# icrdr/3D-UNet-Renal-Anatomy-Extraction

Measured on AMD Instinct MI355X. Metric: train voxels/sec (128^3 patch, bs=2 per GPU), whole job, higher is better.
Workload: dtype bf16; 1 GPU; ResUnet3D(num_pool=4, num_features=32, in=1, out=3) train step (fwd+HybirdLoss+bwd+Adam), 2x1x128^3 per GPU, dropout on; global_batch=2, parallelism=dp1, optimizer=optim.Adam (fused multi-tensor)

## Files before the change

3d-unet-renal-anatomy-extraction_amd/_native.py:

```python
import ctypes
import os
import threading

import torch

_HERE = os.path.dirname(os.path.abspath(__file__))
LIB_PATH = os.environ.get("RU3D_LIB", os.path.join(_HERE, "libru3d.so"))

F32, BF16, F16 = 0, 1, 2
PREDICT_MAX_BATCH = 16
LABEL_I64, LABEL_U8 = 0, 1
ROLE_CONV_FWD, ROLE_CONV_DGRAD, ROLE_CONVT_FWD, ROLE_CONVT_DGRAD, ROLE_BIAS = 0, 1, 2, 3, 4
LOSS_HYBIRD, LOSS_DICELOSS, LOSS_FOCAL, LOSS_DICE = 0, 1, 2, 3
MAX_CLASSES = 8


class Tensor(ctypes.Structure):
    _fields_ = [("ptr", ctypes.c_void_p), ("n", ctypes.c_int32), ("d", ctypes.c_int32), ("h", ctypes.c_int32),
                ("w", ctypes.c_int32), ("c", ctypes.c_int32), ("ld", ctypes.c_int32), ("cseg", ctypes.c_int32),
                ("seg_stride", ctypes.c_int64)]


class PackItem(ctypes.Structure):
    _fields_ = [("src", ctypes.c_void_p), ("dst", ctypes.c_void_p), ("cout", ctypes.c_int32), ("cin", ctypes.c_int32),
                ("k", ctypes.c_int32), ("stride", ctypes.c_int32), ("role", ctypes.c_int32),
                ("cout_seg", ctypes.c_int32), ("cin_seg", ctypes.c_int32)]


class PatchParams(ctypes.Structure):
    _fields_ = [("lo", ctypes.c_int32 * 3), ("before", ctypes.c_int32 * 3), ("patch", ctypes.c_int32 * 3),
                ("flip", ctypes.c_int32 * 3), ("image_cval", ctypes.c_float), ("label_cval", ctypes.c_int32),
                ("do_contrast", ctypes.c_int32), ("do_brightness", ctypes.c_int32), ("do_gamma", ctypes.c_int32),
                ("contrast", ctypes.c_float), ("brightness", ctypes.c_float), ("gamma", ctypes.c_float),
                ("gamma_eps", ctypes.c_float)]


class SpatialParams(ctypes.Structure):
    _fields_ = [("centre", ctypes.c_double * 3), ("matrix", ctypes.c_double * 9), ("lattice", ctypes.c_int32 * 3),
                ("spacing", ctypes.c_int32 * 3)]


class DegradeParams(ctypes.Structure):
    _fields_ = [("do_noise", ctypes.c_int32), ("do_blur", ctypes.c_int32), ("do_low_res", ctypes.c_int32),
                ("noise_key", ctypes.c_uint32 * 2), ("reserved", ctypes.c_int32), ("noise_variance", ctypes.c_double),
                ("blur_sigma", ctypes.c_double), ("low_res_zoom", ctypes.c_double)]


class MorphRow(ctypes.Structure):
    _fields_ = [("dx", ctypes.c_int8), ("dy", ctypes.c_int8), ("zmask", ctypes.c_uint16)]


class RenderTile(ctypes.Structure):
    _fields_ = [("volume", ctypes.c_void_p), ("table", ctypes.c_void_p), ("overlay", ctypes.c_void_p * 2),
                ("overlay_table", ctypes.c_void_p * 2), ("vmin", ctypes.c_double), ("vmax", ctypes.c_double),
                ("origin", ctypes.c_double * 2), ("step", ctypes.c_double * 2), ("x0", ctypes.c_int32),
                ("y0", ctypes.c_int32), ("w", ctypes.c_int32), ("h", ctypes.c_int32), ("X", ctypes.c_int32),
                ("Y", ctypes.c_int32), ("Z", ctypes.c_int32), ("C", ctypes.c_int32), ("channel", ctypes.c_int32),
                ("kind", ctypes.c_int32), ("axis", ctypes.c_int32), ("index", ctypes.c_int32),
                ("overlay_mode", ctypes.c_int32 * 2)]


class RenderView(ctypes.Structure):
    _fields_ = [("o", ctypes.c_double * 3), ("du", ctypes.c_double * 3), ("dv", ctypes.c_double * 3),
                ("dw", ctypes.c_double * 3), ("spacing", ctypes.c_double * 3), ("light", ctypes.c_double * 3),
                ("ambient", ctypes.c_double), ("diffuse", ctypes.c_double), ("background", ctypes.c_double * 3),
                ("num_steps", ctypes.c_int32), ("reserved", ctypes.c_int32)]


class DsLevel(ctypes.Structure):
    _fields_ = [("logits", ctypes.c_void_p), ("stride_n", ctypes.c_int64), ("stride_c", ctypes.c_int64),
                ("stride_v", ctypes.c_int64), ("d", ctypes.c_int32), ("h", ctypes.c_int32), ("w", ctypes.c_int32),
                ("shift", ctypes.c_int32)]


DS_MAX_LEVELS = 8
MASK_NE, MASK_EQ, MASK_GT, MASK_GE = 0, 1, 2, 3
TILE_F32, TILE_U8 = 0, 1
OVERLAY_FILL, OVERLAY_OUTLINE = 0, 1
RENDER_MAX_TILES = 256
MORPH_ERODE, MORPH_DILATE = 0, 1
MORPH_MAX_EXTENT, MORPH_MAX_ROWS = 15, 225
CONFUSION_MAX_CLASSES = 32
ORDER_STATS_MAX_RANKS = 8
EDT_MAX_AXIS = 4096
SPATIAL_MAX_YZ = 2560
BOUNDARY_MAX_AXIS = 2048
DEGRADE_MAX_RADIUS = 16
PACK_MAX = 40
_P = ctypes.POINTER(Tensor)
_vp, _i, _i64, _f, _sz, _u64 = (ctypes.c_void_p, ctypes.c_int, ctypes.c_int64, ctypes.c_float, ctypes.c_size_t,
                                ctypes.c_uint64)
_dbl = ctypes.c_double

_LOSS_VIEW = [_vp, _i64, _i64, _i64, _vp, _i, _i]

SIGNATURES = {
    "ru3d_version": (_i, []),
    "ru3d_last_error": (ctypes.c_char_p, []),
    "ru3d_launch_log_begin": (None, []),
    "ru3d_launch_log_end": (ctypes.c_char_p, []),
    "ru3d_packed_weight_bytes": (_sz, [_i, _i, _i, _i, _i, _i]),
    "ru3d_pack_weight": (_i, [_vp, _vp, _i, _i, _i, _i, _i, _i, _vp]),
    "ru3d_pack_weights": (_i, [ctypes.POINTER(PackItem), _i, _i, _vp]),
    "ru3d_unpad_weight_grad": (_i, [_vp, _vp, _i, _i, _i, _i, _i, _vp]),
    "ru3d_conv3d_workspace_bytes": (_sz, [_P, _P, _i, _i, _i]),
    "ru3d_conv3d_fwd": (_i, [_P, _vp, _vp, _P, _P, _i, _i, _i, _i, _vp, _sz, _vp]),
    "ru3d_conv3d_fwd_in_workspace_bytes": (_sz, [_P, _P, _i, _i, _i]),
    "ru3d_conv3d_fwd_in": (_i, [_P, _vp, _vp, _P, _i, _i, _i, _vp, _vp, _vp, _vp, _sz, _f, _vp]),
    "ru3d_conv3d_fwd_in_lrelu_workspace_bytes": (_sz, [_P, _P, _i, _i, _i]),
    "ru3d_conv3d_fwd_in_lrelu": (_i, [_P, _vp, _vp, _P, _i, _i, _i, _vp, _vp, _vp, _P, _P, _f, _vp, _sz, _f, _vp]),
    "ru3d_planar_concat_supported": (_i, [_i, _i, _i, _i, _i, _i, _i]),
    "ru3d_conv3d_dgrad": (_i, [_P, _vp, _P, _P, _i, _i, _i, _vp, _sz, _vp]),
    "ru3d_conv3d_s2_pair_fwd_in_supported": (_i, [_P, _P, _P, _i]),
    "ru3d_conv3d_s2_pair_fwd_in_workspace_bytes": (_sz, [_P, _P, _i]),
    "ru3d_conv3d_s2_pair_fwd_in": (_i, [_P, _vp, _vp, _P, _vp, _vp, _P, _vp, _vp, _vp, _vp, _sz, _f, _i, _vp]),
    "ru3d_conv3d_s1_dgrad_pair_supported": (_i, [_P, _P, _P, _i]),
    "ru3d_conv3d_s1_dgrad_pair": (_i, [_P, _vp, _P, _vp, _P, _i, _vp]),
    "ru3d_conv3d_s2_dgrad_pair_supported": (_i, [_P, _P, _P, _P, _i]),
    "ru3d_conv3d_s2_dgrad_pair": (_i, [_P, _vp, _P, _vp, _P, _P, _i, _vp]),
    "ru3d_conv3d_wgrad_workspace_bytes": (_sz, [_P, _P, _i, _i, _i]),
    "ru3d_conv3d_wgrad": (_i, [_P, _P, _vp, _vp, _sz, _i, _i, _i, _vp]),
    "ru3d_conv3d_wgrad_bias_workspace_bytes": (_sz, [_P, _P, _i, _i, _i]),
    "ru3d_conv3d_wgrad_bias": (_i, [_P, _P, _vp, _vp, _vp, _sz, _i, _i, _i, _vp]),
    "ru3d_conv3d_wgrad_pair_supported": (_i, [_P, _P, _P, _i, _i]),
    "ru3d_conv3d_wgrad_pair_workspace_bytes": (_sz, [_P, _P, _P, _i, _i]),
    "ru3d_conv3d_wgrad_pair": (_i, [_P, _P, _P, _vp, _vp, _vp, _sz, _i, _i, _vp]),
    "ru3d_head_bwd_supported": (_i, [_P, _P, _P, _i]),
    "ru3d_head_bwd_workspace_bytes": (_sz, [_P, _i]),
    "ru3d_head_bwd": (_i, [_P, _P, _vp, _i, _P, _vp, _vp, _vp, _sz, _i, _vp]),
    "ru3d_convtranspose3d_k3s2p1_fwd": (_i, [_P, _vp, _vp, _P, _i, _vp]),
    "ru3d_convtranspose3d_k3s2p1_fwd_in_workspace_bytes": (_sz, [_P, _P, _i]),
    "ru3d_convtranspose3d_k3s2p1_fwd_in": (_i, [_P, _vp, _vp, _P, _vp, _vp, _vp, _sz, _f, _i, _vp]),
    "ru3d_convtranspose3d_k3s2p1_dgrad": (_i, [_P, _vp, _P, _i, _vp]),
    "ru3d_convtranspose3d_k3s2p1_wgrad_workspace_bytes": (_sz, [_P, _P, _i]),
    "ru3d_convtranspose3d_k3s2p1_wgrad": (_i, [_P, _P, _vp, _vp, _sz, _i, _vp]),
    "ru3d_reduce_workspace_bytes": (_sz, [_P]),
    "ru3d_instnorm_stats": (_i, [_P, _vp, _vp, _vp, _vp, _sz, _f, _i, _vp]),
    "ru3d_in_lrelu_fwd": (_i, [_P, _vp, _vp, _P, _P, _f, _i, _vp]),
    "ru3d_skip1x1_in_lrelu_fwd_supported": (_i, [_P, _P, _P, _i]),
    "ru3d_skip1x1_in_lrelu_fwd": (_i, [_P, _vp, _vp, _P, _vp, _vp, _P, _f, _i, _vp]),
    "ru3d_skip1x1_in_lrelu_head_fwd_supported": (_i, [_P, _P, _P, _P, _i]),
    "ru3d_skip1x1_in_lrelu_head_fwd": (_i, [_P, _vp, _vp, _P, _vp, _vp, _P, _vp, _vp, _P, _f, _i, _vp]),
    "ru3d_head_in_bwd_supported": (_i, [_P, _P, _P, _P, _P, _i]),
    "ru3d_head_in_bwd_workspace_bytes": (_sz, [_P, _i]),
    "ru3d_head_in_bwd": (_i, [_P, _P, _vp, _i, _P, _vp, _vp, _P, _P, _vp, _vp, _vp, _vp, _sz, _f, _i, _vp]),
    "ru3d_in_lrelu_bwd": (_i, [_P, _P, _P, _vp, _vp, _P, _P, _vp, _sz, _f, _i, _vp, _vp, _i, _vp]),
    "ru3d_in_lrelu_bwd_apply": (_i, [_P, _P, _vp, _vp, _vp, _P, _f, _i, _i, _vp]),
    "ru3d_conv3d_dgrad_in_bwd_workspace_bytes": (_sz, [_P, _P, _i, _i, _i]),
    "ru3d_conv3d_dgrad_in_bwd": (_i, [_P, _vp, _P, _vp, _vp, _P, _P, _i, _i, _f, _i, _vp, _sz, _vp]),
    "ru3d_channel_sum": (_i, [_P, _vp, _vp, _sz, _i, _vp]),
    "ru3d_batchnorm_stats_pool": (_i, [_P, _vp, _vp, _vp, _sz, _i, _vp]),
    "ru3d_batchnorm_stats_finalize": (_i, [_vp, _i, _i, _i, _dbl, _vp, _vp, _vp, _f, _f, _vp, _vp, _vp, _vp, _vp, _vp, _vp]),
    "ru3d_affine_lrelu_fwd": (_i, [_P, _vp, _vp, _P, _P, _f, _i, _vp]),
    "ru3d_batchnorm_bwd_pool": (_i, [_P, _P, _P, _vp, _vp, _P, _vp, _vp, _sz, _f, _i, _vp]),
    "ru3d_batchnorm_bwd_apply": (_i, [_P, _P, _vp, _vp, _vp, _vp, _dbl, _P, _vp, _sz, _i, _i, _vp]),
    "ru3d_dropout3d_scale": (_i, [_vp, _i, _f, _u64, _u64, _vp]),
    "ru3d_dropout3d_scale_dev": (_i, [_vp, _i, _f, _u64, _u64, _vp, _vp]),
    "ru3d_pointwise": (_i, [_i, _P, _P, _P, _P, _P, _f, _i, _vp]),
    "ru3d_copy_channels": (_i, [_P, _P, _i, _vp]),
    "ru3d_add": (_i, [_P, _P, _P, _i, _vp]),
    "ru3d_cast_f32": (_i, [_P, _P, _i, _vp]),
    "ru3d_ncdhw_to_ndhwc": (_i, [_vp, _P, _i, _vp]),
    "ru3d_ndhwc_to_ncdhw": (_i, [_P, _vp, _i, _vp]),
    "ru3d_loss_state_bytes": (_sz, [_i]),
    "ru3d_loss_state_bad_labels_offset": (_sz, []),
    "ru3d_loss_workspace_bytes": (_sz, [_i, _i64, _i]),
    "ru3d_loss_fwd": (_i, _LOSS_VIEW + [_i64, _i, _i, _f, _vp, _f, _f, _f, _vp, _vp, _vp, _sz, _vp]),
    "ru3d_loss_bwd": (_i, _LOSS_VIEW + [_i64, _i, _f, _vp, _vp, _vp, _i, _vp]),
    "ru3d_tversky": (_i, [_vp, _vp, _i64, _f, _f, _f, _vp, _vp, _sz, _vp]),
    "ru3d_predict_accumulate": (_i, [_P, _i, _i, _vp, _vp, _i, _i, _i, _i, _i, _i, _vp]),
    "ru3d_predict_merge": (_i, [_vp, _vp, _i, _i, _i, _i, _i, _i, _i, _i, _i, _i, _i, _vp, _vp]),
    "ru3d_predict_gather": (_i, [_vp, _i, _i, _i, _i, _vp, _i, _P, _vp]),
    "ru3d_predict_accumulate_weighted": (_i, [_P, _i, _i, _i, _vp, _vp, _vp, _vp, _vp, _i, _i, _i, _i, _i, _i, _vp]),
    "ru3d_group_loss_state_bytes": (_sz, []),
    "ru3d_group_loss_workspace_bytes": (_sz, [_i, _i64, _i]),
    "ru3d_group_loss_fwd": (_i, _LOSS_VIEW + [_i64, _i, _vp, _i, _i, _i, _i, _f, _vp, _f, _f, _f, _vp, _vp, _vp, _sz,
                                              _vp]),
    "ru3d_group_loss_bwd": (_i, _LOSS_VIEW + [_i64, _i, _vp, _i, _i, _i, _f, _vp, _vp, _vp, _i, _vp]),
    "ru3d_topk_select_workspace_bytes": (_sz, [_i64]),
    "ru3d_topk_select_trip_elements": (_i64, []),
    "ru3d_topk_select": (_i, [_vp, _i64, _i64, _vp, _vp, _sz, _vp]),
    "ru3d_topk_loss_state_bytes": (_sz, []),
    "ru3d_topk_loss_workspace_bytes": (_sz, [_i, _i64, _i]),
    "ru3d_topk_loss_fwd": (_i, _LOSS_VIEW + [_i64, _i, _i64, _i, _vp, _f, _f, _f, _f, _vp, _vp, _vp, _vp, _sz, _vp]),
    "ru3d_topk_loss_fwd_launches": (_i, []),
    "ru3d_topk_loss_fwd_timed": (_i, _LOSS_VIEW + [_i64, _i, _i64, _i, _vp, _f, _f, _f, _f, _vp, _vp, _vp, _vp, _sz,
                                                   _vp, _vp]),
    "ru3d_topk_loss_bwd": (_i, _LOSS_VIEW + [_i64, _i, _i, _vp, _vp, _vp, _vp, _i, _vp]),
    "ru3d_predict_accumulate_groups": (_i, [_P, _i, _i, _i, _vp, _vp, _vp, _vp, _vp, _i, _i, _i, _i, _i, _i, _vp]),
    "ru3d_predict_merge_groups": (_i, [_vp, _vp, _i, _i, _i, _i, _vp, _vp, _i, _i, _i, _i, _i, _i, _vp, _vp]),
    "ru3d_components_workspace_bytes": (_sz, [_i, _i, _i]),
    "ru3d_label_components": (_i, [_vp, _i, _i, _i, _vp, _vp, _vp, _sz, _vp]),
    "ru3d_component_stats": (_i, [_vp, _i, _i, _i, _i, _vp, _vp, _vp]),
    "ru3d_filter_components_workspace_bytes": (_sz, [_i]),
    "ru3d_filter_components": (_i, [_vp, _i, _i, _i, _i, _vp, _i, _vp, _vp, _vp, _vp, _sz, _vp]),
    "ru3d_region_accumulate": (_i, [_vp, _i, _i, _i, _i, _i, _i, _i, _vp, _vp, _i, _i, _i, _vp]),
    "ru3d_cascade_merge": (_i, [_vp, _vp, _i, _i, _i, _i, _vp, _vp]),
    "ru3d_mask_bytes": (_sz, [_i, _i, _i]),
    "ru3d_mask_pack": (_i, [_vp, _i, _i, _i, _i, _i, _vp, _vp]),
    "ru3d_mask_unpack": (_i, [_vp, _i, _i, _i, _i, _i, _vp, _vp]),
    "ru3d_binary_morph": (_i, [_vp, _vp, _i, _i, _i, _i, ctypes.POINTER(MorphRow), _i, _i, _vp]),
    "ru3d_confusion_counts": (_i, [_vp, _vp, _i64, _i, _vp, _vp]),
    "ru3d_threshold_bbox": (_i, [_vp, _i, _i, _i, _i, _f, _vp, _vp, _vp]),
    "ru3d_masked_sample_workspace_bytes": (_sz, [_i, _i, _i]),
    "ru3d_masked_sample": (_i, [_vp, _i, _i, _i, _i, _i, _vp, _i, _i, _vp, _i64, _vp, _vp, _sz, _vp]),
    "ru3d_order_stats_workspace_bytes": (_sz, []),
    "ru3d_order_stats": (_i, [_vp, _i64, ctypes.POINTER(ctypes.c_int64), _i, _vp, _vp, _sz, _vp]),
    "ru3d_moments_workspace_bytes": (_sz, []),
    "ru3d_moments": (_i, [_vp, _i64, _vp, _vp, _sz, _vp]),
    "ru3d_edt_workspace_bytes": (_sz, [_i, _i, _i]),
    "ru3d_edt_squared": (_i, [_vp, _i, _i, _i, ctypes.POINTER(_dbl), _vp, _vp, _sz, _vp]),
    "ru3d_mask_surface": (_i, [_vp, _vp, _i, _i, _i, _vp]),
    "ru3d_edt_gather_workspace_bytes": (_sz, [_i, _i, _i]),
    "ru3d_edt_gather": (_i, [_vp, _vp, _i, _i, _i, _vp, _i64, _vp, _vp, _sz, _vp]),
    "ru3d_edt_reduce_workspace_bytes": (_sz, [_i64]),
    "ru3d_edt_reduce": (_i, [_vp, _vp, _i64, _dbl, _vp, _vp, _sz, _vp]),
    "ru3d_skeleton_workspace_bytes": (_sz, [_i, _i, _i]),
    "ru3d_skeleton_thin": (_i, [_vp, _i, _i, _i, _i, _vp, _sz, _vp]),
    "ru3d_skeleton_classify": (_i, [_vp, _i, _i, _i, _vp, _vp, _vp, _vp]),
    "ru3d_skeleton_length": (_i, [_vp, _i, _i, _i, ctypes.POINTER(_dbl), _vp, _vp, _sz, _vp]),
    "ru3d_skeleton_overlap": (_i, [_vp, _vp, _i, _i, _i, _vp, _vp]),
    "ru3d_skeleton_radius_stats": (_i, [_vp, _i64, _vp, _vp]),
    "ru3d_cldice_workspace_bytes": (_sz, [_i, _i, _i, _i, _i]),
    "ru3d_cldice_state_bytes": (_sz, []),
    "ru3d_soft_skeleton_fwd": (_i, [_vp, _i, _i, _i, _i, _i, _vp, _vp, _vp, _vp, _vp, _sz, _vp]),
    "ru3d_soft_skeleton_bwd": (_i, [_vp, _i, _i, _i, _i, _i, _vp, _vp, _vp, _vp, _vp, _vp, _sz, _vp]),
    "ru3d_cldice_fwd": (_i, _LOSS_VIEW + [_i, _i, _i, _i, _vp, _i, _i, _vp, _f, _vp, _vp, _vp, _vp, _vp, _vp, _vp, _vp,
                                          _sz, _vp]),
    "ru3d_cldice_bwd": (_i, _LOSS_VIEW + [_i, _i, _i, _i, _vp, _i, _i, _vp, _vp, _vp, _vp, _vp, _vp, _vp, _f, _i, _vp,
                                          _vp, _sz, _vp]),
    "ru3d_boundary_workspace_bytes": (_sz, [_i, _i, _i, _i]),
    "ru3d_boundary_state_bytes": (_sz, []),
    "ru3d_signed_distance": (_i, [_vp, _i, _i, _i, _i, _i, _i, _vp, _i, _vp, _vp, _vp, _sz, _vp]),
    "ru3d_boundary_fwd": (_i, _LOSS_VIEW + [_i, _i, _i, _i, _vp, _i, _vp, _vp, _vp, _vp, _vp, _sz, _vp]),
    "ru3d_boundary_bwd": (_i, [_vp, _i64, _i64, _i64, _i, _i, _i, _i, _i, _vp, _i, _vp, _vp, _vp, _f, _i, _vp, _vp]),
    "ru3d_ds_state_bytes": (_sz, []),
    "ru3d_ds_state_bad_labels_offset": (_sz, []),
    "ru3d_ds_block_bytes": (_sz, []),
    "ru3d_ds_loss_workspace_bytes": (_sz, [ctypes.POINTER(DsLevel), _i, _i]),
    "ru3d_ds_loss_fwd": (_i, [ctypes.POINTER(DsLevel), _i, _vp, _i, _i, _i, _i, _i, _i, _i, _f, _vp, _f, _f, _f, _vp, _vp,
                              _vp, _vp, _sz, _vp]),
    "ru3d_ds_loss_bwd": (_i, [ctypes.POINTER(DsLevel), ctypes.POINTER(_vp), _i, _vp, _i, _i, _i, _i, _i, _i, _f, _vp, _vp,
                              _vp]),
    "ru3d_mesh_workspace_bytes": (_sz, [_i, _i, _i]),
    "ru3d_mesh_count": (_i, [_vp, _i, _i, _i, _vp, _vp, _sz, _vp]),
    "ru3d_mesh_emit": (_i, [_vp, _i, _i, _i, _vp, _vp, _i64, _vp, _i64, _vp, _vp, _sz, _vp]),
    "ru3d_mesh_smooth": (_i, [_vp, _vp, _vp, _i64, _dbl, _vp]),
    "ru3d_mesh_measure_workspace_bytes": (_sz, [_i64]),
    "ru3d_mesh_measure": (_i, [_vp, _i64, _vp, _i64, _vp, _vp, _sz, _vp]),
    "ru3d_render_tiles": (_i, [_vp, _i, _vp, _i, _i, _vp]),
    "ru3d_render_surface_workspace_bytes": (_sz, [_i, _i, _i]),
    "ru3d_render_surface_prepare": (_i, [_vp, _i, _i, _i, _vp, _vp, _sz, _vp]),
    "ru3d_render_surface": (_i, [_vp, _i, _i, _i, _vp, ctypes.POINTER(RenderView), _vp, _vp, _i, _i, _vp, _sz, _vp]),
    "ru3d_adam_multi": (_i, [_vp, _vp, _i, _i, _f, _f, _f, _f, _f, _f, _f, _vp]),
    "ru3d_adam_multi_dev": (_i, [_vp, _vp, _i, _i, _vp, _vp]),
    "ru3d_adam_multi_amp": (_i, [_vp, _vp, _i, _i, _vp, _vp, _vp]),
    "ru3d_amp_update": (_i, [_vp, _f, _f, _i, _f, _f, _vp]),
    "ru3d_grad_sumsq": (_i, [_vp, _vp, _i, _i, _vp, _vp]),
    "ru3d_grad_norm_finish": (_i, [_vp, _i, _f, _vp, _f, _vp, _vp]),
    "ru3d_grad_norm": (_i, [_vp, _vp, _i, _i, _vp, _f, _f, _vp, _vp]),
    "ru3d_grad_scale_dev": (_i, [_vp, _vp, _i, _i, _vp, _vp]),
    "ru3d_sgd_multi": (_i, [_vp, _vp, _i, _i, _f, _f, _f, _i, _f, _vp, _vp]),
    "ru3d_sgd_multi_dev": (_i, [_vp, _vp, _i, _i, _vp, _vp, _vp]),
    "ru3d_adamw_multi": (_i, [_vp, _vp, _i, _i, _f, _f, _f, _f, _f, _f, _f, _f, _vp, _vp]),
    "ru3d_adamw_multi_dev": (_i, [_vp, _vp, _i, _i, _vp, _vp, _vp]),
    "ru3d_adam_multi_clip": (_i, [_vp, _vp, _i, _i, _f, _f, _f, _f, _f, _f, _f, _vp, _vp]),
    "ru3d_adam_multi_clip_dev": (_i, [_vp, _vp, _i, _i, _vp, _vp, _vp]),
    "ru3d_adam_step": (_i, [_vp, _vp, _vp, _vp, _i64, _f, _f, _f, _f, _f, _f, _f, _vp]),
    "ru3d_augment_workspace_bytes": (_sz, [_i, _i, _i]),
    "ru3d_augment_label_presence": (_i, [_vp, _i, _i, _i, _i, ctypes.POINTER(ctypes.c_int32),
                                        ctypes.POINTER(ctypes.c_int32), _i, _vp, _vp]),
    "ru3d_augment_patch": (_i, [_vp, _vp, _i, _i, _i, _i, _i, ctypes.POINTER(PatchParams), _vp, _vp, _vp, _vp, _sz,
                               _vp]),
    "ru3d_augment_patch_spatial": (_i, [_vp, _vp, _i, _i, _i, _i, _i, ctypes.POINTER(PatchParams),
                                       ctypes.POINTER(SpatialParams), _vp, _vp, _vp, _vp, _vp, _sz, _vp]),
    "ru3d_augment_degrade_workspace_bytes": (_sz, [_i, _i, _i, _i]),
    "ru3d_augment_degrade": (_i, [_vp, _i, _i, _i, _i, ctypes.POINTER(DegradeParams), _vp, _sz, _vp, _vp]),
    "ru3d_augment_intensity": (_i, [_vp, _i64, _vp, _i, ctypes.POINTER(PatchParams), _vp]),
    "ru3d_grad_scale_check": (_i, [_vp, _vp, _i, _i, _f, _vp, _vp]),
    "ru3d_comm_unique_id": (_i, [_vp]),
    "ru3d_comm_init": (_i, [ctypes.POINTER(_vp), _vp, _i, _i, _i]),
    "ru3d_comm_allreduce": (_i, [_vp, _vp, _i64, _i, _i, _vp]),
    "ru3d_comm_reduce_scatter": (_i, [_vp, _vp, _i64, _i, _i, _vp]),
    "ru3d_comm_all_gather": (_i, [_vp, _vp, _i64, _i, _vp]),
    "ru3d_comm_available": (_i, []),
    "ru3d_comm_destroy": (_i, [_vp]),
    "ru3d_probe_begin": (_i, [_i, _i, _i, _i, _i, _i]),
    "ru3d_probe_end": (_i, [ctypes.POINTER(ctypes.c_int), ctypes.POINTER(ctypes.c_double)]),
    "ru3d_set_cu_budget_device": (_i, [_i, _i]),
    "ru3d_set_cu_budget": (_i, [_i]),
    "ru3d_get_cu_budget": (_i, []),
    "ru3d_flat_cast": (_i, [_vp, _i, _vp, _i, _i64, _f, _vp]),
}
COMM_ID_BYTES = 128


def _load():
    if not os.path.exists(LIB_PATH):
        raise ImportError(
            "libru3d.so not found at %s - build it with `python __graft_entry__.py build` "
            "(hipcc --offload-arch=gfx950). There is no non-HIP fallback for the 3D U-Net hot path." % LIB_PATH)
    lib = ctypes.CDLL(LIB_PATH)
    for name, (res, args) in SIGNATURES.items():
        fn = getattr(lib, name)
        fn.restype = res
        fn.argtypes = args
    return lib


lib = _load()


class Ru3dError(RuntimeError):
    pass


def check(rc, what=""):
    if rc != 0:
        msg = lib.ru3d_last_error().decode("utf-8", "replace")
        raise Ru3dError("ru3d %s failed (status %d): %s" % (what, rc, msg))


_tls = threading.local()


def note_device(device):
    _tls.device = device


def stream(device=None):
    if device is not None:
        _tls.device = device
    dev = getattr(_tls, "device", None)
    return ctypes.c_void_p(torch.cuda.current_stream(dev).cuda_stream)


def dtype_code(dt):
    if dt == torch.float32:
        return F32
    if dt == torch.bfloat16:
        return BF16
    if dt == torch.float16:
        return F16
    raise Ru3dError("ru3d: unsupported storage dtype %s (float32, bfloat16 or float16)" % dt)


def require_device(t, what="tensor"):
    if not t.is_cuda:
        raise Ru3dError("ru3d: %s lives on %s; the MI355X-native path has no CPU fallback - move the model "
                        "and its inputs to a HIP device (.cuda())" % (what, t.device))
    _tls.device = t.device


def new_act(n, c, d, h, w, dtype, device, zero=False):
    buf = (torch.zeros if zero else torch.empty)((n, d, h, w, c), dtype=dtype, device=device)
    return buf.permute(0, 4, 1, 2, 3)


def is_ndhwc(t):
    if t.dim() != 5:
        return False
    n, c, d, h, w = t.shape
    sn, sc, sd, sh, sw = t.stride()
    if c > 1 and sc != 1:
        return False
    ld = None
    for size, stride, inner in ((w, sw, 1), (h, sh, w), (d, sd, h * w), (n, sn, d * h * w)):
        if size > 1:
            if stride % inner != 0:
                return False
            cand = stride // inner
            if ld is None:
                ld = cand
            elif cand != ld:
                return False
    return ld is None or ld >= c


def to_ndhwc(t):
    if is_ndhwc(t):
        return t
    return t.contiguous(memory_format=torch.channels_last_3d)


class Split:

    def __init__(self, t):
        n2, c, d, h, w = t.shape
        if n2 % 2 or not is_ndhwc(t) or not t.is_contiguous(memory_format=torch.channels_last_3d):
            raise Ru3dError("ru3d: a split concat must be a dense NDHWC tensor [2N, C/2, D, H, W]")
        self.t = t
        self.shape = torch.Size((n2 // 2, 2 * c, d, h, w))
        self.dtype = t.dtype
        self.device = t.device
        self.is_cuda = t.is_cuda

    def element_size(self):
        return self.t.element_size()

    def desc(self):
        n, c, d, h, w = self.shape
        _tls.device = self.t.device
        return Tensor(self.t.data_ptr(), n, d, h, w, c, c // 2, c // 2, n * d * h * w * (c // 2))


_GEOM = {}


def desc(t):
# ... 51 lines not shown
```

3d-unet-renal-anatomy-extraction_amd/_ops.py:

```python
import ctypes
import os
import threading
import weakref

import torch

import _native as N
from _native import check, desc, ptr, ref, stream

LRELU_SLOPE = 0.01
IN_EPS = 1e-5


def pack_weight(w, role, dtype, stride=1):
    N.require_device(w, "weight")
    w = w.detach()
    if w.dtype != torch.float32 or not w.is_contiguous():
        w = w.float().contiguous()
    k = w.shape[2]
    if role in (N.ROLE_CONVT_FWD, N.ROLE_CONVT_DGRAD):
        cin, cout = w.shape[0], w.shape[1]
    else:
        cout, cin = w.shape[0], w.shape[1]
    code = N.dtype_code(dtype)
    if role in (N.ROLE_CONVT_FWD, N.ROLE_CONVT_DGRAD):
        stride = 2
    nbytes = N.lib.ru3d_packed_weight_bytes(cout, cin, k, stride, role, code)
    if nbytes == 0:
        raise N.Ru3dError("ru3d: cannot pack weight of shape %s" % (tuple(w.shape),))
    out = torch.empty(nbytes, dtype=torch.uint8, device=w.device)
    check(N.lib.ru3d_pack_weight(ptr(w), ptr(out), cout, cin, k, stride, role, code, stream()), "pack_weight")
    return out


_PACK_PLANS = {}
_PACK_CACHE = {}
WEIGHTS_EPOCH = [0]


def cpad(c):
    return (c + 31) // 32 * 32


def padded_dim(real, seg):
    return (real // seg) * cpad(seg) if seg else real


def seg_of(real, have, nseg=1):
    if real % nseg or nseg * cpad(real // nseg) != have:
        raise N.Ru3dError("ru3d: a tensor with %d channels is not the padded form of %d channels in %d segment(s)"
                          % (have, real, nseg))
    return real // nseg


_PREPACK = {}


def _spec_key(sp, code):
    w, role, stride, cs, ci = sp
    return (code, w.data_ptr(), tuple(w.shape), role, stride, cs, ci)


def _prepacked(specs, code):
    if not _PREPACK:
        return None
    st = None
    outs = []
    for sp in specs:
        hit = _PREPACK.get(_spec_key(sp, code))
        if hit is None:
            return None
        pack, wref, ver, epoch, stream_id = hit
        w = sp[0]
        if st is None:
            st = torch.cuda.current_stream(w.device).cuda_stream
        if wref() is not w or ver != w._version or epoch != WEIGHTS_EPOCH[0] or stream_id != st:
            return None
        outs.append(pack)
    return outs


def prepack(specs, dtype):
    _PREPACK.clear()
    code = N.dtype_code(dtype)
    seen, uniq = set(), []
    for sp in specs:
        sp = sp if len(sp) == 5 else (sp[0], sp[1], sp[2], 0, 0)
        k = _spec_key(sp, code)
        if k not in seen:
            seen.add(k)
            uniq.append(sp)
    if not uniq:
        return

    def order(sp):
        w, role = sp[0], sp[1]
        if role == N.ROLE_BIAS:
            return (2, 0)
        return (0 if w.shape[2] == 3 else 1, 0)
    uniq.sort(key=order)
    packs = pack_weights(uniq, dtype)
    st = torch.cuda.current_stream(uniq[0][0].device).cuda_stream
    for sp, pk in zip(uniq, packs):
        _PREPACK[_spec_key(sp, code)] = (pk, weakref.ref(sp[0]), sp[0]._version, WEIGHTS_EPOCH[0], st)


def pack_weights(specs, dtype):
    code = N.dtype_code(dtype)
    specs = [sp if len(sp) == 5 else (sp[0], sp[1], sp[2], 0, 0) for sp in specs]
    pre = _prepacked(specs, code)
    if pre is not None:
        return pre
    key = (code,) + tuple((w.data_ptr(), w.shape, role, stride, cs, ci) for w, role, stride, cs, ci in specs)
    plan = _PACK_PLANS.get(key)
    if plan is None:
        metas, sizes = [], []
        for w, role, stride, cout_seg, cin_seg in specs:
            N.require_device(w, "weight")
            if w.dtype != torch.float32 or not w.is_contiguous():
                raise N.Ru3dError("ru3d: weights must be contiguous float32 parameters")
            if role == N.ROLE_BIAS:
                cout, cin, k, stride = w.shape[0], 1, 1, 1
                nbytes = 4 * padded_dim(cout, cout_seg)
            else:
                k = w.shape[2]
                if role in (N.ROLE_CONVT_FWD, N.ROLE_CONVT_DGRAD):
                    cin, cout, stride = w.shape[0], w.shape[1], 2
                else:
                    cout, cin = w.shape[0], w.shape[1]
                nbytes = N.lib.ru3d_packed_weight_bytes(padded_dim(cout, cout_seg), padded_dim(cin, cin_seg), k, stride,
                                                        role, code)
            if nbytes == 0:
                raise N.Ru3dError("ru3d: cannot pack weight of shape %s" % (tuple(w.shape),))
            metas.append((w.data_ptr(), cout, cin, k, stride, role, cout_seg, cin_seg))
            sizes.append((nbytes + 255) // 256 * 256)
        offs, off = [], 0
        for sz in sizes:
            offs.append(off)
            off += sz
        chunks = []
        for i0 in range(0, len(metas), N.PACK_MAX):
            chunk = metas[i0:i0 + N.PACK_MAX]
            items = (N.PackItem * len(chunk))()
            for j, (src, cout, cin, k, stride, role, cout_seg, cin_seg) in enumerate(chunk):
                items[j] = N.PackItem(src, 0, cout, cin, k, stride, role, cout_seg, cin_seg)
            chunks.append((i0, items))
        plan = (sizes, offs, off, chunks)
        if len(_PACK_PLANS) > 4096:
            _PACK_PLANS.clear()
        _PACK_PLANS[key] = plan
    sizes, offs, total, chunks = plan
    dev0 = specs[0][0].device
    N.note_device(dev0)
    ver = tuple(sp[0]._version for sp in specs) + (WEIGHTS_EPOCH[0], torch.cuda.current_stream(dev0).cuda_stream)
    use_cache = not torch.is_grad_enabled()
    hit = _PACK_CACHE.get(key) if use_cache else None
    if hit is not None and hit[0] == ver and all(r() is sp[0] for r, sp in zip(hit[2], specs)):
        return hit[1]
    buf = torch.empty(total, dtype=torch.uint8, device=dev0)
    base = buf.data_ptr()
    outs = [buf[o:o + sz] for o, sz in zip(offs, sizes)]
    st = stream()
    for i0, items in chunks:
        for j in range(len(items)):
            items[j].dst = base + offs[i0 + j]
        check(N.lib.ru3d_pack_weights(items, len(items), code, st), "pack_weights")
    if use_cache:
        if len(_PACK_CACHE) > 4096:
            _PACK_CACHE.clear()
        _PACK_CACHE[key] = (ver, outs, [weakref.ref(sp[0]) for sp in specs])
    return outs


def unpad_wgrad(dw_p, cout, cin, cout_seg, cin_seg):
    if not cout_seg and not cin_seg:
        return dw_p
    k = dw_p.shape[2]
    out = torch.empty((cout, cin, k, k, k), dtype=torch.float32, device=dw_p.device)
    N.note_device(dw_p.device)
    check(N.lib.ru3d_unpad_weight_grad(ptr(dw_p), ptr(out), cout, cin, k * k * k, cout_seg, cin_seg, stream()),
          "unpad_weight_grad")
    return out


def _bias(b):
    if b is None:
        return None
    b = b.detach()
    return b if (b.dtype == torch.float32 and b.is_contiguous()) else b.float().contiguous()


def _conv_out(size, k, s):
    return (size + 2 * (k // 2) - k) // s + 1


class Probe:

    def __init__(self, n, cin, cout, extent):
        self.key = (int(n),) + tuple(int(e) for e in extent) + (int(cin), int(cout))
        self.count = 0
        self.total_ms = 0.0
        self.active = False

    def start(self):
        check(N.lib.ru3d_probe_begin(*self.key), "probe_begin")
        self.active = True

    def stop(self):
        if not self.active:
            return
        n = ctypes.c_int(0)
        ms = ctypes.c_double(0.0)
        check(N.lib.ru3d_probe_end(ctypes.byref(n), ctypes.byref(ms)), "probe_end")
        self.count += n.value
        self.total_ms += ms.value
        self.active = False

    def result(self):
        self.stop()
        return self.count, (self.total_ms / self.count if self.count else 0.0)


def set_probe(p):
    cur = _PROBE[0]
    if cur is not None and cur is not p:
        cur.stop()
    _PROBE[0] = p
    if p is not None:
        p.start()


_PROBE = [None]


class launch_log:

    def __init__(self):
        self.names = []

    def __enter__(self):
        N.lib.ru3d_launch_log_begin()
        return self

    def __exit__(self, *exc):
        s = N.lib.ru3d_launch_log_end().decode("utf-8", "replace")
        self.names = s.split(";") if s else []
        return False


def _conv_ws(dsrc, ddst, k, stride, dtype, device):
    if k != 3 or stride != 1 or dtype == torch.float32:
        return None, 0
    need = N.lib.ru3d_conv3d_workspace_bytes(ref(dsrc), ref(ddst), k, stride, N.dtype_code(dtype))
    if need == 0:
        return None, 0
    buf = N.workspace(need, device)
    return ptr(buf), buf.numel()


def conv_fwd(x, pw, bias, cout, k, stride, res=None, out_dtype=None):
    n, _, d, h, w = x.shape
    out_dtype = out_dtype or x.dtype
    y = N.new_act(n, cout, _conv_out(d, k, stride), _conv_out(h, k, stride), _conv_out(w, k, stride), out_dtype,
                  x.device)
    b = _bias(bias)
    dx, dyy = desc(x), desc(y)
    dr = desc(res) if res is not None else None
    ws, wsn = _conv_ws(dx, dyy, k, stride, x.dtype, x.device)
    check(N.lib.ru3d_conv3d_fwd(ref(dx), ptr(pw), ptr(b), ref(dr), ref(dyy), k, stride, N.dtype_code(x.dtype),
                                N.dtype_code(out_dtype), ws, wsn, stream()), "conv3d_fwd")
    return y


def conv_fwd_in(x, pw, bias, cout, k, stride, drop_scale=None):
    n, _, d, h, w = x.shape
    y = N.new_act(n, cout, _conv_out(d, k, stride), _conv_out(h, k, stride), _conv_out(w, k, stride), x.dtype, x.device)
    mean = torch.empty(n * cout, dtype=torch.float32, device=x.device)
    scale = torch.empty(n * cout, dtype=torch.float32, device=x.device)
    b = _bias(bias)
    dx, dyy = desc(x), desc(y)
    code = N.dtype_code(x.dtype)
    ws = N.workspace(N.lib.ru3d_conv3d_fwd_in_workspace_bytes(ref(dx), ref(dyy), k, stride, code), x.device)
    check(N.lib.ru3d_conv3d_fwd_in(ref(dx), ptr(pw), ptr(b), ref(dyy), k, stride, code, ptr(drop_scale), ptr(mean),
                                   ptr(scale), ptr(ws), ws.numel(), IN_EPS, stream()), "conv3d_fwd_in")
    return y, mean, scale


# ... 1133 lines not shown
```

3d-unet-renal-anatomy-extraction_amd/csrc/api.hip:

```cpp
#include "common.h"
#include "conv.h"
#include <string>

#ifndef RU3D_STORAGE_F16

static thread_local std::string g_last_error;

int ru3d_fail(int code, const char* fmt, ...) {
    char buf[512];
    va_list ap;
    va_start(ap, fmt);
    vsnprintf(buf, sizeof(buf), fmt, ap);
    va_end(ap);
    g_last_error = buf;
    return code;
}

static thread_local std::string g_launch_log;
static thread_local bool g_launch_log_armed = false;

int ru3d_check_launch(const char* what) {
    if (g_launch_log_armed) {
        if (!g_launch_log.empty()) g_launch_log += ';';
        g_launch_log += what;
    }
    hipError_t e = hipGetLastError();
    if (e != hipSuccess) {
        ru3d_fail((int)e, "%s: %s", what, hipGetErrorString(e));
        return (int)e > 0 ? (int)e : 1;
    }
    return 0;
}

extern "C" int ru3d_version(void) { return RU3D_VERSION; }
extern "C" const char* ru3d_last_error(void) { return g_last_error.c_str(); }
extern "C" void ru3d_launch_log_begin(void) {
    g_launch_log.clear();
    g_launch_log_armed = true;
}
extern "C" const char* ru3d_launch_log_end(void) {
    g_launch_log_armed = false;
    return g_launch_log.c_str();
}
#endif

namespace RU3D_NS {

static bool dtype_ok(int d) { return d == RU3D_F32 || d == RU3D_BF16; }
static int conv_out(int in, int k, int s) { return (in + 2 * (k / 2) - k) / s + 1; }

static void role_channels(int cout, int cin, int role, int* kin, int* kout, int64_t* s_o, int64_t* s_i, int taps) {
    switch (role) {
        case RU3D_ROLE_CONV_FWD:
            *kin = cin; *kout = cout; *s_o = (int64_t)cin * taps; *s_i = taps; break;
        case RU3D_ROLE_CONV_DGRAD:
            *kin = cout; *kout = cin; *s_o = taps; *s_i = (int64_t)cin * taps; break;
        case RU3D_ROLE_CONVT_FWD:
            *kin = cin; *kout = cout; *s_o = taps; *s_i = (int64_t)cout * taps; break;
        default:
            *kin = cout; *kout = cin; *s_o = (int64_t)cout * taps; *s_i = taps; break;
    }
}

static bool role_uses_mfma(int kin, int kout, int k, int stride, int role, int dtype) {
    (void)stride;
    (void)role;
    return mfma_conv_eligible(kin, kout, k, dtype, dtype);
}

extern "C" size_t ru3d_packed_weight_bytes(int cout, int cin, int k, int stride, int role, int dtype) {
    RU3D_FWD_F16(dtype, ru3d_packed_weight_bytes_f16(cout, cin, k, stride, role, dtype));
    if (cout <= 0 || cin <= 0 || (k != 1 && k != 3) || (stride != 1 && stride != 2) || role < 0 || role > 3 ||
        !dtype_ok(dtype))
        return 0;
    const int taps = k * k * k;
    int kin, kout;
    int64_t s_o, s_i;
    role_channels(cout, cin, role, &kin, &kout, &s_o, &s_i, taps);
    if (role_uses_mfma(kin, kout, k, stride, role, dtype)) return mfma_packed_bytes(kin, kout, taps);
    return (size_t)taps * kin * generic_cout_pad(kout) * (dtype == RU3D_F32 ? 4 : 2);
}

extern "C" int ru3d_pack_weight(const float* src, void* dst, int cout, int cin, int k, int stride, int role, int dtype,
                                void* stream) {
    RU3D_FWD_F16(dtype, ru3d_pack_weight_f16(src, dst, cout, cin, k, stride, role, dtype, stream));
    Ru3dDeviceGuard dev_guard(stream);
    RU3D_REQUIRE(src && dst, "pack_weight: null pointer");
    RU3D_REQUIRE(cout > 0 && cin > 0 && (k == 1 || k == 3) && (stride == 1 || stride == 2),
                 "pack_weight: bad shape cout=%d cin=%d k=%d stride=%d", cout, cin, k, stride);
    RU3D_REQUIRE(role >= 0 && role <= 3 && dtype_ok(dtype), "pack_weight: bad role/dtype");
    const int taps = k * k * k;
    int kin, kout;
    int64_t s_o, s_i;
    role_channels(cout, cin, role, &kin, &kout, &s_o, &s_i, taps);
    if (role_uses_mfma(kin, kout, k, stride, role, dtype))
        return pack_mfma_launch(src, dst, kin, kout, taps, s_o, s_i, 0, as_stream(stream));
    return pack_generic_launch(src, dst, kin, kout, taps, s_o, s_i, 0, dtype, as_stream(stream));
}

static int pad32(int c) { return (c + 31) / 32 * 32; }
static int padded_dim(int real, int seg) { return seg > 0 ? (real / seg) * pad32(seg) : real; }

extern "C" int ru3d_pack_weights(const ru3d_pack_item* items, int count, int dtype, void* stream) {
    RU3D_FWD_F16(dtype, ru3d_pack_weights_f16(items, count, dtype, stream));
    Ru3dDeviceGuard dev_guard(stream);
    RU3D_REQUIRE(items && count > 0 && count <= RU3D_PACK_MAX, "pack_weights: count must be 1..%d", RU3D_PACK_MAX);
    RU3D_REQUIRE(dtype_ok(dtype), "pack_weights: bad dtype");
    PackBatch b;
    b.count = count;
    for (int i = 0; i < count; i++) {
        const ru3d_pack_item& it = items[i];
        RU3D_REQUIRE(it.src && it.dst && it.cout > 0 && it.cin > 0 && (it.k == 1 || it.k == 3) &&
                         (it.stride == 1 || it.stride == 2) && it.role >= 0 && it.role <= RU3D_ROLE_BIAS,
                     "pack_weights: bad item %d", i);
        RU3D_REQUIRE(it.cout_seg >= 0 && it.cin_seg >= 0 && (it.cout_seg == 0 || it.cout % it.cout_seg == 0) &&
                         (it.cin_seg == 0 || it.cin % it.cin_seg == 0),
                     "pack_weights: item %d: segments (%d, %d) do not divide (%d, %d)", i, it.cout_seg, it.cin_seg,
                     it.cout, it.cin);
        PackOne& p = b.item[i];
        p.src = it.src;
        p.dst = it.dst;
        if (it.role == RU3D_ROLE_BIAS) {
            p.mfma = 2;
            p.cout = padded_dim(it.cout, it.cout_seg);
            p.cin = 1; p.taps = 1; p.cout_pad = p.cout; p.s_o = 1; p.s_i = 1;
            p.co_real = it.cout_seg; p.co_pad = it.cout_seg ? pad32(it.cout_seg) : 0;
            p.ci_real = 0; p.ci_pad = 0;
            p.total = p.cout;
            continue;
        }
        const int taps = it.k * it.k * it.k;
        int kin, kout;
        int64_t s_o, s_i;
        role_channels(it.cout, it.cin, it.role, &kin, &kout, &s_o, &s_i, taps);
        const bool in_is_cin = (it.role == RU3D_ROLE_CONV_FWD || it.role == RU3D_ROLE_CONVT_FWD);
        const int kin_seg = in_is_cin ? it.cin_seg : it.cout_seg, kout_seg = in_is_cin ? it.cout_seg : it.cin_seg;
        const int kin_p = padded_dim(kin, kin_seg), kout_p = padded_dim(kout, kout_seg);
        p.cin = kin_p; p.cout = kout_p; p.taps = taps; p.s_o = s_o; p.s_i = s_i;
        p.ci_real = kin_seg; p.ci_pad = kin_seg ? pad32(kin_seg) : 0;
        p.co_real = kout_seg; p.co_pad = kout_seg ? pad32(kout_seg) : 0;
        p.mfma = role_uses_mfma(kin_p, kout_p, it.k, it.stride, it.role, dtype) ? 1 : 0;
        p.cout_pad = generic_cout_pad(kout_p);
        p.total = p.mfma ? (int64_t)taps * kin_p * kout_p : (int64_t)taps * kin_p * p.cout_pad;
    }
    PackPairBatch pairs;
    pairs.count = 0;
    if (dtype == RU3D_BF16) {
        for (int i = 0; i < count; i++) {
            PackOne& p = b.item[i];
            const ru3d_pack_item& it = items[i];
            if (p.mfma != 1 || (p.cin % 32) || (p.cout % 32) || (p.taps != 27 && p.taps != 1)) continue;
            const bool is_t = it.role == RU3D_ROLE_CONVT_FWD || it.role == RU3D_ROLE_CONVT_DGRAD;
            const bool a_major = it.role == RU3D_ROLE_CONV_FWD || it.role == RU3D_ROLE_CONVT_DGRAD;
            const int a_seg = is_t ? it.cin_seg : it.cout_seg, b_seg = is_t ? it.cout_seg : it.cin_seg;
            const int a_realdim = is_t ? it.cin : it.cout, b_realdim = is_t ? it.cout : it.cin;
            int slot = -1;
            for (int j = 0; j < pairs.count; j++)
                if (pairs.item[j].src == it.src && pairs.item[j].taps == p.taps &&
                    pairs.item[j].adim == padded_dim(a_realdim, a_seg) && pairs.item[j].bdim == padded_dim(b_realdim, b_seg) &&
                    pairs.item[j].a_real == a_seg && pairs.item[j].b_real == b_seg &&
                    (a_major ? !pairs.item[j].dst_a : !pairs.item[j].dst_b))
                    slot = j;
            if (slot < 0) {
                slot = pairs.count++;
                PackPair& q = pairs.item[slot];
                q.src = it.src; q.dst_a = nullptr; q.dst_b = nullptr;
                q.adim = padded_dim(a_realdim, a_seg); q.bdim = padded_dim(b_realdim, b_seg); q.taps = p.taps;
                q.a_real = a_seg; q.a_pad = a_seg ? pad32(a_seg) : 0;
                q.b_real = b_seg; q.b_pad = b_seg ? pad32(b_seg) : 0;
                q.s_a = (int64_t)b_realdim * p.taps;
            }
            (a_major ? pairs.item[slot].dst_a : pairs.item[slot].dst_b) = p.dst;
            p.mfma = 3;
        }
    }
    bool rest = false;
    for (int i = 0; i < count; i++) rest = rest || b.item[i].mfma != 3;
    if (pairs.count) {
        int rc = pack_pair_launch(pairs, as_stream(stream));
        if (rc || !rest) return rc;
    }
    return pack_batch_launch(b, dtype, as_stream(stream));
}

#ifndef RU3D_STORAGE_F16
extern "C" int ru3d_unpad_weight_grad(const float* src, float* dst, int cout, int cin, int taps, int cout_seg,
                                      int cin_seg, void* stream) {
    Ru3dDeviceGuard dev_guard(stream);
    RU3D_REQUIRE(src && dst && cout > 0 && cin > 0 && taps > 0, "unpad_weight_grad: bad argument");
    RU3D_REQUIRE(cout_seg >= 0 && cin_seg >= 0 && (cout_seg == 0 || cout % cout_seg == 0) &&
                     (cin_seg == 0 || cin % cin_seg == 0), "unpad_weight_grad: bad segments");
    return unpad_weight_launch(src, dst, cout, cin, taps, cout_seg, cout_seg ? pad32(cout_seg) : 0, cin_seg,
                               cin_seg ? pad32(cin_seg) : 0, padded_dim(cin, cin_seg), as_stream(stream));
}
#endif

static ConvGeom conv_geom(const ru3d_tensor* x, const ru3d_tensor* y, const ru3d_tensor* res, int k, int stride,
                          int transposed = 0, int flip = 0, int zero_far = 0) {
    ConvGeom g;
    g.N = x->n;
    g.Di = x->d; g.Hi = x->h; g.Wi = x->w; g.Cin = x->c; g.ldx = x->ld;
    g.Do = y->d; g.Ho = y->h; g.Wo = y->w; g.Cout = y->c; g.ldy = y->ld;
    g.CoutPad = generic_cout_pad(y->c);
    g.ldr = res ? res->ld : 0;
    g.k = k; g.stride = stride; g.pad = k / 2;
    g.transposed = transposed; g.zero_far = zero_far; g.flip = flip;
    g.x_cseg = x->cseg; g.x_segstride = x->seg_stride; g.y_cseg = y->cseg; g.y_segstride = y->seg_stride;
    return g;
}
static ConvGeom fwd_geom(const ru3d_tensor* x, const ru3d_tensor* y, int k, int stride) { return conv_geom(x, y, nullptr, k, stride); }
static ConvGeom dgrad_s1_geom(const ru3d_tensor* dy, const ru3d_tensor* da, int k) { return conv_geom(dy, da, nullptr, k, 1, 0, 1); }

static Conv3S1Plan s1_plan_for(const ConvGeom& g, int dtype) {
    return mfma_conv_eligible(g.Cin, g.Cout, g.k, dtype, dtype) ? conv3_s1_plan(g) : Conv3S1Plan();
}

static int run_conv(const ru3d_tensor* x, const void* w, const float* bias, const ru3d_tensor* res,
                    const ru3d_tensor* y, int k, int stride, int transposed, int flip, int zero_far, int dtype,
                    int y_dtype, hipStream_t st, void* ws = nullptr, size_t ws_bytes = 0) {
    const ConvGeom g = conv_geom(x, y, res, k, stride, transposed, flip, zero_far);
    if (g.x_cseg || g.y_cseg) {
        if (!(mfma_conv_eligible(g.Cin, g.Cout, k, dtype, y_dtype) && mfma_conv_geometry_ok(g)))
            return ru3d_fail(-1, "conv3d: no kernel takes a split tensor for this shape / dtype");
        return conv_mfma_launch(x->ptr, w, bias, res ? res->ptr : nullptr, y->ptr, g, st, nullptr, ws, ws_bytes);
    }
    if (stem_fwd_eligible(g, dtype, y_dtype, res)) return stem_fwd_launch(x->ptr, w, bias, y->ptr, g, dtype, st);
    if (head_fwd_eligible(g, dtype, res)) return head_fwd_launch(x->ptr, w, bias, y->ptr, g, dtype, y_dtype, st);
    if (!bias && head_dgrad_eligible(g, dtype, y_dtype, res)) return head_dgrad_launch(x->ptr, w, y->ptr, g, dtype, st);
    if (mfma_conv_eligible(g.Cin, g.Cout, k, dtype, y_dtype) && mfma_conv_geometry_ok(g))
        return conv_mfma_launch(x->ptr, w, bias, res ? res->ptr : nullptr, y->ptr, g, st, nullptr, ws, ws_bytes);
    if (mfma_conv_eligible(g.Cin, g.Cout, k, dtype, dtype))
        return ru3d_fail(-1, "conv3d: %d -> %d channels k=%d is packed in MFMA fragment order, which has no kernel for "
                             "input dtype %d -> output dtype %d", g.Cin, g.Cout, k, dtype, y_dtype);
    return conv_generic_launch(x->ptr, w, bias, res ? res->ptr : nullptr, y->ptr, g, dtype, y_dtype, st);
}

static bool res_ok(const ru3d_tensor* res, const ru3d_tensor* y) {
    return !res || (tensor_ok(res) && res->n == y->n && res->d == y->d && res->h == y->h && res->w == y->w &&
                    res->c == y->c);
}

extern "C" size_t ru3d_conv3d_workspace_bytes(const ru3d_tensor* x, const ru3d_tensor* y, int k, int stride, int dtype) {
    RU3D_FWD_F16(dtype, ru3d_conv3d_workspace_bytes_f16(x, y, k, stride, dtype));
    if (!tensor_ok_split(x) || !tensor_ok(y) || dtype != RU3D_BF16 || k != 3 || stride != 1) return 0;
    return s1_plan_for(fwd_geom(x, y, k, stride), dtype).ws_bytes;
}

extern "C" int ru3d_conv3d_fwd(const ru3d_tensor* x, const void* w_packed, const float* bias, const ru3d_tensor* res,
                               const ru3d_tensor* y, int k, int stride, int dtype, int y_dtype, void* ws,
                               size_t ws_bytes, void* stream) {
    RU3D_FWD_F16(dtype, ru3d_conv3d_fwd_f16(x, w_packed, bias, res, y, k, stride, dtype, y_dtype, ws, ws_bytes, stream));
    Ru3dDeviceGuard dev_guard(stream);
    RU3D_REQUIRE(tensor_ok_split(x) && tensor_ok(y) && w_packed, "conv3d_fwd: bad tensor/weight");
    RU3D_REQUIRE((k == 1 || k == 3) && (stride == 1 || stride == 2), "conv3d_fwd: k=%d stride=%d unsupported", k, stride);
    RU3D_REQUIRE(dtype_ok(dtype) && dtype_ok(y_dtype) && !(dtype == RU3D_F32 && y_dtype == RU3D_BF16),
                 "conv3d_fwd: bad dtypes %d -> %d", dtype, y_dtype);
    RU3D_REQUIRE(x->n == y->n && y->d == conv_out(x->d, k, stride) && y->h == conv_out(x->h, k, stride) &&
                     y->w == conv_out(x->w, k, stride),
                 "conv3d_fwd: output extents (%d,%d,%d) do not match input (%d,%d,%d) k=%d s=%d", y->d, y->h, y->w,
                 x->d, x->h, x->w, k, stride);
    RU3D_REQUIRE(res_ok(res, y), "conv3d_fwd: residual shape mismatch");
    return run_conv(x, w_packed, bias, res, y, k, stride, 0, 0, 0, dtype, y_dtype, as_stream(stream), ws, ws_bytes);
}

static size_t fwd_in_ws_bytes(const ru3d_tensor* y, const Conv3S1Plan& p) {
    size_t need = ru3d_reduce_workspace_bytes(y);
    if (p.can_stats && p.slab_bytes > need) need = p.slab_bytes;
    return p.ws_bytes > need ? p.ws_bytes : need;
}

extern "C" size_t ru3d_conv3d_fwd_in_workspace_bytes(const ru3d_tensor* x, const ru3d_tensor* y, int k, int stride,
                                                     int dtype) {
    RU3D_FWD_F16(dtype, ru3d_conv3d_fwd_in_workspace_bytes_f16(x, y, k, stride, dtype));
    if (!tensor_ok_split(x) || !tensor_ok(y)) return 0;
    return fwd_in_ws_bytes(y, s1_plan_for(fwd_geom(x, y, k, stride), dtype));
}

static int conv_fwd_in(const ru3d_tensor* x, const void* w_packed, const float* bias, const ru3d_tensor* y, int k, int stride,
                       int dtype, const float* drop_scale, float* mean, float* scale, void* ws, size_t ws_bytes, float eps,
                       void* stream, const ConvGeom& g, const Conv3S1Plan& p) {
    RU3D_REQUIRE(ws_bytes >= fwd_in_ws_bytes(y, p), "conv3d_fwd_in: workspace too small");
    if (p.can_stats) {
        RU3D_REQUIRE(x->n == y->n && y->d == x->d && y->h == x->h && y->w == x->w, "conv3d_fwd_in: extents mismatch");
        int rc = conv_mfma_launch(x->ptr, w_packed, bias, nullptr, y->ptr, g, as_stream(stream), (float*)ws, nullptr, 0, nullptr,
                                  0, 0.f, nullptr, 0, nullptr, nullptr, &p);
        if (rc) return rc;
        return stats_slab_finalize_launch((const float*)ws, p.gx, p.cb, g.N, g.Cout, 1.0 / ((double)g.Do * g.Ho * g.Wo),
                                          drop_scale, eps, mean, scale, as_stream(stream));
    }
    int rc = ru3d_conv3d_fwd(x, w_packed, bias, nullptr, y, k, stride, dtype, dtype, ws, ws_bytes, stream);
    if (rc) return rc;
    return ru3d_instnorm_stats(y, drop_scale, mean, scale, ws, ws_bytes, eps, dtype, stream);
}

extern "C" int ru3d_conv3d_fwd_in(const ru3d_tensor* x, const void* w_packed, const float* bias, const ru3d_tensor* y,
                                  int k, int stride, int dtype, const float* drop_scale, float* mean, float* scale,
                                  void* ws, size_t ws_bytes, float eps, void* stream) {
    RU3D_FWD_F16(dtype, ru3d_conv3d_fwd_in_f16(x, w_packed, bias, y, k, stride, dtype, drop_scale, mean, scale, ws, ws_bytes, eps, stream));
    Ru3dDeviceGuard dev_guard(stream);
    RU3D_REQUIRE(tensor_ok_split(x) && tensor_ok(y) && w_packed && mean && scale && ws, "conv3d_fwd_in: bad argument");
    const ConvGeom g = fwd_geom(x, y, k, stride);
    return conv_fwd_in(x, w_packed, bias, y, k, stride, dtype, drop_scale, mean, scale, ws, ws_bytes, eps, stream, g,
                       s1_plan_for(g, dtype));
}

static bool small_conv_path(const ConvGeom& g, const Conv3S1Plan& p, int dtype) {
    return g.k == 3 && g.stride == 1 && mfma_conv_eligible(g.Cin, g.Cout, g.k, dtype, dtype) && !p.can_stats;
}

#ifndef RU3D_STORAGE_F16
extern "C" size_t ru3d_conv3d_fwd_in_lrelu_workspace_bytes(const ru3d_tensor* x, const ru3d_tensor* y, int k, int stride,
                                                           int dtype) {
    return ru3d_conv3d_fwd_in_workspace_bytes(x, y, k, stride, dtype);
}
#endif

extern "C" int ru3d_conv3d_fwd_in_lrelu(const ru3d_tensor* x, const void* w_packed, const float* bias, const ru3d_tensor* y,
                                        int k, int stride, int dtype, const float* drop_scale, float* mean, float* scale,
                                        const ru3d_tensor* res, const ru3d_tensor* out, float slope, void* ws,
                                        size_t ws_bytes, float eps, void* stream) {
    RU3D_FWD_F16(dtype, ru3d_conv3d_fwd_in_lrelu_f16(x, w_packed, bias, y, k, stride, dtype, drop_scale, mean, scale, res, out, slope, ws, ws_bytes, eps, stream));
    Ru3dDeviceGuard dev_guard(stream);
    RU3D_REQUIRE(tensor_ok_split(x) && tensor_ok(y) && tensor_ok(out) && w_packed && mean && scale && ws,
                 "conv3d_fwd_in_lrelu: bad argument");
    RU3D_REQUIRE(res_ok(res, y) && res_ok(out, y), "conv3d_fwd_in_lrelu: res / out do not have the shape of y");
    const ConvGeom g = fwd_geom(x, y, k, stride);
    const Conv3S1Plan p = s1_plan_for(g, dtype);
    const int small = (small_conv_path(g, p, dtype) && x->n == y->n && y->d == x->d && y->h == x->h &&
                       y->w == x->w) ? in_small_mode(y, false, res, out) : 0;
    if (small) {
        RU3D_REQUIRE(ws_bytes >= fwd_in_ws_bytes(y, p), "conv3d_fwd_in_lrelu: workspace too small");
// ... 477 lines not shown
```

3d-unet-renal-anatomy-extraction_amd/csrc/conv_generic.hip:

```cpp
#include "common.h"
#include "conv.h"

namespace RU3D_NS {

template <typename T, typename TO, int CO_T, int VEC, bool TRANSPOSED>
__global__ __launch_bounds__(256) void conv_generic_kernel(const T* __restrict__ x, const T* __restrict__ w,
                                                           const float* __restrict__ bias,
                                                           const TO* __restrict__ res, TO* __restrict__ y,
                                                           ConvGeom g) {
    const int64_t total = (int64_t)g.N * g.Do * g.Ho * g.Wo;
    const int64_t vo = (int64_t)blockIdx.x * 256 + threadIdx.x;
    if (vo >= total) return;
    const int co0 = blockIdx.y * CO_T;
    int ow = (int)(vo % g.Wo);
    int64_t t = vo / g.Wo;
    int oh = (int)(t % g.Ho);
    t /= g.Ho;
    int od = (int)(t % g.Do);
    int n = (int)(t / g.Do);

    float acc[CO_T];
#pragma unroll
    for (int j = 0; j < CO_T; j++) acc[j] = 0.f;

    const int k = g.k, s = g.stride, p = g.pad;
    for (int kd = 0; kd < k; kd++) {
        int id;
        if (!TRANSPOSED) {
            id = od * s + kd - p;
            if (id < 0 || id >= g.Di) continue;
        } else {
            int q = od + p - kd;
            if (q < 0 || (q % s) != 0) continue;
            id = q / s;
            if (id >= g.Di) continue;
        }
        for (int kh = 0; kh < k; kh++) {
            int ih;
            if (!TRANSPOSED) {
                ih = oh * s + kh - p;
                if (ih < 0 || ih >= g.Hi) continue;
            } else {
                int q = oh + p - kh;
                if (q < 0 || (q % s) != 0) continue;
                ih = q / s;
                if (ih >= g.Hi) continue;
            }
            for (int kw = 0; kw < k; kw++) {
                int iw;
                if (!TRANSPOSED) {
                    iw = ow * s + kw - p;
                    if (iw < 0 || iw >= g.Wi) continue;
                } else {
                    int q = ow + p - kw;
                    if (q < 0 || (q % s) != 0) continue;
                    iw = q / s;
                    if (iw >= g.Wi) continue;
                }
                const int tap = (kd * k + kh) * k + kw;
                const T* xp = x + ((((int64_t)n * g.Di + id) * g.Hi + ih) * g.Wi + iw) * g.ldx;
                const int wtap = g.flip ? (k * k * k - 1 - tap) : tap;
                const T* wp = w + (int64_t)wtap * g.Cin * g.CoutPad + co0;
                for (int ci = 0; ci < g.Cin; ci += VEC) {
                    float xv[VEC];
                    load_vec<T, VEC>(xp + ci, xv);
#pragma unroll
                    for (int u = 0; u < VEC; u++) {
                        const T* wr = wp + (int64_t)(ci + u) * g.CoutPad;
#pragma unroll
                        for (int j = 0; j < CO_T; j++) acc[j] = fmaf(xv[u], to_f32<T>(wr[j]), acc[j]);
                    }
                }
            }
        }
    }
    const bool far = g.zero_far && (od == g.Do - 1 || oh == g.Ho - 1 || ow == g.Wo - 1);
#pragma unroll
    for (int j = 0; j < CO_T; j++) {
        const int co = co0 + j;
        if (co < g.Cout) {
            float v = acc[j];
            if (bias) v += bias[co];
            if (far) v = 0.f;
            if (res) v += to_f32<TO>(res[vo * g.ldr + co]);
            y[vo * g.ldy + co] = from_f32<TO>(v);
        }
    }
}

int generic_cot(int cout) { return cout <= 4 ? 4 : (cout % 16 == 0 ? 16 : 8); }
int generic_cout_pad(int cout) {
    int t = generic_cot(cout);
    return (cout + t - 1) / t * t;
}

template <typename T, typename TO, int CO_T, int VEC>
static int launch_generic2(const void* x, const void* w, const float* bias, const void* res, void* y,
                           const ConvGeom& g, hipStream_t st) {
    const int64_t total = (int64_t)g.N * g.Do * g.Ho * g.Wo;
    dim3 grid((unsigned)((total + 255) / 256), (unsigned)(g.CoutPad / CO_T));
    if (g.transposed)
        hipLaunchKernelGGL((conv_generic_kernel<T, TO, CO_T, VEC, true>), grid, dim3(256), 0, st, (const T*)x,
                           (const T*)w, bias, (const TO*)res, (TO*)y, g);
    else
        hipLaunchKernelGGL((conv_generic_kernel<T, TO, CO_T, VEC, false>), grid, dim3(256), 0, st, (const T*)x,
                           (const T*)w, bias, (const TO*)res, (TO*)y, g);
    return ru3d_check_launch("conv_generic");
}

template <typename T, typename TO>
static int launch_generic1(const void* x, const void* w, const float* bias, const void* res, void* y,
                           const ConvGeom& g, hipStream_t st) {
    const bool v4 = (g.Cin % 4 == 0) && (g.ldx % 4 == 0) && (((uintptr_t)x) % (4 * sizeof(T)) == 0);
    const int cot = generic_cot(g.Cout);
#define GO(CO, V) return launch_generic2<T, TO, CO, V>(x, w, bias, res, y, g, st)
    if (cot == 4) { if (v4) GO(4, 4); else GO(4, 1); }
    if (cot == 8) { if (v4) GO(8, 4); else GO(8, 1); }
    if (v4) GO(16, 4); else GO(16, 1);
#undef GO
}

int conv_generic_launch(const void* x, const void* w, const float* bias, const void* res, void* y,
                        const ConvGeom& g, int dtype, int y_dtype, hipStream_t st) {
    if (dtype == RU3D_F32 && y_dtype == RU3D_F32) return launch_generic1<float, float>(x, w, bias, res, y, g, st);
    if (dtype == RU3D_BF16 && y_dtype == RU3D_BF16) return launch_generic1<bf16, bf16>(x, w, bias, res, y, g, st);
    if (dtype == RU3D_BF16 && y_dtype == RU3D_F32) return launch_generic1<bf16, float>(x, w, bias, res, y, g, st);
    return ru3d_fail(-1, "conv_generic: unsupported dtype pair (%d -> %d)", dtype, y_dtype);
}

template <typename T>
__global__ void pack_generic_kernel(const float* __restrict__ src, T* __restrict__ dst, int cin, int cout,
                                    int cout_pad, int taps, int64_t s_o, int64_t s_i, int flip) {
    const int64_t total = (int64_t)taps * cin * cout_pad;
    for (int64_t i = (int64_t)blockIdx.x * blockDim.x + threadIdx.x; i < total; i += (int64_t)gridDim.x * blockDim.x) {
        int co = (int)(i % cout_pad);
        int64_t t = i / cout_pad;
        int ci = (int)(t % cin);
        int tap = (int)(t / cin);
        float v = 0.f;
        if (co < cout) {
            int st = flip ? (taps - 1 - tap) : tap;
            v = src[co * s_o + ci * s_i + st];
        }
        dst[i] = from_f32<T>(v);
    }
}

int pack_generic_launch(const float* src, void* dst, int cin, int cout, int taps, int64_t s_o, int64_t s_i,
                        int flip, int dtype, hipStream_t st) {
    const int cp = generic_cout_pad(cout);
    const int64_t total = (int64_t)taps * cin * cp;
    int blocks = (int)((total + 255) / 256);
    if (blocks > 4096) blocks = 4096;
    if (dtype == RU3D_F32)
        hipLaunchKernelGGL(pack_generic_kernel<float>, dim3(blocks), dim3(256), 0, st, src, (float*)dst, cin, cout, cp,
                           taps, s_o, s_i, flip);
    else
        hipLaunchKernelGGL(pack_generic_kernel<bf16>, dim3(blocks), dim3(256), 0, st, src, (bf16*)dst, cin, cout, cp,
                           taps, s_o, s_i, flip);
    return ru3d_check_launch("pack_generic");
}

#define PACK_TILE_FLOATS (32 * (16 * 27 + 1))
__device__ __forceinline__ int pack_src_index(int p, int real, int pad) {
    if (pad == 0) return p;
    const int seg = p / pad, off = p - seg * pad;
    return off < real ? seg * real + off : -1;
}

template <typename T>
__global__ __launch_bounds__(256) void pack_batch_kernel(PackBatch b) {
    __shared__ float tile[PACK_TILE_FLOATS];
    const PackOne& p = b.item[blockIdx.y];
    T* dst = (T*)p.dst;
    const int taps = p.taps;
    if (p.mfma == 3) return;
    if (p.mfma == 2) {
        float* out = (float*)p.dst;
        for (int i = blockIdx.x * 256 + threadIdx.x; i < p.cout; i += gridDim.x * 256) {
            const int sc = pack_src_index(i, p.co_real, p.co_pad);
            out[i] = sc >= 0 ? p.src[sc] : 0.f;
        }
        return;
    }
    const bool rows_co = (p.s_i == taps), rows_ci = (p.s_o == taps);
    if (p.mfma && sizeof(T) == 2 && taps <= 27 && (rows_co || rows_ci)) {
        const int KS = p.cin / 16, NTT = p.cout / 32;
        const int nrows = rows_co ? 32 : 16, rowlen = (rows_co ? 16 : 32) * taps, pitch = rowlen + 1;
        for (int unit = blockIdx.x; unit < KS * NTT; unit += gridDim.x) {
            const int ks = unit / NTT, nt = unit % NTT;
            const int co_s = pack_src_index(nt * 32, p.co_real, p.co_pad);
            const int ci_s = pack_src_index(ks * 16, p.ci_real, p.ci_pad);
            int co_n = 32, ci_n = 16;
            if (p.co_pad) co_n = co_s < 0 ? 0 : min(32, p.co_real - (nt * 32) % p.co_pad);
            if (p.ci_pad) ci_n = ci_s < 0 ? 0 : min(16, p.ci_real - (ks * 16) % p.ci_pad);
            const float* base = p.src + (int64_t)(co_s < 0 ? 0 : co_s) * p.s_o + (int64_t)(ci_s < 0 ? 0 : ci_s) * p.s_i;
            const int64_t row_stride = rows_co ? p.s_o : p.s_i;
            const int row_n = rows_co ? co_n : ci_n, col_n = (rows_co ? ci_n : co_n) * taps;
            __syncthreads();
            for (int e = threadIdx.x; e < nrows * rowlen; e += 256) {
                const int r = e / rowlen, j = e - r * rowlen;
                tile[r * pitch + j] = (r < row_n && j < col_n) ? base[(int64_t)r * row_stride + j] : 0.f;
            }
            __syncthreads();
            for (int e = threadIdx.x; e < taps * 64; e += 256) {
                const int tap = e >> 6, lane = e & 63;
                const int co = lane & 31, ci0 = 8 * (lane >> 5);
                bf16x8 v;
#pragma unroll
                for (int j = 0; j < 8; j++) {
                    const int ci = ci0 + j;
                    const float f = rows_co ? tile[co * pitch + ci * taps + tap] : tile[ci * pitch + co * taps + tap];
                    v[j] = (bf16)f;
                }
                *reinterpret_cast<bf16x8*>((bf16*)p.dst + ((((int64_t)tap * KS + ks) * NTT + nt) * 64 + lane) * 8) = v;
            }
        }
        return;
    }
    for (int64_t i = (int64_t)blockIdx.x * 256 + threadIdx.x; i < p.total; i += (int64_t)gridDim.x * 256) {
        float v = 0.f;
        if (p.mfma) {
            const int KS = p.cin / 16, NTT = p.cout / 32;
            const int j = (int)(i & 7);
            const int lane = (int)((i >> 3) & 63);
            int64_t t = i >> 9;
            const int nt = (int)(t % NTT);
            t /= NTT;
            const int ks = (int)(t % KS);
            const int tap = (int)(t / KS);
            const int co = pack_src_index(nt * 32 + (lane & 31), p.co_real, p.co_pad);
            const int ci = pack_src_index(ks * 16 + 8 * (lane >> 5) + j, p.ci_real, p.ci_pad);
            if (co >= 0 && ci >= 0) v = p.src[co * p.s_o + ci * p.s_i + tap];
        } else {
            const int co = (int)(i % p.cout_pad);
            const int64_t t = i / p.cout_pad;
            const int ci = pack_src_index((int)(t % p.cin), p.ci_real, p.ci_pad);
            const int tap = (int)(t / p.cin);
            const int cs = co < p.cout ? pack_src_index(co, p.co_real, p.co_pad) : -1;
            if (cs >= 0 && ci >= 0) v = p.src[cs * p.s_o + ci * p.s_i + tap];
        }
        dst[i] = from_f32<T>(v);
    }
}

#define PP_PITCH 40
#define PP_PLANE (32 * PP_PITCH + 8)
template <int TAPS>
__global__ __launch_bounds__(256) void pack_pair_kernel(PackPairBatch pb) {
    __shared__ __attribute__((aligned(16))) bf16 tile[TAPS * PP_PLANE];
    const PackPair& p = pb.item[blockIdx.y];
    if (p.taps != TAPS) return;
    constexpr int taps = TAPS;
    const int TA = p.adim / 32, TB = p.bdim / 32;
    const int lane = threadIdx.x & 63, wave = threadIdx.x >> 6;
    for (int unit = blockIdx.x; unit < TA * TB; unit += gridDim.x) {
        const int ta = unit / TB, tb = unit % TB;
        const int a_s = pack_src_index(ta * 32, p.a_real, p.a_pad), b_s = pack_src_index(tb * 32, p.b_real, p.b_pad);
        int a_n = 32, b_n = 32;
        if (p.a_pad) a_n = a_s < 0 ? 0 : min(32, p.a_real - (ta * 32) % p.a_pad);
        if (p.b_pad) b_n = b_s < 0 ? 0 : min(32, p.b_real - (tb * 32) % p.b_pad);
        const float* base = p.src + (int64_t)(a_s < 0 ? 0 : a_s) * p.s_a + (int64_t)(b_s < 0 ? 0 : b_s) * taps;
        constexpr int run = 32 * taps;
        const int run_n = b_n * taps;
        __syncthreads();
        const bool vec_ok = ((p.s_a | run_n) & 3) == 0 && ((((uintptr_t)base) & 15) == 0);
        if (vec_ok) {
            constexpr int run4 = run / 4;
            for (int e0 = threadIdx.x; e0 < 32 * run4; e0 += 8 * 256) {
                f32x4 v[8];
#pragma unroll
                for (int u = 0; u < 8; u++) {
                    const int e = e0 + u * 256;
                    const int a = e / run4, j4 = e - a * run4;
                    const f32x4 z4 = {0.f, 0.f, 0.f, 0.f};
                    v[u] = (e < 32 * run4 && a < a_n && 4 * j4 < run_n)
                               ? *reinterpret_cast<const f32x4*>(base + (int64_t)a * p.s_a + 4 * j4) : z4;
                }
#pragma unroll
                for (int u = 0; u < 8; u++) {
                    const int e = e0 + u * 256;
                    if (e < 32 * run4) {
                        const int a = e / run4, j4 = e - a * run4;
#pragma unroll
                        for (int q = 0; q < 4; q++) {
                            const int j = 4 * j4 + q;
                            const int b = j / taps, tap = j - b * taps;
                            tile[tap * PP_PLANE + a * PP_PITCH + b] = (bf16)v[u][q];
                        }
                    }
                }
            }
        } else {
            for (int e0 = threadIdx.x; e0 < 32 * run; e0 += 4 * 256) {
                float v[4];
#pragma unroll
                for (int u = 0; u < 4; u++) {
                    const int e = e0 + u * 256;
                    const int a = e / run, j = e - a * run;
                    v[u] = (e < 32 * run && a < a_n && j < run_n) ? base[(int64_t)a * p.s_a + j] : 0.f;
                }
#pragma unroll
                for (int u = 0; u < 4; u++) {
                    const int e = e0 + u * 256;
                    const int a = e / run, j = e - a * run;
                    const int b = j / taps, tap = j - b * taps;
                    if (e < 32 * run) tile[tap * PP_PLANE + a * PP_PITCH + b] = (bf16)v[u];
                }
            }
        }
        __syncthreads();
        if (p.dst_a) {
            const int KS = p.bdim / 16, NTT = TA;
            for (int f = wave; f < taps * 2; f += 4) {
                const int tap = f >> 1, kc = f & 1;
                const bf16x8 v = *reinterpret_cast<const bf16x8*>(&tile[tap * PP_PLANE + (lane & 31) * PP_PITCH + 16 * kc + 8 * (lane >> 5)]);
                *reinterpret_cast<bf16x8*>((bf16*)p.dst_a + ((((int64_t)tap * KS + 2 * tb + kc) * NTT + ta) * 64 + lane) * 8) = v;
            }
        }
        if (p.dst_b) {
            const int KS = p.adim / 16, NTT = TB;
            for (int f = wave; f < taps * 2; f += 4) {
                const int tap = f >> 1, kc = f & 1;
                const int a0 = 16 * kc + 8 * (lane >> 5);
                bf16x8 v;
#pragma unroll
                for (int j = 0; j < 8; j++) v[j] = tile[tap * PP_PLANE + (a0 + j) * PP_PITCH + (lane & 31)];
                *reinterpret_cast<bf16x8*>((bf16*)p.dst_b + ((((int64_t)tap * KS + 2 * ta + kc) * NTT + tb) * 64 + lane) * 8) = v;
            }
        }
    }
}

int pack_pair_launch(const PackPairBatch& b, hipStream_t st) {
    int64_t mx = 1;
    for (int i = 0; i < b.count; i++) {
        const int64_t units = (int64_t)(b.item[i].adim / 32) * (b.item[i].bdim / 32);
        mx = units > mx ? units : mx;
    }
    if (mx > 1024) mx = 1024;
    bool t27 = false, t1 = false;
    for (int i = 0; i < b.count; i++) {
        t27 = t27 || b.item[i].taps == 27;
        t1 = t1 || b.item[i].taps == 1;
    }
    if (t27) hipLaunchKernelGGL(pack_pair_kernel<27>, dim3((unsigned)mx, b.count), dim3(256), 0, st, b);
    if (t1) hipLaunchKernelGGL(pack_pair_kernel<1>, dim3((unsigned)mx, b.count), dim3(256), 0, st, b);
    return ru3d_check_launch("pack_pair");
}

__global__ __launch_bounds__(256) void unpad_weight_kernel(const float* __restrict__ src, float* __restrict__ dst,
                                                           int cout, int cin, int taps, int co_real, int co_pad,
                                                           int ci_real, int ci_pad, int cin_p) {
    const int64_t total = (int64_t)cout * cin * taps;
    for (int64_t i = (int64_t)blockIdx.x * 256 + threadIdx.x; i < total; i += (int64_t)gridDim.x * 256) {
        const int tap = (int)(i % taps);
        const int64_t t = i / taps;
        const int ci = (int)(t % cin), co = (int)(t / cin);
        const int cop = co_pad ? (co / co_real) * co_pad + co % co_real : co;
        const int cip = ci_pad ? (ci / ci_real) * ci_pad + ci % ci_real : ci;
        dst[i] = src[((int64_t)cop * cin_p + cip) * taps + tap];
    }
}

int unpad_weight_launch(const float* src, float* dst, int cout, int cin, int taps, int co_real, int co_pad, int ci_real,
                        int ci_pad, int cin_p, hipStream_t st) {
    const int64_t total = (int64_t)cout * cin * taps;
    int64_t blocks = (total + 1023) / 1024;
    if (blocks > 2048) blocks = 2048;
    hipLaunchKernelGGL(unpad_weight_kernel, dim3((unsigned)blocks), dim3(256), 0, st, src, dst, cout, cin, taps, co_real,
                       co_pad, ci_real, ci_pad, cin_p);
    return ru3d_check_launch("unpad_weight_grad");
}

int pack_batch_launch(const PackBatch& b, int dtype, hipStream_t st) {
    int64_t mx = 1;
    for (int i = 0; i < b.count; i++) mx = b.item[i].total > mx ? b.item[i].total : mx;
    int64_t blocks = (mx + 1023) / 1024;
    if (blocks > 2048) blocks = 2048;
    dim3 grid((unsigned)blocks, b.count);
    if (dtype == RU3D_F32)
        hipLaunchKernelGGL(pack_batch_kernel<float>, grid, dim3(256), 0, st, b);
    else
        hipLaunchKernelGGL(pack_batch_kernel<bf16>, grid, dim3(256), 0, st, b);
    return ru3d_check_launch("pack_batch");
}

#define WG_PB 16
template <typename T>
__global__ __launch_bounds__(256) void wgrad_generic_kernel(const T* __restrict__ x, const T* __restrict__ dy,
                                                            float* __restrict__ part, WgradGeom g) {
    __shared__ float xs[WG_PB][64 + 4];
    __shared__ float ds[WG_PB][64 + 4];
    const int tid = threadIdx.x;
    const int chunk = blockIdx.x, tap = blockIdx.y;
    const int co_tiles = (g.Cout + 63) / 64;
    const int ci0 = (blockIdx.z / co_tiles) * 64, co0 = (blockIdx.z % co_tiles) * 64;
    const int kw = tap % g.k, kh = (tap / g.k) % g.k, kd = tap / (g.k * g.k);
    const int ty = tid / 16, tx = tid % 16;
    float acc[4][4];
#pragma unroll
    for (int i = 0; i < 4; i++)
#pragma unroll
        for (int j = 0; j < 4; j++) acc[i][j] = 0.f;

    const int64_t P = (int64_t)g.N * g.Do * g.Ho * g.Wo;
    const int64_t p_begin = (int64_t)chunk * g.chunk_len;
    int64_t p_end = p_begin + g.chunk_len;
    if (p_end > P) p_end = P;

    for (int64_t p0 = p_begin; p0 < p_end; p0 += WG_PB) {
#pragma unroll
        for (int r = 0; r < 4; r++) {
            const int e = tid + r * 256;
            const int pl = e / 64, c = e % 64;
            const int64_t pos = p0 + pl;
            float xv = 0.f, dv = 0.f;
            if (pos < p_end) {
                int ow = (int)(pos % g.Wo);
                int64_t t = pos / g.Wo;
                int oh = (int)(t % g.Ho);
                t /= g.Ho;
                int od = (int)(t % g.Do);
                int n = (int)(t / g.Do);
                if (co0 + c < g.Cout) dv = to_f32<T>(dy[pos * g.lddy + co0 + c]);
                const int id = od * g.stride + kd - g.pad, ih = oh * g.stride + kh - g.pad,
                          iw = ow * g.stride + kw - g.pad;
                if (ci0 + c < g.Cin && id >= 0 && id < g.Di && ih >= 0 && ih < g.Hi && iw >= 0 && iw < g.Wi)
                    xv = to_f32<T>(x[((((int64_t)n * g.Di + id) * g.Hi + ih) * g.Wi + iw) * g.ldx + ci0 + c]);
            }
            xs[pl][c] = xv;
            ds[pl][c] = dv;
        }
        __syncthreads();
#pragma unroll
        for (int pl = 0; pl < WG_PB; pl++) {
            float a[4], b[4];
#pragma unroll
            for (int i = 0; i < 4; i++) a[i] = xs[pl][ty * 4 + i];
#pragma unroll
            for (int j = 0; j < 4; j++) b[j] = ds[pl][tx * 4 + j];
#pragma unroll
            for (int i = 0; i < 4; i++)
#pragma unroll
                for (int j = 0; j < 4; j++) acc[i][j] = fmaf(a[i], b[j], acc[i][j]);
        }
        __syncthreads();
    }
    float* pp = part + ((int64_t)chunk * g.taps + tap) * g.Cin * g.Cout;
#pragma unroll
    for (int i = 0; i < 4; i++) {
        const int ci = ci0 + ty * 4 + i;
        if (ci >= g.Cin) continue;
#pragma unroll
        for (int j = 0; j < 4; j++) {
            const int co = co0 + tx * 4 + j;
            if (co < g.Cout) pp[(int64_t)ci * g.Cout + co] = acc[i][j];
        }
    }
}

template <int QX>
__global__ __launch_bounds__(256) void wgrad_reduce_kernel(const float* __restrict__ part, float* __restrict__ dw,
                                                           int chunks, int taps, int cin, int cout, int64_t s_o,
                                                           int64_t s_i) {
    constexpr int KY = 256 / QX;
    __shared__ f32x4 sh[KY][QX];
    const int64_t total = (int64_t)taps * cin * cout;
    const int ox = threadIdx.x % QX, ky = threadIdx.x / QX;
    const int64_t i0 = ((int64_t)blockIdx.x * QX + ox) * 4;
    f32x4 s = {0.f, 0.f, 0.f, 0.f};
    const bool full = (i0 + 3 < total) && ((total & 3) == 0);
    if (full) {
        f32x4 s0 = s, s1 = s, s2 = s, s3 = s;
        int c = ky;
        for (; c + 3 * KY < chunks; c += 4 * KY) {
            s0 += *reinterpret_cast<const f32x4*>(part + (int64_t)c * total + i0);
            s1 += *reinterpret_cast<const f32x4*>(part + (int64_t)(c + KY) * total + i0);
            s2 += *reinterpret_cast<const f32x4*>(part + (int64_t)(c + 2 * KY) * total + i0);
            s3 += *reinterpret_cast<const f32x4*>(part + (int64_t)(c + 3 * KY) * total + i0);
        }
        for (; c < chunks; c += KY) s0 += *reinterpret_cast<const f32x4*>(part + (int64_t)c * total + i0);
        s = (s0 + s1) + (s2 + s3);
// ... 167 lines not shown
```

3d-unet-renal-anatomy-extraction_amd/csrc/optim.hip:

```cpp
#include "common.h"
#include <stddef.h>

template <class Rule>
__device__ __forceinline__ void multi_body(const ru3d_adam_tensor* __restrict__ tensors,
                                           const int32_t* __restrict__ block_map, int chunk_elems, const Rule rule,
                                           const float* __restrict__ coef) {
    const ru3d_adam_tensor t = tensors[block_map[2 * blockIdx.x]];
    if (!t.grad) return;
    const bool first = rule.first();
    if ((first && !t.exp_avg) || (Rule::kSecond && !t.exp_avg_sq)) return;
    const int64_t begin = (int64_t)block_map[2 * blockIdx.x + 1] * chunk_elems;
    int64_t end = begin + chunk_elems;
    if (end > t.count) end = t.count;
    const float c = coef ? *coef : 1.f;
    uintptr_t bits = ((uintptr_t)t.param) | ((uintptr_t)t.grad);
    if (first) bits |= (uintptr_t)t.exp_avg;
    if (Rule::kSecond) bits |= (uintptr_t)t.exp_avg_sq;
    int64_t i = begin + (int64_t)threadIdx.x * 4;
    if ((bits & 15) == 0) {
        for (; i + 3 < end; i += 1024) {
            f32x4 p = *reinterpret_cast<const f32x4*>(t.param + i);
            const f32x4 g = *reinterpret_cast<const f32x4*>(t.grad + i);
            f32x4 m = {0.f, 0.f, 0.f, 0.f}, v = {0.f, 0.f, 0.f, 0.f};
            if (first) m = *reinterpret_cast<const f32x4*>(t.exp_avg + i);
            if (Rule::kSecond) v = *reinterpret_cast<const f32x4*>(t.exp_avg_sq + i);
#pragma unroll
            for (int k = 0; k < 4; k++) {
                float pk = p[k], mk = m[k], vk = v[k];
                rule.elem(pk, g[k], c, mk, vk);
                p[k] = pk; m[k] = mk; v[k] = vk;
            }
            *reinterpret_cast<f32x4*>(t.param + i) = p;
            if (first) *reinterpret_cast<f32x4*>(t.exp_avg + i) = m;
            if (Rule::kSecond) *reinterpret_cast<f32x4*>(t.exp_avg_sq + i) = v;
        }
    }
    for (; i < end; i += 1024)
        for (int k = 0; k < 4 && i + k < end; k++) {
            float pk = t.param[i + k], mk = first ? t.exp_avg[i + k] : 0.f, vk = Rule::kSecond ? t.exp_avg_sq[i + k] : 0.f;
            rule.elem(pk, t.grad[i + k], c, mk, vk);
            t.param[i + k] = pk;
            if (first) t.exp_avg[i + k] = mk;
            if (Rule::kSecond) t.exp_avg_sq[i + k] = vk;
        }
}

struct SgdRule {
    float lr, mu, wd, gscale;
    bool nesterov;
    static constexpr bool kSecond = false;
    __device__ __forceinline__ bool first() const { return mu != 0.f; }
    __device__ __forceinline__ void elem(float& p, float g, float c, float& b, float&) const {
#pragma clang fp contract(off)
        const float gh = g * gscale * c;
        float d = gh;
        if (wd != 0.f) d = gh + wd * p;
        float u = d;
        if (mu != 0.f) {
            b = mu * b + d;
            u = nesterov ? d + mu * b : b;
        }
        p -= lr * u;
    }
};

__device__ __forceinline__ SgdRule sgd_rule(float lr, float mu, float wd, float nesterov, float gscale) {
    SgdRule r;
    r.lr = lr; r.mu = mu; r.wd = wd; r.gscale = gscale; r.nesterov = nesterov != 0.f;
    return r;
}

__global__ __launch_bounds__(256) void sgd_multi_kernel(const ru3d_adam_tensor* __restrict__ tensors,
                                                        const int32_t* __restrict__ block_map, int chunk_elems, float lr,
                                                        float mu, float wd, float nesterov, float gscale,
                                                        const float* __restrict__ coef) {
    multi_body(tensors, block_map, chunk_elems, sgd_rule(lr, mu, wd, nesterov, gscale), coef);
}

__global__ __launch_bounds__(256) void sgd_multi_dev_kernel(const ru3d_adam_tensor* __restrict__ tensors,
                                                            const int32_t* __restrict__ block_map, int chunk_elems,
                                                            const float* __restrict__ hyper,
                                                            const float* __restrict__ coef) {
    multi_body(tensors, block_map, chunk_elems, sgd_rule(hyper[0], hyper[1], hyper[2], hyper[3], hyper[6]), coef);
}

template <bool kDecay>
struct AdamRule {
    float b1, b2, eps, step, bc2_sqrt, gscale, keep;
    static constexpr bool kSecond = true;
    __device__ __forceinline__ bool first() const { return true; }
    __device__ __forceinline__ void elem(float& p, float g, float c, float& m, float& v) const {
#pragma clang fp contract(off)
        const float gi = g * gscale * c;
        if (kDecay) p = p * keep;
        m = b1 * m + (1.f - b1) * gi;
        v = b2 * v + (1.f - b2) * gi * gi;
        p -= step * (m / (sqrtf(v) / bc2_sqrt + eps));
    }
};

template <bool kDecay>
__device__ __forceinline__ AdamRule<kDecay> adam_rule(float lr, float b1, float b2, float eps, float bc1, float bc2_sqrt,
                                                      float gscale, float wd) {
#pragma clang fp contract(off)
    AdamRule<kDecay> r;
    r.b1 = b1; r.b2 = b2; r.eps = eps; r.bc2_sqrt = bc2_sqrt; r.gscale = gscale;
    r.step = lr / bc1;
    r.keep = 1.f - lr * wd;
    return r;
}

__global__ __launch_bounds__(256) void adam_clip_kernel(const ru3d_adam_tensor* __restrict__ tensors,
                                                        const int32_t* __restrict__ block_map, int chunk_elems, float lr,
                                                        float b1, float b2, float eps, float bc1, float bc2_sqrt,
                                                        float gscale, const float* __restrict__ coef) {
    multi_body(tensors, block_map, chunk_elems, adam_rule<false>(lr, b1, b2, eps, bc1, bc2_sqrt, gscale, 0.f), coef);
}

__global__ __launch_bounds__(256) void adam_clip_dev_kernel(const ru3d_adam_tensor* __restrict__ tensors,
                                                            const int32_t* __restrict__ block_map, int chunk_elems,
                                                            const float* __restrict__ hyper,
                                                            const float* __restrict__ coef) {
    multi_body(tensors, block_map, chunk_elems,
               adam_rule<false>(hyper[0], hyper[1], hyper[2], hyper[3], hyper[4], hyper[7], hyper[6], 0.f), coef);
}

__global__ __launch_bounds__(256) void adamw_multi_kernel(const ru3d_adam_tensor* __restrict__ tensors,
                                                          const int32_t* __restrict__ block_map, int chunk_elems, float lr,
                                                          float b1, float b2, float eps, float wd, float bc1, float bc2,
                                                          float gscale, const float* __restrict__ coef) {
    multi_body(tensors, block_map, chunk_elems, adam_rule<true>(lr, b1, b2, eps, bc1, sqrtf(bc2), gscale, wd), coef);
}

__global__ __launch_bounds__(256) void adamw_multi_dev_kernel(const ru3d_adam_tensor* __restrict__ tensors,
                                                              const int32_t* __restrict__ block_map, int chunk_elems,
                                                              const float* __restrict__ hyper,
                                                              const float* __restrict__ coef) {
    multi_body(tensors, block_map, chunk_elems,
               adam_rule<true>(hyper[0], hyper[1], hyper[2], hyper[3], hyper[4], sqrtf(hyper[5]), hyper[6], hyper[7]),
               coef);
}

__global__ __launch_bounds__(256) void adam_kernel(float* __restrict__ p, const float* __restrict__ g,
                                                   float* __restrict__ m, float* __restrict__ v, int64_t count,
                                                   float lr, float b1, float b2, float eps, float bc1, float bc2_sqrt,
                                                   float gscale) {
    for (int64_t i = (int64_t)blockIdx.x * 256 + threadIdx.x; i < count; i += (int64_t)gridDim.x * 256) {
        const float gi = g[i] * gscale;
        const float mi = b1 * m[i] + (1.f - b1) * gi;
        const float vi = b2 * v[i] + (1.f - b2) * gi * gi;
        m[i] = mi;
        v[i] = vi;
        const float denom = sqrtf(vi) / bc2_sqrt + eps;
        p[i] -= (lr / bc1) * (mi / denom);
    }
}

extern "C" int ru3d_adam_step(float* param, const float* grad, float* exp_avg, float* exp_avg_sq, int64_t count,
                              float lr, float beta1, float beta2, float eps, float bias_corr1, float bias_corr2,
                              float grad_scale, void* stream) {
    Ru3dDeviceGuard dev_guard(stream);
    RU3D_REQUIRE(param && grad && exp_avg && exp_avg_sq && count > 0, "adam_step: bad argument");
    int64_t b = (count + 1023) / 1024;
    if (b > 4096) b = 4096;
    hipLaunchKernelGGL(adam_kernel, dim3((unsigned)b), dim3(256), 0, as_stream(stream), param, grad, exp_avg,
                       exp_avg_sq, count, lr, beta1, beta2, eps, bias_corr1, sqrtf(bias_corr2), grad_scale);
    return ru3d_check_launch("adam_step");
}

__device__ __forceinline__ void adam_multi_body(const ru3d_adam_tensor* __restrict__ tensors,
                                                const int32_t* __restrict__ block_map, int chunk_elems, float lr,
                                                float b1, float b2, float eps, float bc1, float bc2_sqrt, float gscale) {
#pragma clang fp contract(off)
    const ru3d_adam_tensor t = tensors[block_map[2 * blockIdx.x]];
    if (!t.grad) return;
    const int64_t begin = (int64_t)block_map[2 * blockIdx.x + 1] * chunk_elems;
    int64_t end = begin + chunk_elems;
    if (end > t.count) end = t.count;
    const float step = lr / bc1;
    const bool vec = ((((uintptr_t)t.param) | ((uintptr_t)t.grad) | ((uintptr_t)t.exp_avg) | ((uintptr_t)t.exp_avg_sq)) & 15) == 0;
    int64_t i = begin + (int64_t)threadIdx.x * 4;
    if (vec) {
        for (; i + 3 < end; i += 1024) {
            f32x4 p = *reinterpret_cast<const f32x4*>(t.param + i);
            const f32x4 g = *reinterpret_cast<const f32x4*>(t.grad + i);
            f32x4 m = *reinterpret_cast<const f32x4*>(t.exp_avg + i);
            f32x4 v = *reinterpret_cast<const f32x4*>(t.exp_avg_sq + i);
#pragma unroll
            for (int k = 0; k < 4; k++) {
                const float gi = g[k] * gscale;
                m[k] = b1 * m[k] + (1.f - b1) * gi;
                v[k] = b2 * v[k] + (1.f - b2) * gi * gi;
                p[k] -= step * (m[k] / (sqrtf(v[k]) / bc2_sqrt + eps));
            }
            *reinterpret_cast<f32x4*>(t.param + i) = p;
            *reinterpret_cast<f32x4*>(t.exp_avg + i) = m;
            *reinterpret_cast<f32x4*>(t.exp_avg_sq + i) = v;
        }
    }
    for (; i < end; i += 1024)
        for (int k = 0; k < 4 && i + k < end; k++) {
            const float gi = t.grad[i + k] * gscale;
            const float mi = b1 * t.exp_avg[i + k] + (1.f - b1) * gi;
            const float vi = b2 * t.exp_avg_sq[i + k] + (1.f - b2) * gi * gi;
            t.exp_avg[i + k] = mi;
            t.exp_avg_sq[i + k] = vi;
            t.param[i + k] -= step * (mi / (sqrtf(vi) / bc2_sqrt + eps));
        }
}


__global__ __launch_bounds__(256) void adam_multi_kernel(const ru3d_adam_tensor* __restrict__ tensors,
                                                         const int32_t* __restrict__ block_map, int chunk_elems,
                                                         float lr, float b1, float b2, float eps, float bc1,
                                                         float bc2_sqrt, float gscale) {
    adam_multi_body(tensors, block_map, chunk_elems, lr, b1, b2, eps, bc1, bc2_sqrt, gscale);
}

__global__ __launch_bounds__(256) void adam_multi_dev_kernel(const ru3d_adam_tensor* __restrict__ tensors,
                                                             const int32_t* __restrict__ block_map, int chunk_elems,
                                                             const float* __restrict__ hyper) {
    adam_multi_body(tensors, block_map, chunk_elems, hyper[0], hyper[1], hyper[2], hyper[3], hyper[4], hyper[7], hyper[6]);
}

extern "C" int ru3d_adam_multi(const ru3d_adam_tensor* tensors, const int32_t* block_map, int nblocks, int chunk_elems,
                               float lr, float beta1, float beta2, float eps, float bias_corr1, float bias_corr2,
                               float grad_scale, void* stream) {
    Ru3dDeviceGuard dev_guard(stream);
    RU3D_REQUIRE(tensors && block_map && nblocks > 0 && chunk_elems >= 1024 && (chunk_elems % 1024) == 0,
                 "adam_multi: bad argument (chunk_elems must be a positive multiple of 1024)");
    hipLaunchKernelGGL(adam_multi_kernel, dim3((unsigned)nblocks), dim3(256), 0, as_stream(stream), tensors, block_map,
                       chunk_elems, lr, beta1, beta2, eps, bias_corr1, sqrtf(bias_corr2), grad_scale);
    return ru3d_check_launch("adam_multi");
}

extern "C" int ru3d_adam_multi_dev(const ru3d_adam_tensor* tensors, const int32_t* block_map, int nblocks,
                                   int chunk_elems, const float* hyper, void* stream) {
    Ru3dDeviceGuard dev_guard(stream);
    RU3D_REQUIRE(tensors && block_map && hyper && nblocks > 0 && chunk_elems >= 1024 && (chunk_elems % 1024) == 0,
                 "adam_multi_dev: bad argument (chunk_elems must be a positive multiple of 1024)");
    hipLaunchKernelGGL(adam_multi_dev_kernel, dim3((unsigned)nblocks), dim3(256), 0, as_stream(stream), tensors,
                       block_map, chunk_elems, hyper);
    return ru3d_check_launch("adam_multi_dev");
}

__global__ __launch_bounds__(256) void adam_multi_amp_kernel(const ru3d_adam_tensor* __restrict__ tensors,
                                                             const int32_t* __restrict__ block_map, int chunk_elems,
                                                             const float* __restrict__ hyper,
                                                             const ru3d_amp_state* __restrict__ amp) {
    if (amp->found_inf != 0.f) return;
    const int t = __float_as_int(hyper[5]) + amp->steps + 1;
    const double b1d = (double)hyper[1] + (double)hyper[4], b2d = (double)hyper[2] + (double)hyper[7];
    const double bc1 = 1.0 - pow(b1d, (double)t), bc2 = 1.0 - pow(b2d, (double)t);
    adam_multi_body(tensors, block_map, chunk_elems, hyper[0], hyper[1], hyper[2], hyper[3], (float)bc1, sqrtf((float)bc2),
                    amp->inv_scale);
}

__global__ void amp_update_kernel(ru3d_amp_state* amp, float growth, float backoff, int interval, float min_scale,
                                  float max_scale) {
    if (threadIdx.x || blockIdx.x) return;
    if (amp->found_inf != 0.f) {
        amp->scale = fmaxf(amp->scale * backoff, min_scale);
        amp->tracker = 0;
        amp->skipped += 1;
    } else {
        amp->steps += 1;
        amp->tracker += 1;
        if (amp->tracker >= interval) {
            amp->scale = fminf(amp->scale * growth, max_scale);
            amp->tracker = 0;
        }
    }
    amp->inv_scale = 1.f / amp->scale;
    amp->found_inf = 0.f;
}

extern "C" int ru3d_adam_multi_amp(const ru3d_adam_tensor* tensors, const int32_t* block_map, int nblocks, int chunk_elems,
                                   const float* hyper, const ru3d_amp_state* amp, void* stream) {
    Ru3dDeviceGuard dev_guard(stream);
    RU3D_REQUIRE(tensors && block_map && hyper && amp && nblocks > 0 && chunk_elems >= 1024 && (chunk_elems % 1024) == 0,
                 "adam_multi_amp: bad argument (chunk_elems must be a positive multiple of 1024)");
    hipLaunchKernelGGL(adam_multi_amp_kernel, dim3((unsigned)nblocks), dim3(256), 0, as_stream(stream), tensors, block_map,
                       chunk_elems, hyper, amp);
    return ru3d_check_launch("adam_multi_amp");
}

extern "C" int ru3d_amp_update(ru3d_amp_state* amp, float growth_factor, float backoff_factor, int growth_interval,
                               float min_scale, float max_scale, void* stream) {
    Ru3dDeviceGuard dev_guard(stream);
    RU3D_REQUIRE(amp && growth_factor >= 1.f && backoff_factor > 0.f && backoff_factor <= 1.f && growth_interval > 0 &&
                     min_scale > 0.f && max_scale >= min_scale, "amp_update: bad argument");
    hipLaunchKernelGGL(amp_update_kernel, dim3(1), dim3(64), 0, as_stream(stream), amp, growth_factor, backoff_factor,
                       growth_interval, min_scale, max_scale);
    return ru3d_check_launch("amp_update");
}

__global__ __launch_bounds__(256) void grad_scale_check_kernel(const ru3d_adam_tensor* __restrict__ tensors,
                                                               const int32_t* __restrict__ block_map, int chunk_elems,
                                                               float scale, float* __restrict__ found_inf) {
    const ru3d_adam_tensor t = tensors[block_map[2 * blockIdx.x]];
    if (!t.grad) return;
    float* g = const_cast<float*>(t.grad);
    const int64_t begin = (int64_t)block_map[2 * blockIdx.x + 1] * chunk_elems;
    int64_t end = begin + chunk_elems;
    if (end > t.count) end = t.count;
    const bool write = scale != 1.f;
    bool bad = false;
    int64_t i = begin + (int64_t)threadIdx.x * 4;
    if ((((uintptr_t)g) & 15) == 0) {
        for (; i + 3 < end; i += 1024) {
            f32x4 v = *reinterpret_cast<const f32x4*>(g + i);
#pragma unroll
            for (int k = 0; k < 4; k++) {
                bad = bad || !(fabsf(v[k]) <= 3.402823466e38f);
                v[k] *= scale;
            }
            if (write) *reinterpret_cast<f32x4*>(g + i) = v;
        }
    }
    for (; i < end; i += 1024)
        for (int k = 0; k < 4 && i + k < end; k++) {
            const float v = g[i + k];
            bad = bad || !(fabsf(v) <= 3.402823466e38f);
            if (write) g[i + k] = v * scale;
        }
    if (__any(bad) && (threadIdx.x & 63) == 0) *found_inf = 1.f;
}

extern "C" int ru3d_grad_scale_check(const ru3d_adam_tensor* tensors, const int32_t* block_map, int nblocks,
                                     int chunk_elems, float scale, float* found_inf, void* stream) {
    Ru3dDeviceGuard dev_guard(stream);
    RU3D_REQUIRE(tensors && block_map && found_inf && nblocks > 0 && chunk_elems >= 1024 && (chunk_elems % 1024) == 0,
                 "grad_scale_check: bad argument (chunk_elems must be a positive multiple of 1024)");
    hipLaunchKernelGGL(grad_scale_check_kernel, dim3((unsigned)nblocks), dim3(256), 0, as_stream(stream), tensors,
                       block_map, chunk_elems, scale, found_inf);
    return ru3d_check_launch("grad_scale_check");
}

__device__ __forceinline__ double block_sum_d(double v, double* lds) {
    v = wave_sum_d(v);
    if ((threadIdx.x & 63) == 0) lds[threadIdx.x >> 6] = v;
    __syncthreads();
    return ((lds[0] + lds[1]) + lds[2]) + lds[3];
}

__global__ __launch_bounds__(256) void grad_sumsq_kernel(const ru3d_adam_tensor* __restrict__ tensors,
                                                         const int32_t* __restrict__ block_map, int chunk_elems,
                                                         double* __restrict__ partials) {
    __shared__ double lds[4];
    const ru3d_adam_tensor t = tensors[block_map[2 * blockIdx.x]];
    double acc = 0.0;
    if (t.grad) {
        const float* g = t.grad;
        const int64_t begin = (int64_t)block_map[2 * blockIdx.x + 1] * chunk_elems;
        int64_t end = begin + chunk_elems;
        if (end > t.count) end = t.count;
        int64_t i = begin + (int64_t)threadIdx.x * 4;
        if ((((uintptr_t)g) & 15) == 0) {
            for (; i + 3 < end; i += 1024) {
                const f32x4 v = *reinterpret_cast<const f32x4*>(g + i);
#pragma unroll
                for (int k = 0; k < 4; k++) acc += (double)v[k] * (double)v[k];
            }
        }
        for (; i < end; i += 1024)
            for (int k = 0; k < 4 && i + k < end; k++) acc += (double)g[i + k] * (double)g[i + k];
    }
    const double s = block_sum_d(acc, lds);
    if (threadIdx.x == 0) partials[blockIdx.x] = s;
}

__global__ __launch_bounds__(256) void grad_norm_finish_kernel(const double* __restrict__ partials, int n,
                                                               float grad_scale, const float* __restrict__ hyper,
                                                               float max_norm, float* __restrict__ out) {
    __shared__ double lds[4];
    double acc = 0.0;
    for (int i = threadIdx.x; i < n; i += 256) acc += partials[i];
    const double s = block_sum_d(acc, lds);
    if (threadIdx.x == 0) {
        const float gs = hyper ? hyper[6] : grad_scale;
        const float total = (float)((double)gs * sqrt(s));
        const float c = max_norm / (total + 1e-6f);
        out[0] = total;
        out[1] = c > 1.f ? 1.f : c;
    }
}

__global__ __launch_bounds__(256) void grad_scale_dev_kernel(const ru3d_adam_tensor* __restrict__ tensors,
                                                             const int32_t* __restrict__ block_map, int chunk_elems,
                                                             const float* __restrict__ coef) {
    const ru3d_adam_tensor t = tensors[block_map[2 * blockIdx.x]];
    if (!t.grad) return;
    const float c = *coef;
    if (c == 1.f) return;
    float* g = const_cast<float*>(t.grad);
    const int64_t begin = (int64_t)block_map[2 * blockIdx.x + 1] * chunk_elems;
// ... 121 lines not shown
```

3d-unet-renal-anatomy-extraction_amd/graph.py:

```python
import torch

import _native as N
import _ops
import loss as _loss
import optim as _optim

_RING = 8


class GraphedTrainStep:
    def __init__(self, model, criterion, optimizer, warmup=2, scaler=None):
        if not isinstance(optimizer, _optim._Fused):
            raise TypeError("GraphedTrainStep needs optim.Adam, optim.AdamW or optim.SGD (their update kernels read the "
                            "per-step scalars from device memory)")
        if scaler is not None and not optimizer.captures_with_scaler():
            raise TypeError("GraphedTrainStep: a captured fp16 step (device-side loss scaler) needs optim.Adam without "
                            "max_grad_norm; SGD, AdamW and clipped steps run the eager fp16 loop")
        self.model, self.criterion, self.optimizer = model, criterion, optimizer
        self.scaler = scaler
        self.warmup = max(1, int(warmup))
        self.graph = None
        self.key = None
        self.replays = 0
        self.eager_steps = 0

    def _eager(self, x, y):
        self.optimizer.zero_grad(set_to_none=True)
        logits = self.model(x)
        loss = self.criterion(logits, y)
        stepped = True
        if self.scaler is None:
            loss.backward()
            self.optimizer.step()
        elif self.scaler._dev is not None:
            stepped = self.scaler.eager_step(self.optimizer, loss)
        else:
            self.scaler.scale(loss).backward()
            stepped = self.scaler.step(self.optimizer)
        self.eager_steps += 1 if (stepped or self.graph is not None) else 0
        self.skipped_warmup = getattr(self, "skipped_warmup", 0) + (0 if stepped else 1)
        self.logits = _loss.main_output(logits).detach()
        return loss.detach()

    def _capture(self, x, y):
        dev = x.device
        groups = len(self.optimizer.param_groups)
        self.stream = torch.cuda.Stream(dev)
        drop0 = _ops._drop_counter[0]
        import loss as _loss_mod
        try:
            self.x = torch.empty_like(x)
            self.y = torch.empty_like(y)
            self.x.copy_(x)
            self.y.copy_(y)
            self.block = torch.zeros(8 + groups * 32, dtype=torch.uint8, device=dev)
            self.drop_base = self.block[:8].view(torch.int64)
            self.hyper = self.block[8:].view(torch.float32).view(groups, 8)
            self.host = [torch.zeros(8 + groups * 32, dtype=torch.uint8).pin_memory() for _ in range(_RING)]
            self.host_ev = [None] * _RING
            self.optimizer.begin_capture(self.hyper)
            if self.scaler is not None:
                self.scaler.begin_capture(self.optimizer, dev)
            self.optimizer.zero_grad(set_to_none=True)
            g = torch.cuda.CUDAGraph()
            _ops.DROP_OFFSET_BASE[0] = self.drop_base
            _loss_mod.CAPTURE_SINK[0] = self.label_states = []
            self.stream.wait_stream(torch.cuda.current_stream(dev))
            try:
                with torch.cuda.graph(g, stream=self.stream, capture_error_mode="thread_local"):
                    logits = self.model(self.x)
                    loss = self.criterion(logits, self.y)
                    if self.scaler is None:
                        loss.backward()
                        self.optimizer.step()
                    else:
                        self.scaler.scale(loss).backward()
                        self.scaler.step(self.optimizer)
                    self.loss = loss.detach()
                    self._static_logits = _loss_mod.main_output(logits).detach()
            finally:
                _ops.DROP_OFFSET_BASE[0] = None
                _loss_mod.CAPTURE_SINK[0] = None
        except BaseException:
            _ops._drop_counter[0] = drop0
            cap = self.optimizer._captured
            if cap is not None and cap["steps"]:
                cap["dirty"] = True
            self.release()
            raise
        self.draws = _ops._drop_counter[0] - drop0
        _ops._drop_counter[0] = drop0
        self.drop_origin = drop0
        self.graph = g
        self.key = (tuple(x.shape), x.dtype, tuple(y.shape), y.dtype, dev)

    def __call__(self, x, y):
        key = (tuple(x.shape), x.dtype, tuple(y.shape), y.dtype, x.device)
        if self.graph is None:
            if self.eager_steps < self.warmup:
                return self._eager(x, y)
            self._capture(x, y)
        elif key != self.key:
            return self._eager(x, y)
        else:
            self.x.copy_(x, non_blocking=True)
            self.y.copy_(y, non_blocking=True)
        slot = self.replays % _RING
        if self.host_ev[slot] is not None:
            self.host_ev[slot].synchronize()
        host = self.host[slot]
        host[:8].view(torch.int64)[0] = _ops._drop_counter[0] - self.drop_origin
        self.optimizer.replay_scalars(host[8:].view(torch.float32).view(-1, 8))
        self.block.copy_(host, non_blocking=True)
        ev = torch.cuda.Event()
        ev.record()
        self.host_ev[slot] = ev
        self.graph.replay()
        if self.label_states:
            import loss as _loss_mod
            for st in self.label_states:
                _loss_mod._note_label_flag(st)
        _ops._drop_counter[0] += self.draws
        _ops.WEIGHTS_EPOCH[0] += 1
        self.replays += 1
        self.logits = self._static_logits
        return self.loss

    def release(self):
        self.optimizer.sync_captured_steps()
        if self.scaler is not None and self.scaler._dev is not None:
            self.scaler.end_capture()
        self.optimizer.end_capture()
        if self.graph is not None or hasattr(self, "stream"):
            self.optimizer.zero_grad(set_to_none=True)
            sid = self.stream.cuda_stream
            side = _ops._SIDE.get(self.stream.device)
            sids = (sid,) if side is None else (sid, side.cuda_stream)
            for key in [k for k in N._WS if k[1] in sids]:
                del N._WS[key]
            _ops._PREPACK.clear()
            for name in ("x", "y", "loss", "logits", "_static_logits", "block", "drop_base", "hyper", "host", "host_ev",
                         "stream", "label_states"):
                if hasattr(self, name):
                    delattr(self, name)
        self.graph = None
        self.key = None
```

3d-unet-renal-anatomy-extraction_amd/optim.py:

```python
import ctypes

import torch

import _native as N
from _native import check, ptr, stream

_CHUNK = 16384


class _AdamTensor(ctypes.Structure):
    _fields_ = [("param", ctypes.c_void_p), ("grad", ctypes.c_void_p), ("exp_avg", ctypes.c_void_p),
                ("exp_avg_sq", ctypes.c_void_p), ("count", ctypes.c_int64)]


def _check_max_grad_norm(max_grad_norm):
    if max_grad_norm is None:
        return None
    max_grad_norm = float(max_grad_norm)
    if not max_grad_norm >= 0.0:
        raise ValueError("Invalid max_grad_norm: %r" % (max_grad_norm,))
    return max_grad_norm


class _Fused(torch.optim.Optimizer):
    _NAME = "optim"
    _COUNTS_STEPS = True

    def __init__(self, params, defaults, max_grad_norm=None):
        self.max_grad_norm = _check_max_grad_norm(max_grad_norm)
        super().__init__(params, defaults)
        self._plans = {}
        self._clip = {}
        self._norm = None
        self._captured = None
        self.last_grad_norm = None

    def _slots(self, p, group, capturing):
        raise NotImplementedError

    def _launch(self, plan, group, step_no, grad_scale, coef):
        raise NotImplementedError

    def _launch_dev(self, plan, hyper_row, coef):
        raise NotImplementedError

    def _row(self, row, group, step_no, grad_scale):
        raise NotImplementedError

    def _check_group(self, group):
        pass

    def captures_with_scaler(self):
        return False

    def _plan(self, gi, group, captured=False):
        plan = self._plans.get((gi, captured))
        params = [p for p in group["params"]]
        if plan is not None and plan["n"] == len(params):
            return plan
        dev = params[0].device
        blocks = []
        for ti, p in enumerate(params):
            N.require_device(p, "parameter")
            if p.dtype != torch.float32 or not p.is_contiguous():
                raise N.Ru3dError("optim.%s: parameters must be contiguous float32" % self._NAME)
            for c in range((p.numel() + _CHUNK - 1) // _CHUNK):
                blocks += [ti, c]
        bm = torch.tensor(blocks, dtype=torch.int32).to(dev)
        host = torch.empty(len(params) * ctypes.sizeof(_AdamTensor), dtype=torch.uint8).pin_memory()
        table = torch.empty(host.numel(), dtype=torch.uint8, device=dev)
        plan = {"n": len(params), "block_map": bm, "nblocks": len(blocks) // 2, "host": host, "table": table}
        self._plans[(gi, captured)] = plan
        return plan

    def _clip_buffers(self, captured=False):
        plans = [self._plan(gi, group, captured) for gi, group in enumerate(self.param_groups) if group["params"]]
        nblocks = sum(pl["nblocks"] for pl in plans)
        dev = plans[0]["table"].device
        if self._norm is None or self._norm.device != dev:
            self._norm = torch.zeros(2, dtype=torch.float32, device=dev)
        bufs = self._clip.get(captured)
        if bufs is None or bufs["partials"].numel() != nblocks or bufs["partials"].device != dev:
            bufs = {"partials": torch.empty(nblocks, dtype=torch.float64, device=dev)}
            self._clip[captured] = bufs
        bufs["norm"] = self._norm
        return bufs

    @torch.no_grad()
    def step(self, closure=None, grad_scale=1.0):
        loss = None
        if closure is not None:
            with torch.enable_grad():
                loss = closure()
        capturing = self._captured is not None and torch.cuda.is_current_stream_capturing()
        if self._captured is not None and not capturing:
            self.sync_captured_steps()
        clip = self.max_grad_norm is not None
        bufs = self._clip_buffers(capturing) if clip and any(g["params"] for g in self.param_groups) else None
        ready = []
        npartials = 0
        for gi, group in enumerate(self.param_groups):
            params = group["params"]
            if not params:
                continue
            self._check_group(group)
            plan = self._plan(gi, group, capturing)
            N.note_device(params[0].device)
            if plan.get("copied") is not None and not capturing:
                plan["copied"].synchronize()
            arr = (_AdamTensor * len(params)).from_buffer(plan["host"].numpy())
            step_no = None
            any_grad = False
            for i, p in enumerate(params):
                if p.grad is None:
                    arr[i] = _AdamTensor(p.data_ptr(), None, None, None, p.numel())
                    continue
                g = p.grad
                if g.dtype != torch.float32 or not g.is_contiguous():
                    g = g.float().contiguous()
                    p.grad = g
                first, second = self._slots(p, group, capturing)
                if self._COUNTS_STEPS:
                    st = self.state[p]
                    st["step"] += 1
                    step_no = float(st["step"]) if step_no is None else step_no
                    if float(st["step"]) != step_no:
                        raise N.Ru3dError("optim.%s: parameters of one group must share the step count" % self._NAME)
                arr[i] = _AdamTensor(p.data_ptr(), g.data_ptr(), None if first is None else first.data_ptr(),
                                     None if second is None else second.data_ptr(), p.numel())
                any_grad = True
            if not any_grad:
                continue
            step_no = 0.0 if step_no is None else step_no
            plan["table"].copy_(plan["host"], non_blocking=True)
            if capturing:
                plan["copied"] = None
            else:
                ev = torch.cuda.Event()
                ev.record()
                plan["copied"] = ev
            if clip:
                check(N.lib.ru3d_grad_sumsq(ptr(plan["table"]), ptr(plan["block_map"]), plan["nblocks"], _CHUNK,
                                            ptr(bufs["partials"][npartials:]), stream()), "grad_sumsq")
                npartials += plan["nblocks"]
            ready.append((gi, group, plan, step_no))
        coef = None
        if clip and ready:
            N.note_device(bufs["norm"].device)
            hyper0 = self._captured["hyper"][ready[0][0]] if capturing else None
            check(N.lib.ru3d_grad_norm_finish(ptr(bufs["partials"]), npartials, float(grad_scale), ptr(hyper0),
                                              self.max_grad_norm, ptr(bufs["norm"]), stream()), "grad_norm_finish")
            coef = bufs["norm"][1:]
            self.last_grad_norm = bufs["norm"][0]
        for gi, group, plan, step_no in ready:
            N.note_device(plan["table"].device)
            if capturing:
                self._captured["steps"][gi] = step_no - 1.0
                amp = self._captured.get("amp")
                if amp is not None:
                    self._captured["amp_base"][gi] = step_no - 1.0
                    check(N.lib.ru3d_adam_multi_amp(ptr(plan["table"]), ptr(plan["block_map"]), plan["nblocks"], _CHUNK,
                                                    ptr(self._captured["hyper"][gi]), ptr(amp), stream()), "adam_multi_amp")
                else:
                    self._launch_dev(plan, self._captured["hyper"][gi], coef)
                continue
            if self._captured is not None and gi in self._captured["steps"]:
                self._captured["steps"][gi] = step_no
                self._captured["amp_base"][gi] = step_no
            self._launch(plan, group, step_no, float(grad_scale), coef)
        import _ops
        _ops.WEIGHTS_EPOCH[0] += 1
        return loss

    def begin_capture(self, hyper):
        if hyper.shape != (len(self.param_groups), 8) or hyper.dtype != torch.float32:
            raise ValueError("begin_capture: hyper must be float32 [groups, 8]")
        self._captured = {"hyper": hyper, "steps": {}, "amp": None, "amp_base": {}}
        for gi, group in enumerate(self.param_groups):
            if group["params"]:
                self._plan(gi, group, True)
        if self.max_grad_norm is not None and any(g["params"] for g in self.param_groups):
            self._clip_buffers(True)

    def end_capture(self):
        self._captured = None
        for key in [k for k in self._plans if k[1]]:
            del self._plans[key]
        self._clip.pop(True, None)

    def replay_scalars(self, out, grad_scale=1.0):
        cap = self._captured
        cap["dirty"] = True
        for gi, step_no in cap["steps"].items():
            step_no += 1.0
            cap["steps"][gi] = step_no
            self._row(out[gi], self.param_groups[gi], step_no, grad_scale)

    def sync_captured_steps(self):
        cap = self._captured
        if cap is None or not cap.get("dirty"):
            return
        cap["dirty"] = False
        if not self._COUNTS_STEPS:
            return
        if cap.get("amp") is not None:
            taken = int(cap["amp"].view(torch.int32)[5].item())
            for gi in list(cap["steps"]):
                cap["steps"][gi] = cap["amp_base"].get(gi, 0.0) + taken
        for gi, step_no in cap["steps"].items():
            for p in self.param_groups[gi]["params"]:
                st = self.state.get(p)
                if st:
                    st["step"] = torch.tensor(float(step_no))

    def state_dict(self):
        self.sync_captured_steps()
        return super().state_dict()

    def load_state_dict(self, state_dict):
        super().load_state_dict(state_dict)
        for st in self.state.values():
            if torch.is_tensor(st.get("step")) and st["step"].device.type != "cpu":
                st["step"] = st["step"].detach().to("cpu", torch.float32)


class _AdamFamily(_Fused):

    def _slots(self, p, group, capturing):
        st = self.state[p]
        if len(st) == 0:
            if capturing:
                raise N.Ru3dError("optim.%s: take one eager step before capturing (the moment buffers are "
                                  "created and zeroed by the first step)" % self._NAME)
            st["step"] = torch.tensor(0.0)
            st["exp_avg"] = torch.zeros_like(p, memory_format=torch.preserve_format)
            st["exp_avg_sq"] = torch.zeros_like(p, memory_format=torch.preserve_format)
        return st["exp_avg"], st["exp_avg_sq"]

    def _check_group(self, group):
        if group.get("amsgrad") or group.get("maximize"):
            raise N.Ru3dError("optim.%s: amsgrad / maximize are not implemented" % self._NAME)


class Adam(_AdamFamily):
    _NAME = "Adam"

    def __init__(self, params, lr=1e-3, betas=(0.9, 0.999), eps=1e-8, weight_decay=0, amsgrad=False, max_grad_norm=None):
        if weight_decay != 0 or amsgrad:
            raise ValueError("ru3d optim.Adam implements plain Adam (weight_decay=0, amsgrad=False)")
        if lr < 0 or eps < 0 or not (0 <= betas[0] < 1 and 0 <= betas[1] < 1):
            raise ValueError("invalid Adam hyper-parameters")
        super().__init__(params, dict(lr=lr, betas=betas, eps=eps, weight_decay=0, amsgrad=False), max_grad_norm)

    def captures_with_scaler(self):
        return self.max_grad_norm is None

    def _launch(self, plan, group, step_no, grad_scale, coef):
        b1, b2 = group["betas"]
        bc1 = 1.0 - b1 ** step_no
        bc2 = 1.0 - b2 ** step_no
        if coef is None:
            check(N.lib.ru3d_adam_multi(ptr(plan["table"]), ptr(plan["block_map"]), plan["nblocks"], _CHUNK,
                                        float(group["lr"]), float(b1), float(b2), float(group["eps"]), bc1, bc2,
                                        float(grad_scale), stream()), "adam_multi")
        else:
            check(N.lib.ru3d_adam_multi_clip(ptr(plan["table"]), ptr(plan["block_map"]), plan["nblocks"], _CHUNK,
                                             float(group["lr"]), float(b1), float(b2), float(group["eps"]), bc1, bc2,
                                             float(grad_scale), ptr(coef), stream()), "adam_multi_clip")

    def _launch_dev(self, plan, hyper_row, coef):
        if coef is None:
            check(N.lib.ru3d_adam_multi_dev(ptr(plan["table"]), ptr(plan["block_map"]), plan["nblocks"], _CHUNK,
                                            ptr(hyper_row), stream()), "adam_multi_dev")
        else:
            check(N.lib.ru3d_adam_multi_clip_dev(ptr(plan["table"]), ptr(plan["block_map"]), plan["nblocks"], _CHUNK,
                                                 ptr(hyper_row), ptr(coef), stream()), "adam_multi_clip_dev")

    def _row(self, row, group, step_no, grad_scale):
        b1, b2 = group["betas"]
        row[0] = group["lr"]; row[1] = b1; row[2] = b2; row[3] = group["eps"]
        row[4] = 1.0 - b1 ** step_no; row[5] = 1.0 - b2 ** step_no; row[6] = grad_scale
        row[7] = float(row[5]) ** 0.5
        if self._captured.get("amp") is not None:
            gi = next(i for i, g in enumerate(self.param_groups) if g is group)
            row[5:6].view(torch.int32)[0] = int(self._captured["amp_base"].get(gi, 0.0))
            row[4] = b1 - float(torch.tensor(b1, dtype=torch.float32))
            row[7] = b2 - float(torch.tensor(b2, dtype=torch.float32))


class AdamW(_AdamFamily):
    _NAME = "AdamW"

    def __init__(self, params, lr=1e-3, betas=(0.9, 0.999), eps=1e-8, weight_decay=1e-2, amsgrad=False,
                 max_grad_norm=None):
        if not 0.0 <= lr:
            raise ValueError("Invalid learning rate: {}".format(lr))
        if not 0.0 <= eps:
            raise ValueError("Invalid epsilon value: {}".format(eps))
        if not 0.0 <= betas[0] < 1.0:
            raise ValueError("Invalid beta parameter at index 0: {}".format(betas[0]))
        if not 0.0 <= betas[1] < 1.0:
            raise ValueError("Invalid beta parameter at index 1: {}".format(betas[1]))
        if not 0.0 <= weight_decay:
            raise ValueError("Invalid weight_decay value: {}".format(weight_decay))
        if amsgrad:
            raise ValueError("ru3d optim.AdamW does not implement amsgrad")
        super().__init__(params, dict(lr=lr, betas=betas, eps=eps, weight_decay=weight_decay, amsgrad=False),
                         max_grad_norm)

    def _launch(self, plan, group, step_no, grad_scale, coef):
        b1, b2 = group["betas"]
        check(N.lib.ru3d_adamw_multi(ptr(plan["table"]), ptr(plan["block_map"]), plan["nblocks"], _CHUNK,
                                     float(group["lr"]), float(b1), float(b2), float(group["eps"]),
                                     float(group["weight_decay"]), 1.0 - b1 ** step_no, 1.0 - b2 ** step_no,
                                     float(grad_scale), ptr(coef), stream()), "adamw_multi")

    def _launch_dev(self, plan, hyper_row, coef):
        check(N.lib.ru3d_adamw_multi_dev(ptr(plan["table"]), ptr(plan["block_map"]), plan["nblocks"], _CHUNK,
                                         ptr(hyper_row), ptr(coef), stream()), "adamw_multi_dev")

    def _row(self, row, group, step_no, grad_scale):
        b1, b2 = group["betas"]
        row[0] = group["lr"]; row[1] = b1; row[2] = b2; row[3] = group["eps"]
        row[4] = 1.0 - b1 ** step_no; row[5] = 1.0 - b2 ** step_no; row[6] = grad_scale
        row[7] = group["weight_decay"]


class SGD(_Fused):
    _NAME = "SGD"
    _COUNTS_STEPS = False

    def __init__(self, params, lr, momentum=0, dampening=0, weight_decay=0, nesterov=False, max_grad_norm=None):
        if lr < 0.0:
            raise ValueError("Invalid learning rate: {}".format(lr))
        if momentum < 0.0:
            raise ValueError("Invalid momentum value: {}".format(momentum))
        if weight_decay < 0.0:
            raise ValueError("Invalid weight_decay value: {}".format(weight_decay))
        if nesterov and (momentum <= 0 or dampening != 0):
            raise ValueError("Nesterov momentum requires a momentum and zero dampening")
        if dampening != 0:
            raise ValueError("ru3d optim.SGD does not implement dampening")
        super().__init__(params, dict(lr=lr, momentum=momentum, dampening=0, weight_decay=weight_decay,
                                      nesterov=bool(nesterov)), max_grad_norm)

    def _check_group(self, group):
        if group.get("dampening", 0) != 0 or group.get("maximize"):
            raise N.Ru3dError("optim.SGD: dampening / maximize are not implemented")
        if group["nesterov"] and group["momentum"] <= 0:
            raise N.Ru3dError("optim.SGD: Nesterov momentum requires a momentum")

    def _slots(self, p, group, capturing):
        if group["momentum"] == 0:
            return None, None
        st = self.state[p]
        if st.get("momentum_buffer") is None:
            if capturing:
                raise N.Ru3dError("optim.SGD: take one eager step before capturing (the momentum buffers are created "
                                  "and zeroed by the first step)")
            st["momentum_buffer"] = torch.zeros_like(p, memory_format=torch.preserve_format)
        return st["momentum_buffer"], None

    def _launch(self, plan, group, step_no, grad_scale, coef):
        check(N.lib.ru3d_sgd_multi(ptr(plan["table"]), ptr(plan["block_map"]), plan["nblocks"], _CHUNK,
                                   float(group["lr"]), float(group["momentum"]), float(group["weight_decay"]),
                                   int(bool(group["nesterov"])), float(grad_scale), ptr(coef), stream()), "sgd_multi")

    def _launch_dev(self, plan, hyper_row, coef):
        check(N.lib.ru3d_sgd_multi_dev(ptr(plan["table"]), ptr(plan["block_map"]), plan["nblocks"], _CHUNK,
                                       ptr(hyper_row), ptr(coef), stream()), "sgd_multi_dev")

    def _row(self, row, group, step_no, grad_scale):
        row[0] = group["lr"]; row[1] = group["momentum"]; row[2] = group["weight_decay"]
        row[3] = 1.0 if group["nesterov"] else 0.0
        row[4] = 0.0; row[5] = 0.0; row[6] = grad_scale; row[7] = 0.0


_CLIP_TABLES = {}


def clip_grad_norm_(parameters, max_norm):
    if torch.is_tensor(parameters):
        parameters = [parameters]
    params = [p for p in parameters if p.grad is not None]
    max_norm = _check_max_grad_norm(max_norm)
    if max_norm is None:
        raise ValueError("clip_grad_norm_: max_norm is required")
    if not params:
        return torch.zeros(())
    dev = params[0].grad.device
    for p in params:
        N.require_device(p.grad, "gradient")
        if p.grad.device != dev:
            raise N.Ru3dError("clip_grad_norm_: gradients must share one device")
    key = (dev,) + tuple(p.numel() for p in params)
    entry = _CLIP_TABLES.get(key)
    if entry is None:
        if len(_CLIP_TABLES) >= 8:
            _CLIP_TABLES.clear()
        entry = _CLIP_TABLES[key] = {"table": _GradTable("clip_grad_norm_")}
    tab = entry["table"]
    tab.update(params)
    if entry.get("partials") is None or entry["partials"].numel() != tab.nblocks:
        entry["partials"] = torch.empty(tab.nblocks, dtype=torch.float64, device=dev)
    out = torch.empty(2, dtype=torch.float32, device=dev)
    N.note_device(dev)
    check(N.lib.ru3d_grad_norm(ptr(tab.table), ptr(tab.block_map), tab.nblocks, _CHUNK, ptr(entry["partials"]), 1.0,
                               max_norm, ptr(out), stream()), "grad_norm")
# ... 211 lines not shown
```

include/ru3d.h:

```cpp
#ifndef RU3D_H
#define RU3D_H

#include <stddef.h>
#include <stdint.h>

#ifdef __cplusplus
extern "C" {
#endif

#define RU3D_VERSION 201

enum { RU3D_F32 = 0, RU3D_BF16 = 1, RU3D_F16 = 2 };

enum { RU3D_LABEL_I64 = 0, RU3D_LABEL_U8 = 1 };

enum {
    RU3D_ROLE_CONV_FWD = 0,
    RU3D_ROLE_CONV_DGRAD = 1,
    RU3D_ROLE_CONVT_FWD = 2,
    RU3D_ROLE_CONVT_DGRAD = 3,
    RU3D_ROLE_BIAS = 4
};

enum {
// ... 259 lines not shown
int ru3d_skeleton_overlap(const uint64_t* a, const uint64_t* b, int X, int Y, int Z, int64_t* counts, void* stream);
int ru3d_skeleton_radius_stats(const double* sq, int64_t n, double* out, void* stream);

size_t ru3d_cldice_workspace_bytes(int nvol, int A, int B, int Z, int iterations);
int ru3d_soft_skeleton_fwd(const float* x, int nvol, int A, int B, int Z, int iterations, float* delta, float* s,
                           uint8_t* emin, uint8_t* dmax, void* ws, size_t ws_bytes, void* stream);
int ru3d_soft_skeleton_bwd(const float* grad_out, int nvol, int A, int B, int Z, int iterations, const float* delta,
                           const float* s, const uint8_t* emin, const uint8_t* dmax, float* grad_x, void* ws,
                           size_t ws_bytes, void* stream);
size_t ru3d_cldice_state_bytes(void);
int ru3d_cldice_fwd(const float* logits, int64_t stride_n, int64_t stride_c, int64_t stride_v, const void* labels,
                    int label_dtype, int n, int A, int B, int Z, int num_classes, const int* classes, int num_selected,
                    int iterations, const float* weight_v, float smooth, float* delta, float* s, uint8_t* emin,
                    uint8_t* dmax, float* skel_g, void* state, float* loss_out, void* ws, size_t ws_bytes, void* stream);
int ru3d_cldice_bwd(const float* logits, int64_t stride_n, int64_t stride_c, int64_t stride_v, const void* labels,
                    int label_dtype, int n, int A, int B, int Z, int num_classes, const int* classes, int num_selected,
                    int iterations, const float* delta, const float* s, const uint8_t* emin, const uint8_t* dmax,
                    const float* skel_g, const void* state, const float* grad_out, float scale, int accumulate,
                    float* dlogits, void* ws, size_t ws_bytes, void* stream);

#define RU3D_BOUNDARY_MAX_AXIS 2048
size_t ru3d_boundary_workspace_bytes(int nvol, int A, int B, int Z);
int ru3d_signed_distance(const void* labels, int label_dtype, int n, int A, int B, int Z, int num_classes,
                         const int* classes, int num_selected, int32_t* d2_out, float* phi_out, void* ws,
                         size_t ws_bytes, void* stream);
size_t ru3d_boundary_state_bytes(void);
int ru3d_boundary_fwd(const float* logits, int64_t stride_n, int64_t stride_c, int64_t stride_v, const void* labels,
                      int label_dtype, int n, int A, int B, int Z, int num_classes, const int* classes, int num_selected,
                      const float* weight_v, float* phi, void* state, float* loss_out, void* ws, size_t ws_bytes,
                      void* stream);
int ru3d_boundary_bwd(const float* logits, int64_t stride_n, int64_t stride_c, int64_t stride_v, int n, int A, int B,
                      int Z, int num_classes, const int* classes, int num_selected, const float* phi, const void* state,
                      const float* grad_out, float scale, int accumulate, float* dlogits, void* stream);

#define RU3D_DS_MAX_LEVELS 8
typedef struct ru3d_ds_level {
    const float* logits;
    int64_t stride_n, stride_c, stride_v;
    int32_t d, h, w, shift;
} ru3d_ds_level;
size_t ru3d_ds_state_bytes(void);
size_t ru3d_ds_state_bad_labels_offset(void);
size_t ru3d_ds_block_bytes(void);
size_t ru3d_ds_loss_workspace_bytes(const ru3d_ds_level* levels, int num_levels, int n);
int ru3d_ds_loss_fwd(const ru3d_ds_level* levels, int num_levels, const void* labels, int label_dtype, int n, int D, int H,
                     int W, int num_classes, int kind, float gamma, const float* weight_v, float alpha, float beta,
                     float smooth, float* block, void* state, float* loss_out, void* ws, size_t ws_bytes, void* stream);
int ru3d_ds_loss_bwd(const ru3d_ds_level* levels, void* const* dlogits, int num_levels, const void* labels,
                     int label_dtype, int n, int D, int H, int W, int num_classes, float gamma, const void* state,
                     const float* grad_out, void* stream);

size_t ru3d_mesh_workspace_bytes(int X, int Y, int Z);
int ru3d_mesh_count(const uint64_t* bits, int X, int Y, int Z, int64_t* counts, void* ws, size_t ws_bytes, void* stream);
int ru3d_mesh_emit(const uint64_t* bits, int X, int Y, int Z, int32_t* corners, int32_t* neighbours, int64_t vcap,
                   int32_t* faces, int64_t qcap, int64_t* counts, void* ws, size_t ws_bytes, void* stream);
int ru3d_mesh_smooth(const double* src, double* dst, const int32_t* neighbours, int64_t V, double factor, void* stream);
size_t ru3d_mesh_measure_workspace_bytes(int64_t F);
int ru3d_mesh_measure(const double* vertices, int64_t V, const int32_t* faces, int64_t F, double* out, void* ws,
                      size_t ws_bytes, void* stream);

#define RU3D_RENDER_MAX_TILES 256
enum { RU3D_TILE_F32 = 0, RU3D_TILE_U8 = 1 };
enum { RU3D_OVERLAY_FILL = 0, RU3D_OVERLAY_OUTLINE = 1 };
typedef struct ru3d_render_tile {
    const void* volume;
    const uint8_t* table;
    const uint8_t* overlay[2];
    const uint8_t* overlay_table[2];
    double vmin, vmax;
    double origin[2], step[2];
    int32_t x0, y0, w, h;
    int32_t X, Y, Z, C, channel, kind, axis, index;
    int32_t overlay_mode[2];
} ru3d_render_tile;
typedef struct ru3d_render_view {
    double o[3], du[3], dv[3], dw[3];
    double spacing[3];
    double light[3];
    double ambient, diffuse;
    double background[3];
    int32_t num_steps, reserved;
} ru3d_render_view;
int ru3d_render_tiles(const ru3d_render_tile* tiles, int num_tiles, uint8_t* canvas, int H, int W, void* stream);
size_t ru3d_render_surface_workspace_bytes(int X, int Y, int Z);
int ru3d_render_surface_prepare(const uint8_t* labels, int X, int Y, int Z, const uint8_t* table, void* ws, size_t ws_bytes,
                                void* stream);
int ru3d_render_surface(const uint8_t* labels, int X, int Y, int Z, const uint8_t* table, const ru3d_render_view* view,
                        uint8_t* rgb, int32_t* depth, int H, int W, const void* ws, size_t ws_bytes, void* stream);

typedef struct ru3d_patch_params {
    int32_t lo[3];
    int32_t before[3];
    int32_t patch[3];
    int32_t flip[3];
    float image_cval;
    int32_t label_cval;
    int32_t do_contrast, do_brightness, do_gamma;
    float contrast, brightness, gamma;
    float gamma_eps;
} ru3d_patch_params;
size_t ru3d_augment_workspace_bytes(int px, int py, int pz);
int ru3d_augment_label_presence(const void* label, int label_dtype, int X, int Y, int Z, const int32_t* lo,
                                const int32_t* before, int label_cval, uint32_t* mask, void* stream);
int ru3d_augment_patch(const float* image, const void* label, int label_dtype, int X, int Y, int Z, int C,
                       const ru3d_patch_params* p, const uint32_t* presence_mask, float* out_image, int64_t* out_label,
                       void* ws, size_t ws_bytes, void* stream);

#define RU3D_SPATIAL_MAX_YZ 2560
typedef struct ru3d_spatial_params {
    double centre[3];
    double matrix[9];
    int32_t lattice[3];
    int32_t spacing[3];
} ru3d_spatial_params;
int ru3d_augment_patch_spatial(const float* image, const void* label, int label_dtype, int X, int Y, int Z, int C,
                               const ru3d_patch_params* p, const ru3d_spatial_params* sp,
                               const float* lattice ,
                               const uint32_t* presence_mask, float* out_image, int64_t* out_label, void* ws,
                               size_t ws_bytes, void* stream);

#define RU3D_DEGRADE_MAX_RADIUS 16
typedef struct ru3d_degrade_params {
    int32_t do_noise, do_blur, do_low_res;
    uint32_t noise_key[2];
    int32_t reserved;
    double noise_variance;
    double blur_sigma;
    double low_res_zoom;
} ru3d_degrade_params;
size_t ru3d_augment_degrade_workspace_bytes(int C, int px, int py, int pz);
int ru3d_augment_degrade(float* image , int C, int px, int py, int pz,
                         const ru3d_degrade_params* p, void* ws, size_t ws_bytes, double* part, void* stream);
int ru3d_augment_intensity(float* image, int64_t count, const double* part, int nparts, const ru3d_patch_params* p,
                           void* stream);

int ru3d_adam_step(float* param, const float* grad, float* exp_avg, float* exp_avg_sq, int64_t count,
                   float lr, float beta1, float beta2, float eps, float bias_corr1, float bias_corr2,
                   float grad_scale, void* stream);

typedef struct ru3d_adam_tensor {
    float* param;
    const float* grad;
    float* exp_avg;
    float* exp_avg_sq;
    int64_t count;
} ru3d_adam_tensor;
int ru3d_adam_multi(const ru3d_adam_tensor* tensors, const int32_t* block_map, int nblocks, int chunk_elems,
                    float lr, float beta1, float beta2, float eps, float bias_corr1, float bias_corr2,
                    float grad_scale, void* stream);

int ru3d_adam_multi_dev(const ru3d_adam_tensor* tensors, const int32_t* block_map, int nblocks, int chunk_elems,
                        const float* hyper, void* stream);

typedef struct ru3d_amp_state {
    float scale, inv_scale, found_inf;
    int32_t tracker, skipped, steps, reserved0, reserved1;
} ru3d_amp_state;
int ru3d_adam_multi_amp(const ru3d_adam_tensor* tensors, const int32_t* block_map, int nblocks, int chunk_elems,
                        const float* hyper, const ru3d_amp_state* amp, void* stream);
int ru3d_amp_update(ru3d_amp_state* amp, float growth_factor, float backoff_factor, int growth_interval, float min_scale,
                    float max_scale, void* stream);

int ru3d_grad_sumsq(const ru3d_adam_tensor* tensors, const int32_t* block_map, int nblocks, int chunk_elems,
                    double* partials, void* stream);
int ru3d_grad_norm_finish(const double* partials, int npartials, float grad_scale, const float* hyper, float max_norm,
                          float* out, void* stream);
int ru3d_grad_norm(const ru3d_adam_tensor* tensors, const int32_t* block_map, int nblocks, int chunk_elems,
                   double* partials, float grad_scale, float max_norm, float* out, void* stream);
int ru3d_grad_scale_dev(const ru3d_adam_tensor* tensors, const int32_t* block_map, int nblocks, int chunk_elems,
                        const float* coef, void* stream);

int ru3d_sgd_multi(const ru3d_adam_tensor* tensors, const int32_t* block_map, int nblocks, int chunk_elems, float lr,
                   float momentum, float weight_decay, int nesterov, float grad_scale, const float* coef, void* stream);
int ru3d_sgd_multi_dev(const ru3d_adam_tensor* tensors, const int32_t* block_map, int nblocks, int chunk_elems,
                       const float* hyper, const float* coef, void* stream);

int ru3d_adamw_multi(const ru3d_adam_tensor* tensors, const int32_t* block_map, int nblocks, int chunk_elems, float lr,
                     float beta1, float beta2, float eps, float weight_decay, float bias_corr1, float bias_corr2,
                     float grad_scale, const float* coef, void* stream);
int ru3d_adamw_multi_dev(const ru3d_adam_tensor* tensors, const int32_t* block_map, int nblocks, int chunk_elems,
                         const float* hyper, const float* coef, void* stream);

int ru3d_adam_multi_clip(const ru3d_adam_tensor* tensors, const int32_t* block_map, int nblocks, int chunk_elems,
                         float lr, float beta1, float beta2, float eps, float bias_corr1, float bias_corr2,
                         float grad_scale, const float* coef, void* stream);
int ru3d_adam_multi_clip_dev(const ru3d_adam_tensor* tensors, const int32_t* block_map, int nblocks, int chunk_elems,
                             const float* hyper, const float* coef, void* stream);

size_t ru3d_conv3d_dgrad_in_bwd_workspace_bytes(const ru3d_tensor* dy, const ru3d_tensor* da, int k, int stride,
                                                int dtype);
int ru3d_conv3d_dgrad_in_bwd(const ru3d_tensor* dy, const void* w_packed, const ru3d_tensor* act, const float* mean,
                             const float* scale, const ru3d_tensor* da, const ru3d_tensor* dyn, int k, int stride,
                             float slope, int dtype, void* ws, size_t ws_bytes, void* stream);
int ru3d_in_lrelu_bwd_apply(const ru3d_tensor* gout, const ru3d_tensor* out, const float* mean, const float* scale,
                            const float* m12, const ru3d_tensor* dy, float slope, int zero_far, int dtype, void* stream);

int ru3d_batchnorm_stats_pool(const ru3d_tensor* y, const float* drop_scale, double* pooled, void* ws, size_t ws_bytes,
                              int dtype, void* stream);
int ru3d_batchnorm_stats_finalize(const double* pooled, int n, int c, int c_real, double count, const float* drop_scale,
                                  const float* gamma, const float* beta, float eps, float momentum, float* running_mean,
                                  float* running_var, float* fscale, float* fshift, float* a, float* b, void* stream);
int ru3d_affine_lrelu_fwd(const ru3d_tensor* y, const float* scale, const float* shift, const ru3d_tensor* res,
                          const ru3d_tensor* out, float slope, int dtype, void* stream);
int ru3d_batchnorm_bwd_pool(const ru3d_tensor* gout, const ru3d_tensor* out, const ru3d_tensor* y, const float* a,
                            const float* b, const ru3d_tensor* gpre, double* pooled, void* ws, size_t ws_bytes,
                            float slope, int dtype, void* stream);
int ru3d_batchnorm_bwd_apply(const ru3d_tensor* gpre, const ru3d_tensor* y, const float* a, const float* b,
                             const float* fscale, const double* pooled, double count, const ru3d_tensor* dy, void* ws,
                             size_t ws_bytes, int zero_far, int dtype, void* stream);

int ru3d_grad_scale_check(const ru3d_adam_tensor* tensors, const int32_t* block_map, int nblocks, int chunk_elems,
                          float scale, float* found_inf, void* stream);

#define RU3D_COMM_ID_BYTES 128
int ru3d_comm_unique_id(void* id_out);
int ru3d_comm_init(void** comm_out, const void* unique_id, int world, int rank, int device);
int ru3d_comm_allreduce(void* comm, void* buf, int64_t count, int dtype, int average, void* stream);
int ru3d_comm_reduce_scatter(void* comm, void* buf, int64_t count_per_rank, int dtype, int average, void* stream);
int ru3d_comm_all_gather(void* comm, void* buf, int64_t count_per_rank, int dtype, void* stream);
int ru3d_comm_available(void);
int ru3d_comm_destroy(void* comm);
int ru3d_probe_begin(int n, int d, int h, int w, int cin, int cout);
int ru3d_probe_end(int* launches, double* total_ms);
int ru3d_set_cu_budget_device(int device, int cus);
int ru3d_set_cu_budget(int cus);
int ru3d_get_cu_budget(void);
int ru3d_flat_cast(const void* src, int src_dtype, void* dst, int dst_dtype, int64_t count, float scale, void* stream);

#ifdef __cplusplus
}
#endif
#endif
```

Before: 267.7 million voxels/s.

## Fuse Adam update with bf16 weight repacking into MFMA fragment layouts

Adds an Adam kernel that, for conv weights with pair-packable layouts, updates fp32 params and directly writes the bf16 packed fragment buffers used by the forward and dgrad convolutions. The separate per-step weight repack pass over those weights is no longer needed. Prepack entries become persistent per-stream objects with version and epoch tracking, so only stale packs are rebuilt. This adds considerable bookkeeping complexity (capture, stream moves, epochs) and a risk of stale packed weights if the tracking is wrong.

```diff
diff --git a/3d-unet-renal-anatomy-extraction_amd/_native.py b/3d-unet-renal-anatomy-extraction_amd/_native.py
--- a/3d-unet-renal-anatomy-extraction_amd/_native.py
+++ b/3d-unet-renal-anatomy-extraction_amd/_native.py
@@ -25,6 +25,17 @@
     _fields_ = [("src", ctypes.c_void_p), ("dst", ctypes.c_void_p), ("cout", ctypes.c_int32), ("cin", ctypes.c_int32),
                 ("k", ctypes.c_int32), ("stride", ctypes.c_int32), ("role", ctypes.c_int32),
                 ("cout_seg", ctypes.c_int32), ("cin_seg", ctypes.c_int32)]
+
+
+class AdamPackItem(ctypes.Structure):
+    _fields_ = [("param", ctypes.c_void_p), ("grad", ctypes.c_void_p), ("exp_avg", ctypes.c_void_p),
+                ("exp_avg_sq", ctypes.c_void_p), ("dst_a", ctypes.c_void_p), ("dst_b", ctypes.c_void_p),
+                ("adim", ctypes.c_int32), ("bdim", ctypes.c_int32), ("taps", ctypes.c_int32), ("s_a", ctypes.c_int64),
+                ("a_real", ctypes.c_int32), ("a_pad", ctypes.c_int32), ("b_real", ctypes.c_int32),
+                ("b_pad", ctypes.c_int32)]
+
+
+ADAM_PACK_ROWS = 16
 
 
 class PatchParams(ctypes.Structure):
@@ -255,6 +266,8 @@
     "ru3d_adam_multi": (_i, [_vp, _vp, _i, _i, _f, _f, _f, _f, _f, _f, _f, _vp]),
     "ru3d_adam_multi_dev": (_i, [_vp, _vp, _i, _i, _vp, _vp]),
     "ru3d_adam_multi_amp": (_i, [_vp, _vp, _i, _i, _vp, _vp, _vp]),
+    "ru3d_adam_pack_multi": (_i, [_vp, _vp, _i, _i, _f, _f, _f, _f, _f, _f, _f, _i, _vp]),
+    "ru3d_adam_pack_multi_dev": (_i, [_vp, _vp, _i, _i, _vp, _i, _vp]),
     "ru3d_amp_update": (_i, [_vp, _f, _f, _i, _f, _f, _vp]),
     "ru3d_grad_sumsq": (_i, [_vp, _vp, _i, _i, _vp, _vp]),
     "ru3d_grad_norm_finish": (_i, [_vp, _i, _f, _vp, _f, _vp, _vp]),
diff --git a/3d-unet-renal-anatomy-extraction_amd/_ops.py b/3d-unet-renal-anatomy-extraction_amd/_ops.py
--- a/3d-unet-renal-anatomy-extraction_amd/_ops.py
+++ b/3d-unet-renal-anatomy-extraction_amd/_ops.py
@@ -54,6 +54,24 @@
 
 
 _PREPACK = {}
+_PACK_GEN = [0]
+_PACK_ITEMS = {}
+CAPTURE_KEEP = [None]
+
+
+class _Pack:
+    __slots__ = ("buf", "wref", "ver", "epoch", "spec", "code", "pooled", "in_capture")
+
+    def current(self):
+        w = self.wref()
+        if w is None or self.ver != w._version or self.epoch != WEIGHTS_EPOCH[0]:
+            return False
+        return not self.in_capture or torch.cuda.is_current_stream_capturing()
+
+    def mark_current(self, in_capture=False):
+        self.ver = self.wref()._version
+        self.epoch = WEIGHTS_EPOCH[0]
+        self.in_capture = in_capture
 
 
 def _spec_key(sp, code):
@@ -67,21 +85,64 @@
     st = None
     outs = []
     for sp in specs:
-        hit = _PREPACK.get(_spec_key(sp, code))
-        if hit is None:
-            return None
-        pack, wref, ver, epoch, stream_id = hit
         w = sp[0]
         if st is None:
             st = torch.cuda.current_stream(w.device).cuda_stream
-        if wref() is not w or ver != w._version or epoch != WEIGHTS_EPOCH[0] or stream_id != st:
+        e = _PREPACK.get((_spec_key(sp, code), st))
+        if e is None or e.wref() is not w or not e.current():
             return None
-        outs.append(pack)
+        outs.append(e.buf)
     return outs
 
 
+def _pack_meta(sp, code):
+    w, role, stride, cout_seg, cin_seg = sp
+    N.require_device(w, "weight")
+    if w.dtype != torch.float32 or not w.is_contiguous():
+        raise N.Ru3dError("ru3d: weights must be contiguous float32 parameters")
+    if role == N.ROLE_BIAS:
+        cout, cin, k, stride = w.shape[0], 1, 1, 1
+        nbytes = 4 * padded_dim(cout, cout_seg)
+    else:
+        k = w.shape[2]
+        if role in (N.ROLE_CONVT_FWD, N.ROLE_CONVT_DGRAD):
+            cin, cout, stride = w.shape[0], w.shape[1], 2
+        else:
+            cout, cin = w.shape[0], w.shape[1]
+        nbytes = N.lib.ru3d_packed_weight_bytes(padded_dim(cout, cout_seg), padded_dim(cin, cin_seg), k, stride,
+                                                role, code)
+    if nbytes == 0:
+        raise N.Ru3dError("ru3d: cannot pack weight of shape %s" % (tuple(w.shape),))
+    return (w.data_ptr(), cout, cin, k, stride, role, cout_seg, cin_seg), nbytes
+
+
+def _pack_entries(entries, capturing=False):
+    if not entries:
+        return
+    code = entries[0].code
+    key = (code,) + tuple(id(e) for e in entries)
+    hit = _PACK_ITEMS.get(key)
+    if hit is None or hit[0] != _PACK_GEN[0]:
+        chunks = []
+        for i0 in range(0, len(entries), N.PACK_MAX):
+            part = entries[i0:i0 + N.PACK_MAX]
+            items = (N.PackItem * len(part))()
+            for j, e in enumerate(part):
+                src, cout, cin, k, stride, role, cout_seg, cin_seg = _pack_meta((e.wref(),) + e.spec, code)[0]
+                items[j] = N.PackItem(src, e.buf.data_ptr(), cout, cin, k, stride, role, cout_seg, cin_seg)
+            chunks.append(items)
+        if len(_PACK_ITEMS) > 64:
+            _PACK_ITEMS.clear()
+        hit = _PACK_ITEMS[key] = (_PACK_GEN[0], chunks, list(entries))
+    N.note_device(entries[0].buf.device)
+    st = stream()
+    for items in hit[1]:
+        check(N.lib.ru3d_pack_weights(items, len(items), code, st), "pack_weights")
+    for e in entries:
+        e.mark_current(capturing)
+
+
 def prepack(specs, dtype):
-    _PREPACK.clear()
     code = N.dtype_code(dtype)
     seen, uniq = set(), []
     for sp in specs:
@@ -89,20 +150,125 @@
         k = _spec_key(sp, code)
         if k not in seen:
             seen.add(k)
-            uniq.append(sp)
+            uniq.append((k, sp))
     if not uniq:
         return
 
-    def order(sp):
-        w, role = sp[0], sp[1]
+    def order(ksp):
+        w, role = ksp[1][0], ksp[1][1]
         if role == N.ROLE_BIAS:
             return (2, 0)
         return (0 if w.shape[2] == 3 else 1, 0)
     uniq.sort(key=order)
-    packs = pack_weights(uniq, dtype)
-    st = torch.cuda.current_stream(uniq[0][0].device).cuda_stream
-    for sp, pk in zip(uniq, packs):
-        _PREPACK[_spec_key(sp, code)] = (pk, weakref.ref(sp[0]), sp[0]._version, WEIGHTS_EPOCH[0], st)
+    st = torch.cuda.current_stream(uniq[0][1][0].device).cuda_stream
+    capturing = torch.cuda.is_current_stream_capturing()
+    keep = (CAPTURE_KEEP[0] or ()) if capturing else None
+    stale = []
+    for k, sp in uniq:
+        w = sp[0]
+        e = _PREPACK.get((k, st))
+        if e is None or e.wref() is not w:
+            if e is None:
+                for dead in [kk for kk, ee in _PREPACK.items() if ee.wref() is None]:
+                    del _PREPACK[dead]
+            e = _Pack()
+            e.buf = torch.empty(_pack_meta(sp, code)[1], dtype=torch.uint8, device=w.device)
+            e.wref, e.ver, e.epoch, e.spec, e.code = weakref.ref(w), -1, -1, sp[1:], code
+            e.pooled, e.in_capture = capturing, False
+            _PREPACK[(k, st)] = e
+            _PACK_GEN[0] += 1
+        if not e.current() or (capturing and id(e) not in keep):
+            stale.append(e)
+    _pack_entries(stale, capturing)
+
+
+def move_packs(src_stream, dst_stream):
+    if src_stream == dst_stream:
+        return
+    for key in [k for k in _PREPACK if k[1] == src_stream]:
+        _PREPACK[(key[0], dst_stream)] = _PREPACK.pop(key)
+    _PACK_GEN[0] += 1
+
+
+def drop_packs(stream_id, back_to=None):
+    for key in [k for k in _PREPACK if k[1] == stream_id]:
+        e = _PREPACK.pop(key)
+        if not e.pooled and back_to is not None and back_to != stream_id:
+            _PREPACK.setdefault((key[0], back_to), e)
+    _PACK_ITEMS.clear()
+    _ADAM_PACKS[0] = _ADAM_PACKS[1] = None
+    _PACK_GEN[0] += 1
+
+
+class AdamPack:
+    __slots__ = ("wref", "a", "b", "code", "adim", "bdim", "taps", "s_a", "a_real", "a_pad", "b_real", "b_pad")
+
+    def entries(self):
+        return [e for e in (self.a, self.b) if e is not None]
+
+    def units(self):
+        return (self.adim // N.ADAM_PACK_ROWS) * (self.bdim // 32)
+
+
+def _pair_form(key):
+    code, _, shape, role, _, cs, ci = key
+    if code not in (N.BF16, N.F16) or role == N.ROLE_BIAS or len(shape) != 5 or shape[2] not in (1, 3):
+        return None
+    conv_t = role in (N.ROLE_CONVT_FWD, N.ROLE_CONVT_DGRAD)
+    a_seg, b_seg = (ci, cs) if conv_t else (cs, ci)
+    if padded_dim(shape[0], a_seg) % 32 or padded_dim(shape[1], b_seg) % 32:
+        return None
+    return role in (N.ROLE_CONV_FWD, N.ROLE_CONVT_DGRAD), a_seg, b_seg
+
+
+_ADAM_PACKS = [None, None]
+
+
+def adam_packs(stream_id):
+    if _ADAM_PACKS[0] == (_PACK_GEN[0], stream_id):
+        return _ADAM_PACKS[1]
+    by_w = {}
+    for (key, st), e in _PREPACK.items():
+        form = _pair_form(key) if st == stream_id else None
+        w = e.wref()
+        if form is not None and w is not None:
+            by_w.setdefault(id(w), []).append((key, form, e, w))
+    out = {}
+    for wid, forms in by_w.items():
+        if len(forms) > 2 or len({(k[0], f[1], f[2]) for k, f, _, _ in forms}) != 1 or \
+                len({f[0] for _, f, _, _ in forms}) != len(forms):
+            continue
+        key, (_, a_seg, b_seg), _, w = forms[0]
+        ap = AdamPack()
+        ap.wref, ap.code, ap.a, ap.b = weakref.ref(w), key[0], None, None
+        for _, f, e, _ in forms:
+            if f[0]:
+                ap.a = e
+            else:
+                ap.b = e
+        shape = key[2]
+        ap.taps = shape[2] ** 3
+        ap.adim, ap.bdim, ap.s_a = padded_dim(shape[0], a_seg), padded_dim(shape[1], b_seg), shape[1] * ap.taps
+        ap.a_real, ap.a_pad = a_seg, cpad(a_seg) if a_seg else 0
+        ap.b_real, ap.b_pad = b_seg, cpad(b_seg) if b_seg else 0
+        out[wid] = ap
+    _ADAM_PACKS[0], _ADAM_PACKS[1] = (_PACK_GEN[0], stream_id), out
+    return out
+
+
+def adam_packs_written(packs, old_epoch, updated=None):
+    for i, ap in enumerate(packs):
+        for e in ap.entries():
+            if updated is None or updated[i]:
+                e.mark_current()
+            elif e.epoch == old_epoch and e.wref() is not None and e.ver == e.wref()._version:
+                e.epoch = WEIGHTS_EPOCH[0]
+
+
+def repack_stale(packs):
+    stale = [e for ap in packs for e in ap.entries() if not e.current()]
+    if stale:
+        _pack_entries(stale)
 
 
 def pack_weights(specs, dtype):
@@ -115,24 +281,9 @@
     plan = _PACK_PLANS.get(key)
     if plan is None:
         metas, sizes = [], []
-        for w, role, stride, cout_seg, cin_seg in specs:
-            N.require_device(w, "weight")
-            if w.dtype != torch.float32 or not w.is_contiguous():
-                raise N.Ru3dError("ru3d: weights must be contiguous float32 parameters")
-            if role == N.ROLE_BIAS:
-                cout, cin, k, stride = w.shape[0], 1, 1, 1
-                nbytes = 4 * padded_dim(cout, cout_seg)
-            else:
-                k = w.shape[2]
-                if role in (N.ROLE_CONVT_FWD, N.ROLE_CONVT_DGRAD):
-                    cin, cout, stride = w.shape[0], w.shape[1], 2
-                else:
-                    cout, cin = w.shape[0], w.shape[1]
-                nbytes = N.lib.ru3d_packed_weight_bytes(padded_dim(cout, cout_seg), padded_dim(cin, cin_seg), k, stride,
-                                                        role, code)
-            if nbytes == 0:
-                raise N.Ru3dError("ru3d: cannot pack weight of shape %s" % (tuple(w.shape),))
-            metas.append((w.data_ptr(), cout, cin, k, stride, role, cout_seg, cin_seg))
+        for sp in specs:
+            meta, nbytes = _pack_meta(sp, code)
+            metas.append(meta)
             sizes.append((nbytes + 255) // 256 * 256)
         offs, off = [], 0
         for sz in sizes:
diff --git a/3d-unet-renal-anatomy-extraction_amd/csrc/api.hip b/3d-unet-renal-anatomy-extraction_amd/csrc/api.hip
--- a/3d-unet-renal-anatomy-extraction_amd/csrc/api.hip
+++ b/3d-unet-renal-anatomy-extraction_amd/csrc/api.hip
@@ -174,9 +174,11 @@
             p.mfma = 3;
         }
     }
-    bool rest = false;
-    for (int i = 0; i < count; i++) rest = rest || b.item[i].mfma != 3;
     if (pairs.count) {
+        int rest = 0;
+        for (int i = 0; i < count; i++)
+            if (b.item[i].mfma != 3) b.item[rest++] = b.item[i];
+        b.count = rest;
         int rc = pack_pair_launch(pairs, as_stream(stream));
         if (rc || !rest) return rc;
     }
diff --git a/3d-unet-renal-anatomy-extraction_amd/csrc/conv_generic.hip b/3d-unet-renal-anatomy-extraction_amd/csrc/conv_generic.hip
--- a/3d-unet-renal-anatomy-extraction_amd/csrc/conv_generic.hip
+++ b/3d-unet-renal-anatomy-extraction_amd/csrc/conv_generic.hip
@@ -1,5 +1,6 @@
 #include "common.h"
 #include "conv.h"
+#include "pack_pair.h"
 
 namespace RU3D_NS {
 
@@ -162,11 +163,6 @@
 }
 
 #define PACK_TILE_FLOATS (32 * (16 * 27 + 1))
-__device__ __forceinline__ int pack_src_index(int p, int real, int pad) {
-    if (pad == 0) return p;
-    const int seg = p / pad, off = p - seg * pad;
-    return off < real ? seg * real + off : -1;
-}
 
 template <typename T>
 __global__ __launch_bounds__(256) void pack_batch_kernel(PackBatch b) {
@@ -174,7 +170,6 @@
     const PackOne& p = b.item[blockIdx.y];
     T* dst = (T*)p.dst;
     const int taps = p.taps;
-    if (p.mfma == 3) return;
     if (p.mfma == 2) {
         float* out = (float*)p.dst;
         for (int i = blockIdx.x * 256 + threadIdx.x; i < p.cout; i += gridDim.x * 256) {
@@ -244,23 +239,20 @@
     }
 }
 
-#define PP_PITCH 40
-#define PP_PLANE (32 * PP_PITCH + 8)
 template <int TAPS>
 __global__ __launch_bounds__(256) void pack_pair_kernel(PackPairBatch pb) {
-    __shared__ __attribute__((aligned(16))) bf16 tile[TAPS * PP_PLANE];
+    __shared__ __attribute__((aligned(16))) bf16 tile[TAPS * PP_PLANE(32)];
     const PackPair& p = pb.item[blockIdx.y];
     if (p.taps != TAPS) return;
     constexpr int taps = TAPS;
+    constexpr int PLANE = PP_PLANE(32);
     const int TA = p.adim / 32, TB = p.bdim / 32;
-    const int lane = threadIdx.x & 63, wave = threadIdx.x >> 6;
     for (int unit = blockIdx.x; unit < TA * TB; unit += gridDim.x) {
         const int ta = unit / TB, tb = unit % TB;
-        const int a_s = pack_src_index(ta * 32, p.a_real, p.a_pad), b_s = pack_src_index(tb * 32, p.b_real, p.b_pad);
-        int a_n = 32, b_n = 32;
-        if (p.a_pad) a_n = a_s < 0 ? 0 : min(32, p.a_real - (ta * 32) % p.a_pad);
-        if (p.b_pad) b_n = b_s < 0 ? 0 : min(32, p.b_real - (tb * 32) % p.b_pad);
-        const float* base = p.src + (int64_t)(a_s < 0 ? 0 : a_s) * p.s_a + (int64_t)(b_s < 0 ? 0 : b_s) * taps;
+        int a_s, b_s;
+        const int a_n = pp_block_real(ta * 32, 32, p.a_real, p.a_pad, &a_s);
+        const int b_n = pp_block_real(tb * 32, 32, p.b_real, p.b_pad, &b_s);
+        const float* base = p.src + (int64_t)a_s * p.s_a + (int64_t)b_s * taps;
         constexpr int run = 32 * taps;
         const int run_n = b_n * taps;
         __syncthreads();
@@ -286,7 +278,7 @@
                         for (int q = 0; q < 4; q++) {
                             const int j = 4 * j4 + q;
                             const int b = j / taps, tap = j - b * taps;
-                            tile[tap * PP_PLANE + a * PP_PITCH + b] = (bf16)v[u][q];
+                            tile[tap * PLANE + a * PP_PITCH + b] = (bf16)v[u][q];
                         }
                     }
                 }
@@ -305,30 +297,12 @@
                     const int e = e0 + u * 256;
                     const int a = e / run, j = e - a * run;
                     const int b = j / taps, tap = j - b * taps;
-                    if (e < 32 * run) tile[tap * PP_PLANE + a * PP_PITCH + b] = (bf16)v[u];
+                    if (e < 32 * run) tile[tap * PLANE + a * PP_PITCH + b] = (bf16)v[u];
                 }
             }
         }
         __syncthreads();
-        if (p.dst_a) {
-            const int KS = p.bdim / 16, NTT = TA;
-            for (int f = wave; f < taps * 2; f += 4) {
-                const int tap = f >> 1, kc = f & 1;
-                const bf16x8 v = *reinterpret_cast<const bf16x8*>(&tile[tap * PP_PLANE + (lane & 31) * PP_PITCH + 16 * kc + 8 * (lane >> 5)]);
-                *reinterpret_cast<bf16x8*>((bf16*)p.dst_a + ((((int64_t)tap * KS + 2 * tb + kc) * NTT + ta) * 64 + lane) * 8) = v;
-            }
-        }
-        if (p.dst_b) {
-            const int KS = p.adim / 16, NTT = TB;
-            for (int f = wave; f < taps * 2; f += 4) {
-                const int tap = f >> 1, kc = f & 1;
-                const int a0 = 16 * kc + 8 * (lane >> 5);
-                bf16x8 v;
-#pragma unroll
-                for (int j = 0; j < 8; j++) v[j] = tile[tap * PP_PLANE + (a0 + j) * PP_PITCH + (lane & 31)];
-                *reinterpret_cast<bf16x8*>((bf16*)p.dst_b + ((((int64_t)tap * KS + 2 * ta + kc) * NTT + tb) * 64 + lane) * 8) = v;
-            }
-        }
+        pp_store_fragments<TAPS, bf16, 32>(tile, p.dst_a, p.dst_b, p.adim, p.bdim, ta * 32, tb);
     }
 }
 
diff --git a/3d-unet-renal-anatomy-extraction_amd/csrc/optim.hip b/3d-unet-renal-anatomy-extraction_amd/csrc/optim.hip
--- a/3d-unet-renal-anatomy-extraction_amd/csrc/optim.hip
+++ b/3d-unet-renal-anatomy-extraction_amd/csrc/optim.hip
@@ -1,4 +1,5 @@
 #include "common.h"
+#include "pack_pair.h"
 #include <stddef.h>
 
 template <class Rule>
@@ -168,6 +169,15 @@
     return ru3d_check_launch("adam_step");
 }
 
+__device__ __forceinline__ void adam_elem(float& p, float g, float& m, float& v, float b1, float b2, float eps, float step,
+                                          float bc2_sqrt, float gscale) {
+#pragma clang fp contract(off)
+    const float gi = g * gscale;
+    m = b1 * m + (1.f - b1) * gi;
+    v = b2 * v + (1.f - b2) * gi * gi;
+    p -= step * (m / (sqrtf(v) / bc2_sqrt + eps));
+}
+
 __device__ __forceinline__ void adam_multi_body(const ru3d_adam_tensor* __restrict__ tensors,
                                                 const int32_t* __restrict__ block_map, int chunk_elems, float lr,
                                                 float b1, float b2, float eps, float bc1, float bc2_sqrt, float gscale) {
@@ -188,10 +198,9 @@
             f32x4 v = *reinterpret_cast<const f32x4*>(t.exp_avg_sq + i);
 #pragma unroll
             for (int k = 0; k < 4; k++) {
-                const float gi = g[k] * gscale;
-                m[k] = b1 * m[k] + (1.f - b1) * gi;
-                v[k] = b2 * v[k] + (1.f - b2) * gi * gi;
-                p[k] -= step * (m[k] / (sqrtf(v[k]) / bc2_sqrt + eps));
+                float pk = p[k], mk = m[k], vk = v[k];
+                adam_elem(pk, g[k], mk, vk, b1, b2, eps, step, bc2_sqrt, gscale);
+                p[k] = pk; m[k] = mk; v[k] = vk;
             }
             *reinterpret_cast<f32x4*>(t.param + i) = p;
             *reinterpret_cast<f32x4*>(t.exp_avg + i) = m;
@@ -200,12 +209,11 @@
     }
     for (; i < end; i += 1024)
         for (int k = 0; k < 4 && i + k < end; k++) {
-            const float gi = t.grad[i + k] * gscale;
-            const float mi = b1 * t.exp_avg[i + k] + (1.f - b1) * gi;
-            const float vi = b2 * t.exp_avg_sq[i + k] + (1.f - b2) * gi * gi;
-            t.exp_avg[i + k] = mi;
-            t.exp_avg_sq[i + k] = vi;
-            t.param[i + k] -= step * (mi / (sqrtf(vi) / bc2_sqrt + eps));
+            float pk = t.param[i + k], mk = t.exp_avg[i + k], vk = t.exp_avg_sq[i + k];
+            adam_elem(pk, t.grad[i + k], mk, vk, b1, b2, eps, step, bc2_sqrt, gscale);
+            t.exp_avg[i + k] = mk;
+            t.exp_avg_sq[i + k] = vk;
+            t.param[i + k] = pk;
         }
 }
 
@@ -242,6 +250,165 @@
     hipLaunchKernelGGL(adam_multi_dev_kernel, dim3((unsigned)nblocks), dim3(256), 0, as_stream(stream), tensors,
                        block_map, chunk_elems, hyper);
     return ru3d_check_launch("adam_multi_dev");
+}
+
+#define AP_ROWS 16
+template <int TAPS, typename T16>
+__device__ __forceinline__ void adam_pack_body(const ru3d_adam_pack_item* __restrict__ items,
+                                               const int32_t* __restrict__ block_map, T16* tile, float lr, float b1,
+                                               float b2, float eps, float bc1, float bc2_sqrt, float gscale) {
+#pragma clang fp contract(off)
+    const ru3d_adam_pack_item it = items[block_map[2 * blockIdx.x]];
+    if (!it.grad || it.taps != TAPS) return;
+    const int TB = it.bdim / 32;
+    const int unit = block_map[2 * blockIdx.x + 1];
+    if (unit < 0 || unit >= (it.adim / AP_ROWS) * TB) return;
+    const int a0 = (unit / TB) * AP_ROWS, tb = unit % TB;
+    int a_s, b_s;
+    const int a_n = pp_block_real(a0, AP_ROWS, it.a_real, it.a_pad, &a_s);
+    const int b_n = pp_block_real(tb * 32, 32, it.b_real, it.b_pad, &b_s);
+    const int64_t off = (int64_t)a_s * it.s_a + (int64_t)b_s * TAPS;
+    float* __restrict__ p = it.param + off;
+    const float* __restrict__ g = it.grad + off;
+    float* __restrict__ m = it.exp_avg + off;
+    float* __restrict__ v = it.exp_avg_sq + off;
+    constexpr int run = 32 * TAPS, PLANE = PP_PLANE(AP_ROWS);
+    const int run_n = b_n * TAPS;
+    const float step = lr / bc1;
+    const bool vec_ok = ((it.s_a | run_n) & 3) == 0 &&
+                        (((uintptr_t)p | (uintptr_t)g | (uintptr_t)m | (uintptr_t)v) & 15) == 0;
+    if (vec_ok) {
+        constexpr int run4 = run / 4;
+        for (int e0 = threadIdx.x; e0 < AP_ROWS * run4; e0 += 2 * 256) {
+            const f32x4 z4 = {0.f, 0.f, 0.f, 0.f};
+            f32x4 pv[2], gv[2], mv[2], vv[2];
+#pragma unroll
+            for (int u = 0; u < 2; u++) {
+                const int e = e0 + u * 256;
+                const int r = e / run4, j4 = e - r * run4;
+                const bool real = e < AP_ROWS * run4 && r < a_n && 4 * j4 < run_n;
+                const int64_t i = (int64_t)r * it.s_a + 4 * j4;
+                pv[u] = real ? *reinterpret_cast<const f32x4*>(p + i) : z4;
+                gv[u] = real ? *reinterpret_cast<const f32x4*>(g + i) : z4;
+                mv[u] = real ? *reinterpret_cast<const f32x4*>(m + i) : z4;
+                vv[u] = real ? *reinterpret_cast<const f32x4*>(v + i) : z4;
+            }
+#pragma unroll
+            for (int u = 0; u < 2; u++) {
+                const int e = e0 + u * 256;
+                if (e >= AP_ROWS * run4) continue;
+                const int r = e / run4, j4 = e - r * run4;
+                if (r < a_n && 4 * j4 < run_n) {
+#pragma unroll
+                    for (int q = 0; q < 4; q++) {
+                        float pk = pv[u][q], mk = mv[u][q], vk = vv[u][q];
+                        adam_elem(pk, gv[u][q], mk, vk, b1, b2, eps, step, bc2_sqrt, gscale);
+                        pv[u][q] = pk; mv[u][q] = mk; vv[u][q] = vk;
+                    }
+                    const int64_t i = (int64_t)r * it.s_a + 4 * j4;
+                    *reinterpret_cast<f32x4*>(p + i) = pv[u];
+                    *reinterpret_cast<f32x4*>(m + i) = mv[u];
+                    *reinterpret_cast<f32x4*>(v + i) = vv[u];
+                }
+#pragma unroll
+                for (int q = 0; q < 4; q++) {
+                    const int j = 4 * j4 + q;
+                    const int b = j / TAPS, tap = j - b * TAPS;
+                    tile[tap * PLANE + r * PP_PITCH + b] = (T16)pv[u][q];
+                }
+            }
+        }
+    } else {
+        for (int e0 = threadIdx.x; e0 < AP_ROWS * run; e0 += 4 * 256) {
+            float pv[4], gv[4], mv[4], vv[4];
+#pragma unroll
+            for (int u = 0; u < 4; u++) {
+                const int e = e0 + u * 256;
+                const int r = e / run, j = e - r * run;
+                const bool real = e < AP_ROWS * run && r < a_n && j < run_n;
+                const int64_t i = (int64_t)r * it.s_a + j;
+                pv[u] = real ? p[i] : 0.f;
+                gv[u] = real ? g[i] : 0.f;
+                mv[u] = real ? m[i] : 0.f;
+                vv[u] = real ? v[i] : 0.f;
+            }
+#pragma unroll
+            for (int u = 0; u < 4; u++) {
+                const int e = e0 + u * 256;
+                if (e >= AP_ROWS * run) continue;
+                const int r = e / run, j = e - r * run;
+                if (r < a_n && j < run_n) {
+                    adam_elem(pv[u], gv[u], mv[u], vv[u], b1, b2, eps, step, bc2_sqrt, gscale);
+                    const int64_t i = (int64_t)r * it.s_a + j;
+                    p[i] = pv[u];
+                    m[i] = mv[u];
+                    v[i] = vv[u];
+                }
+                const int b = j / TAPS, tap = j - b * TAPS;
+                tile[tap * PLANE + r * PP_PITCH + b] = (T16)pv[u];
+            }
+        }
+    }
+    __syncthreads();
+    pp_store_fragments<TAPS, T16, AP_ROWS>(tile, it.dst_a, it.dst_b, it.adim, it.bdim, a0, tb);
+}
+
+template <int TAPS, typename T16>
+__global__ __launch_bounds__(256) void adam_pack_pair_kernel(const ru3d_adam_pack_item* __restrict__ items,
+                                                             const int32_t* __restrict__ block_map, float lr, float b1,
+                                                             float b2, float eps, float bc1, float bc2_sqrt, float gscale) {
+    __shared__ __attribute__((aligned(16))) T16 tile[TAPS * PP_PLANE(AP_ROWS)];
+    adam_pack_body<TAPS, T16>(items, block_map, tile, lr, b1, b2, eps, bc1, bc2_sqrt, gscale);
+}
+
+template <int TAPS, typename T16>
+__global__ __launch_bounds__(256) void adam_pack_pair_dev_kernel(const ru3d_adam_pack_item* __restrict__ items,
+                                                                 const int32_t* __restrict__ block_map,
+                                                                 const float* __restrict__ hyper) {
+    __shared__ __attribute__((aligned(16))) T16 tile[TAPS * PP_PLANE(AP_ROWS)];
+    adam_pack_body<TAPS, T16>(items, block_map, tile, hyper[0], hyper[1], hyper[2], hyper[3], hyper[4], hyper[7], hyper[6]);
+}
+
+template <typename T16>
+static int adam_pack_launch(const ru3d_adam_pack_item* items, const int32_t* block_map, int n27, int n1, float lr, float b1,
+                            float b2, float eps, float bc1, float bc2_sqrt, float gscale, const float* hyper,
+                            hipStream_t st) {
+    const int32_t* map1 = block_map + 2 * (int64_t)n27;
+    if (hyper) {
+        if (n27) hipLaunchKernelGGL((adam_pack_pair_dev_kernel<27, T16>), dim3((unsigned)n27), dim3(256), 0, st, items, block_map, hyper);
+        if (n1) hipLaunchKernelGGL((adam_pack_pair_dev_kernel<1, T16>), dim3((unsigned)n1), dim3(256), 0, st, items, map1, hyper);
+    } else {
+        if (n27) hipLaunchKernelGGL((adam_pack_pair_kernel<27, T16>), dim3((unsigned)n27), dim3(256), 0, st, items, block_map, lr, b1, b2, eps, bc1, bc2_sqrt, gscale);
+        if (n1) hipLaunchKernelGGL((adam_pack_pair_kernel<1, T16>), dim3((unsigned)n1), dim3(256), 0, st, items, map1, lr, b1, b2, eps, bc1, bc2_sqrt, gscale);
+    }
+    return ru3d_check_launch("adam_pack_multi");
+}
+
+extern "C" int ru3d_adam_pack_multi(const ru3d_adam_pack_item* items, const int32_t* block_map, int nblocks27, int nblocks1,
+                                    float lr, float beta1, float beta2, float eps, float bias_corr1, float bias_corr2,
+                                    float grad_scale, int dtype, void* stream) {
+    Ru3dDeviceGuard dev_guard(stream);
+    RU3D_REQUIRE(items && block_map && nblocks27 >= 0 && nblocks1 >= 0 && nblocks27 + (int64_t)nblocks1 > 0,
+                 "adam_pack_multi: bad argument");
+    RU3D_REQUIRE(dtype == RU3D_BF16 || dtype == RU3D_F16, "adam_pack_multi: the packs are bf16 or fp16 (dtype %d)", dtype);
+    if (dtype == RU3D_F16)
+        return adam_pack_launch<_Float16>(items, block_map, nblocks27, nblocks1, lr, beta1, beta2, eps, bias_corr1,
+                                          sqrtf(bias_corr2), grad_scale, nullptr, as_stream(stream));
+    return adam_pack_launch<__bf16>(items, block_map, nblocks27, nblocks1, lr, beta1, beta2, eps, bias_corr1,
+                                    sqrtf(bias_corr2), grad_scale, nullptr, as_stream(stream));
+}
+
+extern "C" int ru3d_adam_pack_multi_dev(const ru3d_adam_pack_item* items, const int32_t* block_map, int nblocks27,
+                                        int nblocks1, const float* hyper, int dtype, void* stream) {
+    Ru3dDeviceGuard dev_guard(stream);
+    RU3D_REQUIRE(items && block_map && hyper && nblocks27 >= 0 && nblocks1 >= 0 && nblocks27 + (int64_t)nblocks1 > 0,
+                 "adam_pack_multi_dev: bad argument");
+    RU3D_REQUIRE(dtype == RU3D_BF16 || dtype == RU3D_F16, "adam_pack_multi_dev: the packs are bf16 or fp16 (dtype %d)", dtype);
+    if (dtype == RU3D_F16)
+        return adam_pack_launch<_Float16>(items, block_map, nblocks27, nblocks1, 0.f, 0.f, 0.f, 0.f, 0.f, 0.f, 0.f, hyper,
+                                          as_stream(stream));
+    return adam_pack_launch<__bf16>(items, block_map, nblocks27, nblocks1, 0.f, 0.f, 0.f, 0.f, 0.f, 0.f, 0.f, hyper,
+                                    as_stream(stream));
 }
 
 __global__ __launch_bounds__(256) void adam_multi_amp_kernel(const ru3d_adam_tensor* __restrict__ tensors,
diff --git a/3d-unet-renal-anatomy-extraction_amd/csrc/pack_pair.h b/3d-unet-renal-anatomy-extraction_amd/csrc/pack_pair.h
--- /dev/null
+++ b/3d-unet-renal-anatomy-extraction_amd/csrc/pack_pair.h
@@ -0,0 +1,50 @@
+#pragma once
+#include "common.h"
+
+__host__ __device__ __forceinline__ int pack_src_index(int p, int real, int pad) {
+    if (pad == 0) return p;
+    const int seg = p / pad, off = p - seg * pad;
+    return off < real ? seg * real + off : -1;
+}
+
+#define PP_PITCH 40
+#define PP_PLANE(arows) ((arows) * PP_PITCH + 8)
+
+__device__ __forceinline__ int pp_block_real(int p0, int n, int real, int pad, int* first) {
+    const int s = pack_src_index(p0, real, pad);
+    *first = s < 0 ? 0 : s;
+    if (!pad) return n;
+    return s < 0 ? 0 : min(n, real - p0 % pad);
+}
+
+template <int TAPS, typename T16, int AROWS>
+__device__ __forceinline__ void pp_store_fragments(const T16* tile, void* dst_a, void* dst_b, int adim, int bdim, int a0,
+                                                   int tb) {
+    typedef __attribute__((ext_vector_type(8))) T16 T16x8;
+    constexpr int PLANE = PP_PLANE(AROWS);
+    const int lane = threadIdx.x & 63, wave = threadIdx.x >> 6;
+    const int ta = a0 >> 5;
+    if (dst_a) {
+        const int KS = bdim / 16, NTT = adim / 32;
+        const int r = (lane & 31) - (a0 & 31);
+        for (int f = wave; f < TAPS * 2; f += 4) {
+            const int tap = f >> 1, kc = f & 1;
+            if (AROWS == 32 || (unsigned)r < (unsigned)AROWS) {
+                const T16x8 v = *reinterpret_cast<const T16x8*>(&tile[tap * PLANE + r * PP_PITCH + 16 * kc + 8 * (lane >> 5)]);
+                *reinterpret_cast<T16x8*>((T16*)dst_a + ((((int64_t)tap * KS + 2 * tb + kc) * NTT + ta) * 64 + lane) * 8) = v;
+            }
+        }
+    }
+    if (dst_b) {
+        const int KS = adim / 16, NTT = bdim / 32;
+        constexpr int NKC = AROWS / 16;
+        for (int f = wave; f < TAPS * NKC; f += 4) {
+            const int tap = f / NKC, kc = f % NKC;
+            const int r0 = 16 * kc + 8 * (lane >> 5);
+            T16x8 v;
+#pragma unroll
+            for (int j = 0; j < 8; j++) v[j] = tile[tap * PLANE + (r0 + j) * PP_PITCH + (lane & 31)];
+            *reinterpret_cast<T16x8*>((T16*)dst_b + ((((int64_t)tap * KS + a0 / 16 + kc) * NTT + tb) * 64 + lane) * 8) = v;
+        }
+    }
+}
diff --git a/3d-unet-renal-anatomy-extraction_amd/graph.py b/3d-unet-renal-anatomy-extraction_amd/graph.py
--- a/3d-unet-renal-anatomy-extraction_amd/graph.py
+++ b/3d-unet-renal-anatomy-extraction_amd/graph.py
@@ -19,10 +19,12 @@
         self.model, self.criterion, self.optimizer = model, criterion, optimizer
         self.scaler = scaler
         self.warmup = max(1, int(warmup))
+        self._packs = []
         self.graph = None
         self.key = None
         self.replays = 0
         self.eager_steps = 0
+        self._packs = []
 
     def _eager(self, x, y):
         self.optimizer.zero_grad(set_to_none=True)
@@ -58,12 +60,21 @@
             self.hyper = self.block[8:].view(torch.float32).view(groups, 8)
             self.host = [torch.zeros(8 + groups * 32, dtype=torch.uint8).pin_memory() for _ in range(_RING)]
             self.host_ev = [None] * _RING
-            self.optimizer.begin_capture(self.hyper)
+            cur = torch.cuda.current_stream(dev)
+            self.stream.wait_stream(cur)
+            self._home = cur.cuda_stream
+            _ops.move_packs(self._home, self.stream.cuda_stream)
+            self.optimizer.begin_capture(self.hyper, stream=self.stream if self.scaler is None else None)
+            self._packs = self.optimizer.capture_packs()
+            if self._packs:
+                with torch.cuda.stream(self.stream):
+                    _ops.repack_stale(self._packs)
             if self.scaler is not None:
                 self.scaler.begin_capture(self.optimizer, dev)
             self.optimizer.zero_grad(set_to_none=True)
             g = torch.cuda.CUDAGraph()
             _ops.DROP_OFFSET_BASE[0] = self.drop_base
+            _ops.CAPTURE_KEEP[0] = {id(e) for ap in self._packs for e in ap.entries()}
             _loss_mod.CAPTURE_SINK[0] = self.label_states = []
             self.stream.wait_stream(torch.cuda.current_stream(dev))
             try:
@@ -80,6 +91,7 @@
                     self._static_logits = _loss_mod.main_output(logits).detach()
             finally:
                 _ops.DROP_OFFSET_BASE[0] = None
+                _ops.CAPTURE_KEEP[0] = None
                 _loss_mod.CAPTURE_SINK[0] = None
         except BaseException:
             _ops._drop_counter[0] = drop0
@@ -115,13 +127,18 @@
         ev = torch.cuda.Event()
         ev.record()
         self.host_ev[slot] = ev
+        if self._packs:
+            _ops.repack_stale(self._packs)
         self.graph.replay()
         if self.label_states:
             import loss as _loss_mod
             for st in self.label_states:
                 _loss_mod._note_label_flag(st)
         _ops._drop_counter[0] += self.draws
+        old_epoch = _ops.WEIGHTS_EPOCH[0]
         _ops.WEIGHTS_EPOCH[0] += 1
+        if self._packs:
+            _ops.adam_packs_written(self._packs, old_epoch)
         self.replays += 1
         self.logits = self._static_logits
         return self.loss
@@ -138,7 +155,7 @@
             sids = (sid,) if side is None else (sid, side.cuda_stream)
             for key in [k for k in N._WS if k[1] in sids]:
                 del N._WS[key]
-            _ops._PREPACK.clear()
+            _ops.drop_packs(sid, getattr(self, "_home", None))
             for name in ("x", "y", "loss", "logits", "_static_logits", "block", "drop_base", "hyper", "host", "host_ev",
                          "stream", "label_states"):
                 if hasattr(self, name):
diff --git a/3d-unet-renal-anatomy-extraction_amd/optim.py b/3d-unet-renal-anatomy-extraction_amd/optim.py
--- a/3d-unet-renal-anatomy-extraction_amd/optim.py
+++ b/3d-unet-renal-anatomy-extraction_amd/optim.py
@@ -1,4 +1,5 @@
 import ctypes
+import os
 
 import torch
 
@@ -25,6 +26,7 @@
 class _Fused(torch.optim.Optimizer):
     _NAME = "optim"
     _COUNTS_STEPS = True
+    _PACKS = False
 
     def __init__(self, params, defaults, max_grad_norm=None):
         self.max_grad_norm = _check_max_grad_norm(max_grad_norm)
@@ -53,10 +55,12 @@
     def captures_with_scaler(self):
         return False
 
-    def _plan(self, gi, group, captured=False):
-        plan = self._plans.get((gi, captured))
-        params = [p for p in group["params"]]
-        if plan is not None and plan["n"] == len(params):
+    def _plan(self, gi, group, captured=False, rest=None):
+        key = (gi, captured) if rest is None else (gi, captured, "rest")
+        plan = self._plans.get(key)
+        params = [p for p in group["params"]] if rest is None else rest[0]
+        sig = None if rest is None else rest[1]
+        if plan is not None and plan["n"] == len(params) and plan["sig"] == sig:
             return plan
         dev = params[0].device
         blocks = []
@@ -69,8 +73,61 @@
         bm = torch.tensor(blocks, dtype=torch.int32).to(dev)
         host = torch.empty(len(params) * ctypes.sizeof(_AdamTensor), dtype=torch.uint8).pin_memory()
         table = torch.empty(host.numel(), dtype=torch.uint8, device=dev)
-        plan = {"n": len(params), "block_map": bm, "nblocks": len(blocks) // 2, "host": host, "table": table}
-        self._plans[(gi, captured)] = plan
+        plan = {"n": len(params), "sig": sig, "block_map": bm, "nblocks": len(blocks) // 2, "host": host, "table": table}
+        self._plans[key] = plan
+        return plan
+
+    def _pack_plan(self, gi, group, captured, grad_scale=1.0, stream_id=None):
+        if not self._PACKS:
+            return None
+        if captured and stream_id is None:
+            if self._captured.get("amp") is not None:
+                return None
+            plan = self._plans.get((gi, True, "pack"))
+            return plan if plan is not None and plan["packs"] else None
+        if self.max_grad_norm is not None or os.environ.get("RU3D_ADAM_PACK", "1") == "0":
+            return None
+        if not captured and float(grad_scale) != 1.0:
+            return None
+        import _ops
+        params = group["params"]
+        if stream_id is None:
+            stream_id = torch.cuda.current_stream(params[0].device).cuda_stream
+        reg = _ops.adam_packs(stream_id)
+        if not reg:
+            return None
+        key = (gi, captured, "pack")
+        sig = (_ops._PACK_GEN[0], stream_id, len(params))
+        plan = self._plans.get(key)
+        if plan is not None and plan["sig"] == sig:
+            return plan if plan["packs"] else None
+        fused = []
+        for p in params:
+            ap = reg.get(id(p))
+            if ap is not None and ap.wref() is p:
+                fused.append((p, ap))
+        fused.sort(key=lambda t: -t[0].numel())
+        fused = [t for t in fused if t[1].code == fused[0][1].code]
+        plan = {"sig": sig, "packs": [ap for _, ap in fused], "params": [p for p, _ in fused]}
+        self._plans[key] = plan
+        if not fused:
+            return None
+        dev = params[0].device
+        index = {id(p): i for i, (p, _) in enumerate(fused)}
+        maps = {27: [], 1: []}
+        for i, (_, ap) in enumerate(fused):
+            for u in range(ap.units()):
+                maps[ap.taps] += [i, u]
+        host = torch.empty(len(fused) * ctypes.sizeof(N.AdamPackItem), dtype=torch.uint8).pin_memory()
+        arr = (N.AdamPackItem * len(fused)).from_buffer(host.numpy())
+        for i, (p, ap) in enumerate(fused):
+            arr[i] = N.AdamPackItem(p.data_ptr(), None, None, None, None if ap.a is None else ap.a.buf.data_ptr(),
+                                    None if ap.b is None else ap.b.buf.data_ptr(), ap.adim, ap.bdim, ap.taps, ap.s_a,
+                                    ap.a_real, ap.a_pad, ap.b_real, ap.b_pad)
+        plan.update(index=index, rest=[p for p in params if id(p) not in index], code=fused[0][1].code, host=host,
+                    table=torch.empty(host.numel(), dtype=torch.uint8, device=dev),
+                    block_map=torch.tensor(maps[27] + maps[1], dtype=torch.int32).to(dev),
+                    n27=len(maps[27]) // 2, n1=len(maps[1]) // 2)
         return plan
 
     def _clip_buffers(self, captured=False):
@@ -104,16 +161,27 @@
             if not params:
                 continue
             self._check_group(group)
-            plan = self._plan(gi, group, capturing)
+            fp = self._pack_plan(gi, group, capturing, grad_scale)
+            rest = params if fp is None else fp["rest"]
+            plan = self._plan(gi, group, capturing, None if fp is None else (rest, fp["sig"])) if rest else None
             N.note_device(params[0].device)
-            if plan.get("copied") is not None and not capturing:
-                plan["copied"].synchronize()
-            arr = (_AdamTensor * len(params)).from_buffer(plan["host"].numpy())
+            for pl in (plan, fp):
+                if pl is not None and pl.get("copied") is not None and not capturing:
+                    pl["copied"].synchronize()
+            arr = (_AdamTensor * len(rest)).from_buffer(plan["host"].numpy()) if plan is not None else None
+            farr = (N.AdamPackItem * len(fp["params"])).from_buffer(fp["host"].numpy()) if fp is not None else None
+            updated = [False] * len(fp["params"]) if fp is not None else None
             step_no = None
             any_grad = False
-            for i, p in enumerate(params):
+            ri = 0
+            for p in params:
+                fi = fp["index"].get(id(p)) if fp is not None else None
                 if p.grad is None:
-                    arr[i] = _AdamTensor(p.data_ptr(), None, None, None, p.numel())
+                    if fi is None:
+                        arr[ri] = _AdamTensor(p.data_ptr(), None, None, None, p.numel())
+                        ri += 1
+                    else:
+                        farr[fi].grad = None
                     continue
                 g = p.grad
                 if g.dtype != torch.float32 or not g.is_contiguous():
@@ -126,24 +194,38 @@
                     step_no = float(st["step"]) if step_no is None else step_no
                     if float(st["step"]) != step_no:
                         raise N.Ru3dError("optim.%s: parameters of one group must share the step count" % self._NAME)
-                arr[i] = _AdamTensor(p.data_ptr(), g.data_ptr(), None if first is None else first.data_ptr(),
-                                     None if second is None else second.data_ptr(), p.numel())
-                any_grad = True
+                if fi is None:
+                    arr[ri] = _AdamTensor(p.data_ptr(), g.data_ptr(), None if first is None else first.data_ptr(),
+                                          None if second is None else second.data_ptr(), p.numel())
+                    ri += 1
+                    any_grad = True
+                else:
+                    it = farr[fi]
+                    it.param, it.grad, it.exp_avg, it.exp_avg_sq = (p.data_ptr(), g.data_ptr(), first.data_ptr(),
+                                                                    second.data_ptr())
+                    updated[fi] = True
             if not any_grad:
+                plan = None
+            if fp is not None and not any(updated):
+                fp = None
+            if plan is None and fp is None:
                 continue
             step_no = 0.0 if step_no is None else step_no
-            plan["table"].copy_(plan["host"], non_blocking=True)
-            if capturing:
-                plan["copied"] = None
-            else:
+            for pl in (plan, fp):
+                if pl is not None:
+                    pl["table"].copy_(pl["host"], non_blocking=True)
+            ev = None
+            if not capturing:
                 ev = torch.cuda.Event()
                 ev.record()
-                plan["copied"] = ev
+            for pl in (plan, fp):
+                if pl is not None:
+                    pl["copied"] = ev
             if clip:
                 check(N.lib.ru3d_grad_sumsq(ptr(plan["table"]), ptr(plan["block_map"]), plan["nblocks"], _CHUNK,
                                             ptr(bufs["partials"][npartials:]), stream()), "grad_sumsq")
                 npartials += plan["nblocks"]
-            ready.append((gi, group, plan, step_no))
+            ready.append((gi, group, plan, fp, step_no, updated))
         coef = None
         if clip and ready:
             N.note_device(bufs["norm"].device)
@@ -152,8 +234,11 @@
                                               self.max_grad_norm, ptr(bufs["norm"]), stream()), "grad_norm_finish")
             coef = bufs["norm"][1:]
             self.last_grad_norm = bufs["norm"][0]
-        for gi, group, plan, step_no in ready:
-            N.note_device(plan["table"].device)
+        written = []
+        for gi, group, plan, fp, step_no, updated in ready:
+            N.note_device((plan or fp)["table"].device)
+            if fp is not None:
+                written.append((fp["packs"], updated))
             if capturing:
                 self._captured["steps"][gi] = step_no - 1.0
                 amp = self._captured.get("amp")
@@ -161,26 +246,43 @@
                     self._captured["amp_base"][gi] = step_no - 1.0
                     check(N.lib.ru3d_adam_multi_amp(ptr(plan["table"]), ptr(plan["block_map"]), plan["nblocks"], _CHUNK,
                                                     ptr(self._captured["hyper"][gi]), ptr(amp), stream()), "adam_multi_amp")
-                else:
+                    continue
+                if fp is not None:
+                    self._launch_pack_dev(fp, self._captured["hyper"][gi])
+                if plan is not None:
                     self._launch_dev(plan, self._captured["hyper"][gi], coef)
                 continue
             if self._captured is not None and gi in self._captured["steps"]:
                 self._captured["steps"][gi] = step_no
                 self._captured["amp_base"][gi] = step_no
-            self._launch(plan, group, step_no, float(grad_scale), coef)
+            if fp is not None:
+                self._launch_pack(fp, group, step_no, float(grad_scale))
+            if plan is not None:
+                self._launch(plan, group, step_no, float(grad_scale), coef)
         import _ops
+        old_epoch = _ops.WEIGHTS_EPOCH[0]
         _ops.WEIGHTS_EPOCH[0] += 1
+        for packs, updated in written:
+            _ops.adam_packs_written(packs, old_epoch, updated)
         return loss
 
-    def begin_capture(self, hyper):
+    def begin_capture(self, hyper, stream=None):
         if hyper.shape != (len(self.param_groups), 8) or hyper.dtype != torch.float32:
             raise ValueError("begin_capture: hyper must be float32 [groups, 8]")
         self._captured = {"hyper": hyper, "steps": {}, "amp": None, "amp_base": {}}
         for gi, group in enumerate(self.param_groups):
             if group["params"]:
                 self._plan(gi, group, True)
+                if stream is not None:
+                    fp = self._pack_plan(gi, group, True, stream_id=stream.cuda_stream)
+                    if fp is not None and fp["rest"]:
+                        self._plan(gi, group, True, (fp["rest"], fp["sig"]))
         if self.max_grad_norm is not None and any(g["params"] for g in self.param_groups):
             self._clip_buffers(True)
+
+    def capture_packs(self):
+        return [ap for key, plan in self._plans.items() if len(key) == 3 and key[1] and key[2] == "pack"
+                for ap in plan["packs"]]
 
     def end_capture(self):
         self._captured = None
@@ -254,6 +356,18 @@
 
     def captures_with_scaler(self):
         return self.max_grad_norm is None
+
+    _PACKS = True
+
+    def _launch_pack(self, fp, group, step_no, grad_scale):
+        b1, b2 = group["betas"]
+        check(N.lib.ru3d_adam_pack_multi(ptr(fp["table"]), ptr(fp["block_map"]), fp["n27"], fp["n1"], float(group["lr"]),
+                                         float(b1), float(b2), float(group["eps"]), 1.0 - b1 ** step_no,
+                                         1.0 - b2 ** step_no, float(grad_scale), fp["code"], stream()), "adam_pack_multi")
+
+    def _launch_pack_dev(self, fp, hyper_row):
+        check(N.lib.ru3d_adam_pack_multi_dev(ptr(fp["table"]), ptr(fp["block_map"]), fp["n27"], fp["n1"], ptr(hyper_row),
+                                             fp["code"], stream()), "adam_pack_multi_dev")
 
     def _launch(self, plan, group, step_no, grad_scale, coef):
         b1, b2 = group["betas"]
diff --git a/include/ru3d.h b/include/ru3d.h
--- a/include/ru3d.h
+++ b/include/ru3d.h
@@ -435,6 +435,23 @@
 int ru3d_adam_multi_dev(const ru3d_adam_tensor* tensors, const int32_t* block_map, int nblocks, int chunk_elems,
                         const float* hyper, void* stream);
 
+typedef struct ru3d_adam_pack_item {
+    float* param;
+    const float* grad;
+    float* exp_avg;
+    float* exp_avg_sq;
+    void* dst_a;
+    void* dst_b;
+    int32_t adim, bdim, taps;
+    int64_t s_a;
+    int32_t a_real, a_pad, b_real, b_pad;
+} ru3d_adam_pack_item;
+int ru3d_adam_pack_multi(const ru3d_adam_pack_item* items, const int32_t* block_map, int nblocks27, int nblocks1,
+                         float lr, float beta1, float beta2, float eps, float bias_corr1, float bias_corr2,
+                         float grad_scale, int dtype, void* stream);
+int ru3d_adam_pack_multi_dev(const ru3d_adam_pack_item* items, const int32_t* block_map, int nblocks27, int nblocks1,
+                             const float* hyper, int dtype, void* stream);
+
 typedef struct ru3d_amp_state {
     float scale, inv_scale, found_inf;
     int32_t tracker, skipped, steps, reserved0, reserved1;
```

After: 269.9 million voxels/s (median of 6 runs). Within noise of the previous version (+0.8%).
